# Samsung/tf-fast-rnnt

Hardware: AMD Instinct MI355X
Metric: rnnt_loss_pruned_fwd_bwd_throughput (higher is better)
Workload: dtype f32; 1 GPU; c3: rnnt_loss_pruned fwd+bwd step, B=32/GPU T=1000 S=200 C=500 s_range=5, regular, full boundary, first pass rnnt_loss_simple; global_batch=32, am_pruned=broadcast view

## Files before the change

### tf-fast-rnnt_amd/csrc/capi.hip

```cpp
#include "ftr_common.h"
#ifdef FTR_DIAG
#include "../../include/ftr_diag.h"
#endif
#include <stdlib.h>
#include <string.h>

namespace ftr {
namespace {
thread_local char g_err[512] = {0};
#ifdef FTR_DIAG
int g_mi_impl = -1;
#endif

int device_ok() {
  int n = 0;
  hipError_t e = hipGetDeviceCount(&n);
  if (e != hipSuccess || n <= 0) {
    (void)hipGetLastError();
    set_error("no usable HIP device (%s); this library has no CPU path", e == hipSuccess ? "device count is 0" : hipGetErrorString(e));
    return FTR_ERR_NO_DEVICE;
  }
  return FTR_OK;
}

// ... 334 lines not shown
int ftr_pruned_joiner_act_bwd_ws_dt(const void* g_out, const void* out, int kind, int act, const int32_t* ranges,
                                    void* d_am, void* d_lm, int B, int T, int S1, int C, int r,
                                    void* workspace, size_t workspace_bytes, void* stream) {
  clear_error();
  FTR_TRY(check_dtype("pruned_joiner_act_bwd_ws_dt", kind, 0));
  FTR_TRY(check_act("pruned_joiner_act_bwd_ws_dt", act));
  const char* what = "do_pruning_bwd_ws";
  FTR_TRY(check_sizes(what, B >= 0 && T >= 0 && S1 >= 1 && C >= 0 && r >= 0));
  if ((size_t)B * C == 0) return FTR_OK;
  FTR_TRY(pointers_then_device(what, g_out && out && ranges && d_am && d_lm));
  return pruned_joiner_act_bwd_ws(g_out, out, kind, act, ranges, d_am, d_lm, B, T, S1, C, r, workspace, workspace_bytes, stream_of(stream));
}

static int pruned_logprobs_fwd_entry(const void* logits, int dtype, const int32_t* symbols, const int32_t* ranges,
                                     const int32_t* boundary, int termination_symbol, double delay_penalty,
                                     float* lse, float* px, float* py, int B, int T, int S, int C, int r,
                                     int modified, int hat, void* stream) {
  const char* what = hat ? "hat_pruned_logprobs_fwd" : "pruned_logprobs_fwd";
  clear_error();
  FTR_TRY(check_builder(what, B >= 0 && T >= 1 && S >= 1 && C >= 1 && r >= 1, termination_symbol, C, false, hat));
  FTR_TRY(check_s_range(what, r, S));
  if (B == 0) return FTR_OK;
  FTR_TRY(pointers_then_device(what, logits && symbols && ranges && lse && px && py));
  return pruned_logprobs_fwd(logits, dtype, symbols, ranges, boundary, termination_symbol, delay_penalty, lse, px, py, B, T, S, C, r, modified, hat, stream_of(stream));
}

int ftr_pruned_logprobs_fwd_f32(const float* logits, const int32_t* symbols, const int32_t* ranges,
                                const int32_t* boundary, int termination_symbol, double delay_penalty,
                                float* lse, float* px, float* py, int B, int T, int S, int C, int r,
                                int modified, void* stream) {
  return pruned_logprobs_fwd_entry(logits, FTR_DTYPE_F32, symbols, ranges, boundary, termination_symbol, delay_penalty, lse, px, py, B, T, S, C, r, modified, 0, stream);
}

int ftr_hat_pruned_logprobs_fwd_f32(const float* logits, const int32_t* symbols, const int32_t* ranges,
                                    const int32_t* boundary, int termination_symbol, double delay_penalty,
                                    float* lse, float* px, float* py, int B, int T, int S, int C, int r,
                                    int modified, void* stream) {
  return pruned_logprobs_fwd_entry(logits, FTR_DTYPE_F32, symbols, ranges, boundary, termination_symbol, delay_penalty, lse, px, py, B, T, S, C, r, modified, 1, stream);
}

int ftr_pruned_logprobs_fwd_dt(const void* logits, int kind, const int32_t* symbols, const int32_t* ranges,
                               const int32_t* boundary, int termination_symbol, double delay_penalty, float* lse,
                               float* px, float* py, int B, int T, int S, int C, int r, int modified, int flags,
                               void* stream) {
  clear_error();
  FTR_TRY(check_dtype("pruned_logprobs_fwd_dt", kind, flags));
  return pruned_logprobs_fwd_entry(logits, kind, symbols, ranges, boundary, termination_symbol, delay_penalty, lse, px, py, B, T, S, C, r, modified, flags & FTR_PRUNED_HAT, stream);
}

int ftr_pruned_logprobs_bwd_f32(const float* logits, const int32_t* symbols, const int32_t* ranges,
                                const int32_t* boundary, int termination_symbol, const float* lse,
                                const float* gpx, const float* gpy, const float* scale, float* glogits,
                                int B, int T, int S, int C, int r, int modified, void* stream) {
  const char* what = "pruned_logprobs_bwd";
  clear_error();
  FTR_TRY(check_builder(what, B >= 0 && T >= 1 && S >= 1 && C >= 1 && r >= 1, termination_symbol, C));
  if (B == 0) return FTR_OK;
  FTR_TRY(pointers_then_device(what, logits && symbols && ranges && lse && gpx && gpy && glogits));
  return pruned_logprobs_bwd(logits, FTR_DTYPE_F32, symbols, ranges, boundary, termination_symbol, lse, gpx, gpy, Scale{scale, 1, 1.0f}, glogits, B, T, S, C, r, modified, 0, stream_of(stream));
}

static int rowmax_exp_entry(const char* what, const float* x, float* probs, float* rowmax, float* rowsum, const float* dotvec,
                            float* dot, bool extras_there, long long rows, int C, void* stream) {
  clear_error();
  FTR_REQUIRE(rows >= 0 && C >= 0, "%s: negative size", what);
  if (rows == 0 || C == 0) return FTR_OK;
  FTR_TRY(pointers_then_device(what, x && probs && rowmax && extras_there));
  return simple_rowmax_exp(x, probs, rowmax, rowsum, dotvec, dot, (size_t)rows, C, stream_of(stream));
}

int ftr_rowmax_exp_f32(const float* x, float* probs, float* rowmax, long long rows, int C, void* stream) {
  return rowmax_exp_entry("rowmax_exp", x, probs, rowmax, nullptr, nullptr, nullptr, true, rows, C, stream);
}

int ftr_rowmax_exp_sum_f32(const float* x, float* probs, float* rowmax, float* rowsum, long long rows, int C,
                           void* stream) {
  return rowmax_exp_entry("rowmax_exp_sum", x, probs, rowmax, rowsum, nullptr, nullptr, rowsum != nullptr, rows, C, stream);
}

int ftr_rowmax_exp_dot_f32(const float* x, float* probs, float* rowmax, const float* dotvec, float* dot, long long rows,
                           int C, void* stream) {
  return rowmax_exp_entry("rowmax_exp_dot", x, probs, rowmax, nullptr, dotvec, dot, dotvec && dot, rows, C, stream);
}

int ftr_rowmax_exp_pair_f32(const float* x1, float* probs1, float* rowmax1, long long rows1, const float* x2, float* probs2,
                            float* rowmax2, long long rows2, int C, void* stream) {
  clear_error();
  FTR_REQUIRE(rows1 >= 0 && rows2 >= 0 && C >= 0, "rowmax_exp_pair: negative size");
  if (rows1 + rows2 == 0 || C == 0) return FTR_OK;
  FTR_TRY(pointers_then_device("rowmax_exp_pair", (rows1 == 0 || (x1 && probs1 && rowmax1)) && (rows2 == 0 || (x2 && probs2 && rowmax2))));
  return simple_rowmax_exp_pair(x1, probs1, rowmax1, (size_t)rows1, x2, probs2, rowmax2, (size_t)rows2, C, stream_of(stream));
}

int ftr_rowdot_f32(const float* x, const float* v, float* dot, long long rows, int C, void* stream) {
  clear_error();
  FTR_REQUIRE(rows >= 0 && C >= 0, "rowdot: negative size");
  if (rows == 0) return FTR_OK;
  FTR_TRY(pointers_then_device("rowdot", dot && ((x && v) || C == 0)));
  return simple_rowdot(x, v, dot, (size_t)rows, C, stream_of(stream));
}

size_t ftr_colsum_weighted_workspace_floats(long long rows, int C) {
  return (rows < 0 || C < 0) ? 0 : simple_colsum_workspace_floats((size_t)rows, C);
}

int ftr_colsum_weighted_f32(const float* x, const float* w, float* out, float* workspace, size_t workspace_floats,
                            long long rows, int C, void* stream) {
  clear_error();
  FTR_REQUIRE(rows >= 0 && C >= 0, "colsum_weighted: negative size");
  if (C == 0) return FTR_OK;
  FTR_TRY(pointers_then_device("colsum_weighted", out && ((x && w && workspace) || rows == 0)));
  return simple_colsum_weighted(x, w, out, workspace, workspace_floats, (size_t)rows, C, stream_of(stream));
}

static int simple_fwd_entry(const char* what, bool smoothed, const float* am, const float* lm, const int32_t* symbols,
                            const float* prod, const float* am_max, const float* lm_max, const float* lmonly_norm,
                            const float* amonly_norm, const float* unigram_log, const int32_t* boundary,
                            int termination_symbol, double delay_penalty, float combined_scale, float lm_only_scale,
                            float am_only_scale, float* px, float* py, int B, int T, int S, int C, int modified, void* stream) {
  clear_error();
  FTR_TRY(check_builder(what, B >= 0 && T >= 1 && S >= 0 && C >= 1, termination_symbol, C));
  if (B == 0) return FTR_OK;
  FTR_TRY(pointers_then_device(what, am && lm && prod && am_max && lm_max && (!smoothed || (lmonly_norm && amonly_norm && unigram_log)) && py && (symbols || S == 0) && (px || S == 0)));
  return simple_logprobs_fwd(am, lm, symbols, prod, am_max, lm_max, boundary, termination_symbol, delay_penalty, lmonly_norm, amonly_norm, unigram_log, combined_scale, lm_only_scale, am_only_scale, px, py, B, T, S, C, modified, stream_of(stream));
}

int ftr_simple_logprobs_fwd_f32(const float* am, const float* lm, const int32_t* symbols, const float* prod,
                                const float* am_max, const float* lm_max, const int32_t* boundary,
                                int termination_symbol, double delay_penalty, float* px, float* py, int B, int T,
                                int S, int C, int modified, void* stream) {
  return simple_fwd_entry("simple_logprobs_fwd", false, am, lm, symbols, prod, am_max, lm_max, nullptr, nullptr, nullptr, boundary, termination_symbol, delay_penalty, 1.0f, 0.0f, 0.0f, px, py, B, T, S, C, modified, stream);
}

int ftr_smoothed_logprobs_fwd_f32(const float* am, const float* lm, const int32_t* symbols, const float* prod,
                                  const float* am_max, const float* lm_max, const float* lmonly_norm,
                                  const float* amonly_norm, const float* unigram_log, const int32_t* boundary,
                                  int termination_symbol, float combined_scale, float lm_only_scale,
                                  float am_only_scale, float* px, float* py, int B, int T, int S, int C,
                                  int modified, void* stream) {
  return simple_fwd_entry("smoothed_logprobs_fwd", true, am, lm, symbols, prod, am_max, lm_max, lmonly_norm, amonly_norm, unigram_log, boundary, termination_symbol, 0.0, combined_scale, lm_only_scale, am_only_scale, px, py, B, T, S, C, modified, stream);
}

int ftr_smoothed_logprobs_fwd_pen_f32(const float* am, const float* lm, const int32_t* symbols, const float* prod,
                                      const float* am_max, const float* lm_max, const float* lmonly_norm,
                                      const float* amonly_norm, const float* unigram_log, const int32_t* boundary,
                                      int termination_symbol, double delay_penalty, float combined_scale,
                                      float lm_only_scale, float am_only_scale, float* px, float* py, int B, int T,
                                      int S, int C, int modified, void* stream) {
  return simple_fwd_entry("smoothed_logprobs_fwd_pen", true, am, lm, symbols, prod, am_max, lm_max, lmonly_norm, amonly_norm, unigram_log, boundary, termination_symbol, delay_penalty, combined_scale, lm_only_scale, am_only_scale, px, py, B, T, S, C, modified, stream);
}

static int bwd_w_entry(const char* what, const float* gpx, const float* gpy, const float* scale, int scale_stride,
                       float scale_mul, const float* prod, const int32_t* boundary, float combined_scale, float* W,
                       float* rsx, float* rsy, int B, int T, int S, int modified, void* stream) {
  clear_error();
  FTR_TRY(check_sizes(what, B >= 0 && T >= 1 && S >= 0));
  FTR_TRY(check_scale_stride(what, scale_stride));
  if (B == 0) return FTR_OK;
  FTR_TRY(pointers_then_device(what, gpy && prod && W && rsx && rsy && (gpx || S == 0)));
  return simple_logprobs_bwd_w(gpx, gpy, Scale{scale, scale_stride, scale_mul}, prod, boundary, W, rsx, rsy, combined_scale, B, T, S, modified, stream_of(stream));
}

int ftr_simple_logprobs_bwd_w_f32(const float* gpx, const float* gpy, const float* prod, const int32_t* boundary,
                                  float* W, float* rsx, float* rsy, int B, int T, int S, int modified, void* stream) {
  return bwd_w_entry("simple_logprobs_bwd_w", gpx, gpy, nullptr, 0, 1.0f, prod, boundary, 1.0f, W, rsx, rsy, B, T, S, modified, stream);
}

int ftr_smoothed_logprobs_bwd_w_f32(const float* gpx, const float* gpy, const float* prod, const int32_t* boundary,
                                    float combined_scale, float* W, float* rsx, float* rsy, int B, int T, int S,
                                    int modified, void* stream) {
  return bwd_w_entry("smoothed_logprobs_bwd_w", gpx, gpy, nullptr, 0, 1.0f, prod, boundary, combined_scale, W, rsx, rsy, B, T, S, modified, stream);
}

int ftr_simple_logprobs_bwd_w_scaled_f32(const float* gpx, const float* gpy, const float* scale, int scale_stride,
                                         float scale_mul, const float* prod, const int32_t* boundary, float* W,
                                         float* rsx, float* rsy, int B, int T, int S, int modified, void* stream) {
  return bwd_w_entry("simple_logprobs_bwd_w_scaled", gpx, gpy, scale, scale_stride, scale_mul, prod, boundary, 1.0f, W, rsx, rsy, B, T, S, modified, stream);
}

int ftr_smoothed_logprobs_bwd_w_scaled_f32(const float* gpx, const float* gpy, const float* scale, int scale_stride,
                                           float scale_mul, const float* prod, const int32_t* boundary,
                                           float combined_scale, float* W, float* rsx, float* rsy, int B, int T, int S,
                                           int modified, void* stream) {
  return bwd_w_entry("smoothed_logprobs_bwd_w_scaled", gpx, gpy, scale, scale_stride, scale_mul, prod, boundary, combined_scale, W, rsx, rsy, B, T, S, modified, stream);
}

static int bwd_am_entry(const char* what, bool smoothed, const float* gpx, const float* gpy, const float* scale,
                        int scale_stride, float scale_mul, const float* damp, const float* am_probs,
                        const int32_t* symbols, const int32_t* boundary, int termination_symbol, float direct_scale,
                        const float* unigram, const float* am_dot, float am_only_scale, float* R, float* d_am, int B,
                        int T, int S, int C, int modified, void* stream) {
  clear_error();
  FTR_TRY(check_builder(what, B >= 0 && T >= 1 && S >= 0 && C >= 1, termination_symbol, C, true));
  FTR_TRY(check_scale_stride(what, scale_stride));
  if (B == 0) return FTR_OK;
  FTR_TRY(pointers_then_device(what, gpy && damp && am_probs && d_am && (!smoothed || (unigram && am_dot && R)) && (gpx || S == 0) && (symbols || S == 0)));
  return simple_logprobs_bwd_am(gpx, gpy, Scale{scale, scale_stride, scale_mul}, damp, am_probs, symbols, boundary, termination_symbol, direct_scale, unigram, am_dot, am_only_scale, R, d_am, B, T, S, C, modified, stream_of(stream));
}

int ftr_simple_logprobs_bwd_am_f32(const float* gpx, const float* gpy, const float* damp, const float* am_probs,
                                   const int32_t* symbols, const int32_t* boundary, int termination_symbol,
                                   float* d_am, int B, int T, int S, int C, int modified, void* stream) {
  return bwd_am_entry("simple_logprobs_bwd_am", false, gpx, gpy, nullptr, 0, 1.0f, damp, am_probs, symbols, boundary, termination_symbol, 1.0f, nullptr, nullptr, 0.0f, nullptr, d_am, B, T, S, C, modified, stream);
}

int ftr_smoothed_logprobs_bwd_am_f32(const float* gpx, const float* gpy, const float* damp, const float* am_probs,
                                     const int32_t* symbols, const int32_t* boundary, int termination_symbol,
                                     float direct_scale, const float* unigram, const float* am_dot,
                                     float am_only_scale, float* R, float* d_am, int B, int T, int S, int C,
                                     int modified, void* stream) {
  return bwd_am_entry("smoothed_logprobs_bwd_am", true, gpx, gpy, nullptr, 0, 1.0f, damp, am_probs, symbols, boundary, termination_symbol, direct_scale, unigram, am_dot, am_only_scale, R, d_am, B, T, S, C, modified, stream);
}

int ftr_simple_logprobs_bwd_am_scaled_f32(const float* gpx, const float* gpy, const float* scale, int scale_stride,
                                          float scale_mul, const float* damp, const float* am_probs,
                                          const int32_t* symbols, const int32_t* boundary, int termination_symbol,
                                          float* d_am, int B, int T, int S, int C, int modified, void* stream) {
  return bwd_am_entry("simple_logprobs_bwd_am_scaled", false, gpx, gpy, scale, scale_stride, scale_mul, damp, am_probs, symbols, boundary, termination_symbol, 1.0f, nullptr, nullptr, 0.0f, nullptr, d_am, B, T, S, C, modified, stream);
}

int ftr_smoothed_logprobs_bwd_am_scaled_f32(const float* gpx, const float* gpy, const float* scale, int scale_stride,
                                            float scale_mul, const float* damp, const float* am_probs,
                                            const int32_t* symbols, const int32_t* boundary, int termination_symbol,
                                            float direct_scale, const float* unigram, const float* am_dot,
                                            float am_only_scale, float* R, float* d_am, int B, int T, int S, int C,
                                            int modified, void* stream) {
  return bwd_am_entry("smoothed_logprobs_bwd_am_scaled", true, gpx, gpy, scale, scale_stride, scale_mul, damp, am_probs, symbols, boundary, termination_symbol, direct_scale, unigram, am_dot, am_only_scale, R, d_am, B, T, S, C, modified, stream);
}

static int bwd_lm_entry(const char* what, bool smoothed, const float* dlmp, const float* lm_probs, const int32_t* symbols,
                        const float* rsx, const float* rsy, int termination_symbol, float direct_scale,
                        const float* row_term, const float* inv_rowsum, const float* unigram_grad, float* d_lm, int B,
                        int S, int C, void* stream) {
  clear_error();
  FTR_TRY(check_builder(what, B >= 0 && S >= 0 && C >= 1, termination_symbol, C, true));
  if (B == 0) return FTR_OK;
  FTR_TRY(pointers_then_device(what, dlmp && lm_probs && rsx && rsy && d_lm && (!smoothed || (row_term && inv_rowsum && unigram_grad)) && (symbols || S == 0)));
  return simple_logprobs_bwd_lm(dlmp, lm_probs, symbols, rsx, rsy, termination_symbol, direct_scale, row_term, inv_rowsum, unigram_grad, d_lm, B, S, C, stream_of(stream));
}

int ftr_simple_logprobs_bwd_lm_f32(const float* dlmp, const float* lm_probs, const int32_t* symbols,
                                   const float* rsx, const float* rsy, int termination_symbol, float* d_lm, int B,
                                   int S, int C, void* stream) {
  return bwd_lm_entry("simple_logprobs_bwd_lm", false, dlmp, lm_probs, symbols, rsx, rsy, termination_symbol, 1.0f, nullptr, nullptr, nullptr, d_lm, B, S, C, stream);
}

int ftr_smoothed_logprobs_bwd_lm_f32(const float* dlmp, const float* lm_probs, const int32_t* symbols,
                                     const float* rsx, const float* rsy, int termination_symbol, float direct_scale,
                                     const float* row_term, const float* inv_rowsum, const float* unigram_grad,
                                     float* d_lm, int B, int S, int C, void* stream) {
  return bwd_lm_entry("smoothed_logprobs_bwd_lm", true, dlmp, lm_probs, symbols, rsx, rsy, termination_symbol, direct_scale, row_term, inv_rowsum, unigram_grad, d_lm, B, S, C, stream);
}

int ftr_negated_reduce_f32(const float* ans, int B, int reduction, float* out, void* stream) {
  clear_error();
  FTR_REQUIRE(B >= 1 && reduction >= 0 && reduction <= 2, "negated_reduce: bad arguments B=%d reduction=%d", B, reduction);
  FTR_TRY(pointers_then_device("negated_reduce", ans && out));
  return negated_reduce(ans, B, reduction, out, stream_of(stream));
}

static int pruned_logprobs_bwd_scaled_entry(const void* logits, int dtype, const int32_t* symbols, const int32_t* ranges,
                                            const int32_t* boundary, int termination_symbol, const float* lse,
                                            const float* gpx, const float* gpy, const float* scale, int scale_stride,
                                            float scale_mul, void* glogits, int B, int T, int S, int C, int r,
                                            int modified, int hat, void* stream) {
  const char* what = hat ? "hat_pruned_logprobs_bwd_scaled" : "pruned_logprobs_bwd_scaled";
  clear_error();
  FTR_TRY(check_builder(what, B >= 0 && T >= 1 && S >= 0 && C >= 1 && r >= 1, termination_symbol, C, true, hat));
  FTR_TRY(check_scale_stride(what, scale_stride));
  if (B == 0) return FTR_OK;
  FTR_TRY(pointers_then_device(what, logits && ranges && lse && gpy && glogits && (symbols || S == 0) && (gpx || S == 0)));
  return pruned_logprobs_bwd(logits, dtype, symbols, ranges, boundary, termination_symbol, lse, gpx, gpy, Scale{scale, scale_stride, scale_mul}, glogits, B, T, S, C, r, modified, hat, stream_of(stream));
}

int ftr_pruned_logprobs_bwd_scaled_f32(const float* logits, const int32_t* symbols, const int32_t* ranges,
                                       const int32_t* boundary, int termination_symbol, const float* lse,
                                       const float* gpx, const float* gpy, const float* scale, int scale_stride,
                                       float scale_mul, float* glogits, int B, int T, int S, int C, int r,
                                       int modified, void* stream) {
  return pruned_logprobs_bwd_scaled_entry(logits, FTR_DTYPE_F32, symbols, ranges, boundary, termination_symbol, lse, gpx, gpy, scale, scale_stride, scale_mul, glogits, B, T, S, C, r, modified, 0, stream);
}

int ftr_hat_pruned_logprobs_bwd_scaled_f32(const float* logits, const int32_t* symbols, const int32_t* ranges,
                                           const int32_t* boundary, int termination_symbol, const float* lse,
                                           const float* gpx, const float* gpy, const float* scale, int scale_stride,
                                           float scale_mul, float* glogits, int B, int T, int S, int C, int r,
                                           int modified, void* stream) {
  return pruned_logprobs_bwd_scaled_entry(logits, FTR_DTYPE_F32, symbols, ranges, boundary, termination_symbol, lse, gpx, gpy, scale, scale_stride, scale_mul, glogits, B, T, S, C, r, modified, 1, stream);
}

int ftr_pruned_logprobs_bwd_scaled_dt(const void* logits, int kind, const int32_t* symbols, const int32_t* ranges,
                                      const int32_t* boundary, int termination_symbol, const float* lse,
                                      const float* gpx, const float* gpy, const float* scale, int scale_stride,
                                      float scale_mul, void* glogits, int B, int T, int S, int C, int r, int modified,
                                      int flags, void* stream) {
  clear_error();
  FTR_TRY(check_dtype("pruned_logprobs_bwd_scaled_dt", kind, flags));
  return pruned_logprobs_bwd_scaled_entry(logits, kind, symbols, ranges, boundary, termination_symbol, lse, gpx, gpy, scale, scale_stride, scale_mul, glogits, B, T, S, C, r, modified, flags & FTR_PRUNED_HAT, stream);
}

int ftr_simple_logprobs_fused_supported(int C) { return simple_fused_supported(C); }
int ftr_simple_logprobs_fused_bwd_supported(int T, int C) { return simple_fused_bwd_supported(T, C); }

int ftr_normalizer_gemm_f32(int kind, const float* x, const float* y, float* out, int B, int T, int S1, int C, void* stream) {
  FTR_REQUIRE(B >= 0 && T >= 0 && S1 >= 0 && C >= 0, "normalizer_gemm: bad sizes");
  if ((size_t)B * T * S1 * C == 0) return FTR_OK;
  FTR_REQUIRE(x && y && out, "normalizer_gemm: null pointer");
  return normalizer_gemm(kind, x, y, out, B, T, S1, C, reinterpret_cast<hipStream_t>(stream));
}

int ftr_normalizer_gemm_choice(int kind, int B, int T, int S1, int C, int* solution, float* us, float* us_default, int* candidates) {
  return normalizer_gemm_choice(kind, B, T, S1, C, solution, us, us_default, candidates);
}

int ftr_normalizer_gemm_set_choice(int kind, int B, int T, int S1, int C, int solution) {
  return normalizer_gemm_set_choice(kind, B, T, S1, C, solution);
}

static int fused_fwd_entry(const char* what, bool smoothed, const float* am, const float* lm, const int32_t* symbols,
                           const float* am_probs, const float* lm_probs, const float* am_max, const float* lm_max,
                           const float* lmonly_norm, const float* amonly_norm, const float* unigram_log,
                           const int32_t* boundary, int termination_symbol, double delay_penalty, float combined_scale,
                           float lm_only_scale, float am_only_scale, float* px, float* py, float* prod, int B, int T,
                           int S, int C, int modified, void* stream) {
  clear_error();
  FTR_TRY(check_builder(what, B >= 0 && T >= 1 && S >= 0 && C >= 1, termination_symbol, C));
  if (B == 0) return FTR_OK;
  FTR_TRY(pointers_then_device(what, am && lm && am_probs && lm_probs && am_max && lm_max && (!smoothed || (lmonly_norm && amonly_norm && unigram_log)) && py && (symbols || S == 0) && (px || S == 0)));
  return simple_fused_fwd(am, lm, symbols, am_probs, lm_probs, am_max, lm_max, boundary, termination_symbol, delay_penalty, lmonly_norm, amonly_norm, unigram_log, combined_scale, lm_only_scale, am_only_scale, px, py, prod, B, T, S, C, modified, stream_of(stream));
}

int ftr_simple_logprobs_fused_fwd_f32(const float* am, const float* lm, const int32_t* symbols, const float* am_probs,
                                      const float* lm_probs, const float* am_max, const float* lm_max,
                                      const int32_t* boundary, int termination_symbol, double delay_penalty, float* px,
                                      float* py, float* prod, int B, int T, int S, int C, int modified, void* stream) {
  return fused_fwd_entry("simple_logprobs_fused_fwd", false, am, lm, symbols, am_probs, lm_probs, am_max, lm_max, nullptr, nullptr, nullptr, boundary, termination_symbol, delay_penalty, 1.0f, 0.0f, 0.0f, px, py, prod, B, T, S, C, modified, stream);
}

int ftr_smoothed_logprobs_fused_fwd_f32(const float* am, const float* lm, const int32_t* symbols, const float* am_probs,
                                        const float* lm_probs, const float* am_max, const float* lm_max,
                                        const float* lmonly_norm, const float* amonly_norm, const float* unigram_log,
                                        const int32_t* boundary, int termination_symbol, double delay_penalty,
                                        float combined_scale, float lm_only_scale, float am_only_scale, float* px,
                                        float* py, float* prod, int B, int T, int S, int C, int modified, void* stream) {
  return fused_fwd_entry("smoothed_logprobs_fused_fwd", true, am, lm, symbols, am_probs, lm_probs, am_max, lm_max, lmonly_norm, amonly_norm, unigram_log, boundary, termination_symbol, delay_penalty, combined_scale, lm_only_scale, am_only_scale, px, py, prod, B, T, S, C, modified, stream);
}

static int fused_bwd_am_entry(const char* what, bool smoothed, const float* gpx, const float* gpy, const float* scale,
                              int scale_stride, float scale_mul, const float* prod, const float* lm_probs,
                              const float* am_probs, const int32_t* symbols, const int32_t* boundary,
                              int termination_symbol, float combined_scale, float direct_scale, const float* unigram,
                              const float* am_dot, float am_only_scale, float* R, float* d_am, int B, int T, int S, int C,
                              int modified, void* stream) {
  clear_error();
  FTR_TRY(check_builder(what, B >= 0 && T >= 1 && S >= 0 && C >= 1, termination_symbol, C, true));
  FTR_TRY(check_scale_stride(what, scale_stride));
  if (B == 0) return FTR_OK;
  FTR_TRY(pointers_then_device(what, gpy && prod && lm_probs && am_probs && d_am && (!smoothed || (unigram && am_dot && R)) && (gpx || S == 0) && (symbols || S == 0)));
  return simple_fused_bwd_am(gpx, gpy, Scale{scale, scale_stride, scale_mul}, prod, lm_probs, am_probs, symbols, boundary, termination_symbol, combined_scale, direct_scale, unigram, am_dot, am_only_scale, R, d_am, B, T, S, C, modified, stream_of(stream));
}

int ftr_simple_logprobs_fused_bwd_am_f32(const float* gpx, const float* gpy, const float* scale, int scale_stride,
                                         float scale_mul, const float* prod, const float* lm_probs, const float* am_probs,
                                         const int32_t* symbols, const int32_t* boundary, int termination_symbol,
                                         float* d_am, int B, int T, int S, int C, int modified, void* stream) {
  return fused_bwd_am_entry("simple_logprobs_fused_bwd_am", false, gpx, gpy, scale, scale_stride, scale_mul, prod, lm_probs, am_probs, symbols, boundary, termination_symbol, 1.0f, 1.0f, nullptr, nullptr, 0.0f, nullptr, d_am, B, T, S, C, modified, stream);
}

int ftr_smoothed_logprobs_fused_bwd_am_f32(const float* gpx, const float* gpy, const float* scale, int scale_stride,
                                           float scale_mul, const float* prod, const float* lm_probs,
                                           const float* am_probs, const int32_t* symbols, const int32_t* boundary,
                                           int termination_symbol, float combined_scale, float direct_scale,
                                           const float* unigram, const float* am_dot, float am_only_scale, float* R,
                                           float* d_am, int B, int T, int S, int C, int modified, void* stream) {
  return fused_bwd_am_entry("smoothed_logprobs_fused_bwd_am", true, gpx, gpy, scale, scale_stride, scale_mul, prod, lm_probs, am_probs, symbols, boundary, termination_symbol, combined_scale, direct_scale, unigram, am_dot, am_only_scale, R, d_am, B, T, S, C, modified, stream);
}

static int fused_bwd_am_w_entry(const char* what, bool smoothed, const float* gpx, const float* gpy, const float* scale,
                                int scale_stride, float scale_mul, const float* W, const float* lm_probs,
                                const float* am_probs, const int32_t* symbols, const int32_t* boundary,
                                int termination_symbol, float direct_scale, const float* unigram, const float* am_dot,
                                float am_only_scale, float* R, float* d_am, int B, int T, int S, int C, int modified,
                                void* stream) {
  clear_error();
  FTR_TRY(check_builder(what, B >= 0 && T >= 1 && S >= 0 && C >= 1, termination_symbol, C, true));
  FTR_TRY(check_scale_stride(what, scale_stride));
  if (B == 0) return FTR_OK;
  FTR_TRY(pointers_then_device(what, gpy && W && lm_probs && am_probs && d_am && (!smoothed || (unigram && am_dot && R)) && (gpx || S == 0) && (symbols || S == 0)));
  return simple_fused_bwd_am_w(gpx, gpy, Scale{scale, scale_stride, scale_mul}, W, lm_probs, am_probs, symbols, boundary, termination_symbol, direct_scale, unigram, am_dot, am_only_scale, R, d_am, B, T, S, C, modified, stream_of(stream));
}

int ftr_simple_logprobs_fused_bwd_am_w_f32(const float* gpx, const float* gpy, const float* scale, int scale_stride,
                                           float scale_mul, const float* W, const float* lm_probs, const float* am_probs,
                                           const int32_t* symbols, const int32_t* boundary, int termination_symbol,
                                           float* d_am, int B, int T, int S, int C, int modified, void* stream) {
  return fused_bwd_am_w_entry("simple_logprobs_fused_bwd_am_w", false, gpx, gpy, scale, scale_stride, scale_mul, W, lm_probs, am_probs, symbols, boundary, termination_symbol, 1.0f, nullptr, nullptr, 0.0f, nullptr, d_am, B, T, S, C, modified, stream);
}

int ftr_smoothed_logprobs_fused_bwd_am_w_f32(const float* gpx, const float* gpy, const float* scale, int scale_stride,
                                             float scale_mul, const float* W, const float* lm_probs,
                                             const float* am_probs, const int32_t* symbols, const int32_t* boundary,
                                             int termination_symbol, float direct_scale, const float* unigram,
                                             const float* am_dot, float am_only_scale, float* R, float* d_am, int B, int T,
                                             int S, int C, int modified, void* stream) {
  return fused_bwd_am_w_entry("smoothed_logprobs_fused_bwd_am_w", true, gpx, gpy, scale, scale_stride, scale_mul, W, lm_probs, am_probs, symbols, boundary, termination_symbol, direct_scale, unigram, am_dot, am_only_scale, R, d_am, B, T, S, C, modified, stream);
}

int ftr_simple_logprobs_fused_bwd_am_w_columns(int B, int T, int C) { return simple_fused_bwd_columns(B, T, C); }

int ftr_mutual_information_band_supported(int T, int S, int r) { return mi_band_supported(T, S, r); }

static int pruned_band_fwd_entry(const void* logits, int dtype, const int32_t* symbols, const int32_t* ranges, const int32_t* boundary,
                                 int termination_symbol, double delay_penalty, float* lse, float* px_band, float* py_band,
                                 int B, int T, int S, int C, int r, int modified, int hat, void* stream) {
  const char* what = hat ? "hat_pruned_band_fwd" : "pruned_band_fwd";
  clear_error();
  FTR_TRY(check_builder(what, B >= 0 && T >= 1 && S >= 0 && C >= 1 && r >= 1, termination_symbol, C, false, hat));
  if (B == 0) return FTR_OK;
  FTR_TRY(pointers_then_device(what, logits && ranges && lse && px_band && py_band && (symbols || S == 0)));
  FTR_TRY(lse_rows_dtype(logits, dtype, lse, (size_t)B * T * r, C, termination_symbol, hat, stream_of(stream)));
  return band_gather(logits, dtype, symbols, ranges, boundary, lse, termination_symbol, delay_penalty, px_band, py_band, B, T, S, C, r, modified, hat, stream_of(stream));
}

int ftr_pruned_band_fwd_f32(const float* logits, const int32_t* symbols, const int32_t* ranges, const int32_t* boundary,
                            int termination_symbol, double delay_penalty, float* lse, float* px_band, float* py_band,
                            int B, int T, int S, int C, int r, int modified, void* stream) {
  return pruned_band_fwd_entry(logits, FTR_DTYPE_F32, symbols, ranges, boundary, termination_symbol, delay_penalty, lse, px_band, py_band, B, T, S, C, r, modified, 0, stream);
}

int ftr_hat_pruned_band_fwd_f32(const float* logits, const int32_t* symbols, const int32_t* ranges, const int32_t* boundary,
                                int termination_symbol, double delay_penalty, float* lse, float* px_band, float* py_band,
                                int B, int T, int S, int C, int r, int modified, void* stream) {
  return pruned_band_fwd_entry(logits, FTR_DTYPE_F32, symbols, ranges, boundary, termination_symbol, delay_penalty, lse, px_band, py_band, B, T, S, C, r, modified, 1, stream);
}

int ftr_pruned_band_fwd_dt(const void* logits, int kind, const int32_t* symbols, const int32_t* ranges,
                           const int32_t* boundary, int termination_symbol, double delay_penalty, float* lse,
                           float* px_band, float* py_band, int B, int T, int S, int C, int r, int modified, int flags,
                           void* stream) {
  clear_error();
  FTR_TRY(check_dtype("pruned_band_fwd_dt", kind, flags));
  return pruned_band_fwd_entry(logits, kind, symbols, ranges, boundary, termination_symbol, delay_penalty, lse, px_band, py_band, B, T, S, C, r, modified, flags & FTR_PRUNED_HAT, stream);
}

int ftr_band_ranges_check_i32(const int32_t* ranges, const int32_t* boundary, int32_t* flags, int B, int T, int r, void* stream) {
  clear_error();
  FTR_TRY(check_sizes("band_ranges_check", B >= 0 && T >= 0 && r >= 1));
  FTR_TRY(pointers_then_device("band_ranges_check", flags && (ranges || B == 0 || T == 0)));
  return band_ranges_check(ranges, boundary, flags, B, T, r, stream_of(stream));
}

int ftr_mutual_information_band_f32(const float* px_band, const float* py_band, const int32_t* ranges,
                                    const int32_t* boundary, float* ans, float* gx_band, float* gy_band, int B, int T,
                                    int S, int r, int modified, void* stream) {
  return ftr_mutual_information_band_ws_f32(px_band, py_band, ranges, boundary, nullptr, 0, ans, gx_band, gy_band, B, T, S, r, modified, stream);
}

size_t ftr_mutual_information_band_workspace_floats(int B, int T, int S, int r) {
  return (B < 0 || T < 1 || S < 0 || r < 1) ? 0 : mi_band_workspace_floats(B, T, S, r);
}

int ftr_mutual_information_band_ws_f32(const float* px_band, const float* py_band, const int32_t* ranges,
                                       const int32_t* boundary, float* workspace, size_t workspace_floats, float* ans,
                                       float* gx_band, float* gy_band, int B, int T, int S, int r, int modified,
                                       void* stream) {
  clear_error();
  FTR_TRY(check_sizes("mutual_information_band", B >= 0 && T >= 1 && S >= 0 && r >= 1));
  if (B == 0) return FTR_OK;
  FTR_TRY(pointers_then_device("mutual_information_band", px_band && py_band && ranges && ans && gx_band && gy_band));
  return mi_band(px_band, py_band, ranges, boundary, workspace, workspace_floats, ans, gx_band, gy_band, B, T, S, r, modified, stream_of(stream));
}

static int pruned_band_bwd_scaled_entry(const void* logits, int dtype, const int32_t* symbols, const int32_t* ranges,
                                        const int32_t* boundary, int termination_symbol, const float* lse,
                                        const float* gx_band, const float* gy_band, const float* scale, int scale_stride,
                                        float scale_mul, void* glogits, int B, int T, int S, int C, int r, int modified,
                                        int hat, void* stream) {
  const char* what = hat ? "hat_pruned_band_bwd_scaled" : "pruned_band_bwd_scaled";
  clear_error();
  FTR_TRY(check_builder(what, B >= 0 && T >= 1 && S >= 0 && C >= 1 && r >= 1, termination_symbol, C, true, hat));
  FTR_TRY(check_scale_stride(what, scale_stride));
  if (B == 0) return FTR_OK;
  FTR_TRY(pointers_then_device(what, logits && ranges && lse && gx_band && gy_band && glogits && (symbols || S == 0)));
  return band_grad_banded(logits, dtype, symbols, ranges, boundary, termination_symbol, lse, gx_band, gy_band, Scale{scale, scale_stride, scale_mul}, glogits, B, T, S, C, r, modified, hat, stream_of(stream));
}

int ftr_pruned_band_bwd_scaled_f32(const float* logits, const int32_t* symbols, const int32_t* ranges,
                                   const int32_t* boundary, int termination_symbol, const float* lse,
                                   const float* gx_band, const float* gy_band, const float* scale, int scale_stride,
                                   float scale_mul, float* glogits, int B, int T, int S, int C, int r, int modified,
                                   void* stream) {
  return pruned_band_bwd_scaled_entry(logits, FTR_DTYPE_F32, symbols, ranges, boundary, termination_symbol, lse, gx_band, gy_band, scale, scale_stride, scale_mul, glogits, B, T, S, C, r, modified, 0, stream);
}

int ftr_hat_pruned_band_bwd_scaled_f32(const float* logits, const int32_t* symbols, const int32_t* ranges,
                                       const int32_t* boundary, int termination_symbol, const float* lse,
                                       const float* gx_band, const float* gy_band, const float* scale, int scale_stride,
                                       float scale_mul, float* glogits, int B, int T, int S, int C, int r, int modified,
                                       void* stream) {
  return pruned_band_bwd_scaled_entry(logits, FTR_DTYPE_F32, symbols, ranges, boundary, termination_symbol, lse, gx_band, gy_band, scale, scale_stride, scale_mul, glogits, B, T, S, C, r, modified, 1, stream);
}

int ftr_pruned_band_bwd_scaled_dt(const void* logits, int kind, const int32_t* symbols, const int32_t* ranges,
                                  const int32_t* boundary, int termination_symbol, const float* lse,
                                  const float* gx_band, const float* gy_band, const float* scale, int scale_stride,
                                  float scale_mul, void* glogits, int B, int T, int S, int C, int r, int modified,
                                  int flags, void* stream) {
  clear_error();
  FTR_TRY(check_dtype("pruned_band_bwd_scaled_dt", kind, flags));
  return pruned_band_bwd_scaled_entry(logits, kind, symbols, ranges, boundary, termination_symbol, lse, gx_band, gy_band, scale, scale_stride, scale_mul, glogits, B, T, S, C, r, modified, flags & FTR_PRUNED_HAT, stream);
}

namespace {
int mb_check_durations(const char* what, const int32_t* durations, int D, bool first_is_one) {
  FTR_REQUIRE(D >= 1 && D <= 8, "%s: D = %d, the number of blanks must be in 1..8", what, D);
  FTR_REQUIRE(durations, "%s: null durations", what);
  for (int j = 0; j < D; ++j) {
    FTR_REQUIRE(durations[j] >= 1 && durations[j] <= 32, "%s: durations[%d] = %d is outside 1..32", what, j, durations[j]);
    FTR_REQUIRE(j == 0 || durations[j] > durations[j - 1], "%s: durations must be strictly increasing (durations[%d] = %d after %d)",
                what, j, durations[j], durations[j - 1]);
  }
  FTR_REQUIRE(!first_is_one || durations[0] == 1, "%s: durations[0] = %d, the standard blank advances one frame", what, durations[0]);
  return FTR_OK;
}
int mb_check_ids(const char* what, const int32_t* ids, int D, int blank, int C) {
  FTR_REQUIRE(C >= 1 && blank >= 0 && blank < C, "%s: termination_symbol %d not in [0,%d)", what, blank, C);
  FTR_REQUIRE(ids || D == 1, "%s: null big_blank_ids", what);
  for (int j = 0; j + 1 < D; ++j) {
    FTR_REQUIRE(ids[j] >= 0 && ids[j] < C, "%s: big_blank_ids[%d] = %d not in [0,%d)", what, j, ids[j], C);
    FTR_REQUIRE(ids[j] != blank, "%s: big_blank_ids[%d] = %d is the termination_symbol", what, j, ids[j]);
    for (int i = 0; i < j; ++i)
      FTR_REQUIRE(ids[i] != ids[j], "%s: big_blank_ids[%d] = %d is a duplicate of big_blank_ids[%d]", what, j, ids[j], i);
  }
  return FTR_OK;
}
}

namespace {
int tdt_check_list(const char* what, const char* name, const int32_t* v, int n, int nmax, int lo, int hi = 16) {
  FTR_REQUIRE(n >= 1 && n <= nmax, "%s: %s holds %d values, must be 1..%d", what, name, n, nmax);
  FTR_REQUIRE(v, "%s: null %s", what, name);
  for (int j = 0; j < n; ++j) {
    FTR_REQUIRE(v[j] >= lo && v[j] <= hi, "%s: %s[%d] = %d is outside %d..%d", what, name, j, v[j], lo, hi);
    FTR_REQUIRE(j == 0 || v[j] > v[j - 1], "%s: %s must be strictly increasing (%s[%d] = %d after %d)", what, name, name, j,
                v[j], v[j - 1]);
  }
  return FTR_OK;
}
int tdt_check_moves(const char* what, const int32_t* token_durations, int Dx, const int32_t* blank_durations, int Dy,
                    int blank_hi = 16, int max_moves = 9) {
  FTR_TRY(tdt_check_list(what, "token_durations", token_durations, Dx, 8, 0));
  FTR_TRY(tdt_check_list(what, "blank_durations", blank_durations, Dy, 8, 1, blank_hi));
  FTR_REQUIRE(Dx + Dy <= max_moves, "%s: Dx + Dy = %d moves (token_durations and blank_durations together), at most %d", what,
              Dx + Dy, max_moves);
  return FTR_OK;
}
int tdt_check_head(const char* what, const int32_t* durations, int N, double sigma, int blank, int C) {
  FTR_TRY(tdt_check_list(what, "durations", durations, N, 5, 0));
  FTR_REQUIRE(durations[N - 1] >= 1, "%s: durations holds no positive value: no move advances a frame", what);
  FTR_REQUIRE(sigma >= 0.0, "%s: sigma = %g must not be negative", what, sigma);
  FTR_REQUIRE(C >= 1 && blank >= 0 && blank < C, "%s: termination_symbol %d not in [0,%d)", what, blank, C);
// ... 398 lines not shown
```

### tf-fast-rnnt_amd/csrc/ftr_common.h

```cpp
#pragma once
#include <hip/hip_runtime.h>
#include <stdint.h>
#include <stdio.h>
#include <stdarg.h>
#include "../../include/ftr_kd.h"
#include "../../include/ftr_prune_sum.h"
#include "../../include/ftr_joiner_act.h"
#include "../../include/ftr_fused.h"
#include "../../include/ftr_band_tdt.h"
#include "../../include/ftr_band_multiblank.h"
#include "../../include/ftr_band_viterbi.h"

namespace ftr {

void set_error(const char* fmt, ...);
void clear_error();

inline int check_launch(const char* what) {
  hipError_t e = hipGetLastError();
  if (e != hipSuccess) {
    set_error("%s: launch failed: %s", what, hipGetErrorString(e));
    return FTR_ERR_LAUNCH;
  }
  return FTR_OK;
}

inline int require_rows_32bit(const char* what, size_t rows) {
  if (rows > 0x7fffffffull) {
    set_error("%s: %zu rows (B*T*s_range) exceed the 2^31 - 1 that the launch grids index", what, rows);
    return FTR_ERR_INVALID_ARG;
  }
  return FTR_OK;
}

__global__ void zero_words_kernel(uint32_t* __restrict__ p, size_t n);
__global__ void copy_words_kernel(uint32_t* __restrict__ dst, const uint32_t* __restrict__ src, size_t n);
inline int zero_words(void* p, size_t n_words, hipStream_t st, const char* what) {
  if (n_words == 0) return FTR_OK;
  const size_t blocks = (n_words + 4 * 256 - 1) / (4 * 256);
  hipLaunchKernelGGL(zero_words_kernel, dim3((unsigned)(blocks > 4096 ? 4096 : blocks)), dim3(256), 0, st, static_cast<uint32_t*>(p), n_words);
  return check_launch(what);
}
inline int copy_words(void* dst, const void* src, size_t n_words, hipStream_t st, const char* what) {
  if (n_words == 0) return FTR_OK;
  const size_t blocks = (n_words + 255) / 256;
  hipLaunchKernelGGL(copy_words_kernel, dim3((unsigned)(blocks > 4096 ? 4096 : blocks)), dim3(256), 0, st, static_cast<uint32_t*>(dst),
                     static_cast<const uint32_t*>(src), n_words);
  return check_launch(what);
}

constexpr float kNeg = -1.0e30f;
constexpr float kNegThresh = -1.0e29f;
constexpr float kLog2e = 1.4426950408889634f;
constexpr float kLn2 = 0.6931471805599453f;

typedef float f4u __attribute__((ext_vector_type(4), aligned(4)));
typedef float f4 __attribute__((ext_vector_type(4)));

struct bf16_t { uint16_t bits; };
struct fp16_t { uint16_t bits; };
typedef uint16_t h4 __attribute__((ext_vector_type(4)));

__device__ __forceinline__ float elem_to_float(float v) { return v; }
__device__ __forceinline__ float elem_to_float(bf16_t v) { return (float)__builtin_bit_cast(__bf16, v.bits); }
__device__ __forceinline__ float elem_to_float(fp16_t v) { return (float)__builtin_bit_cast(_Float16, v.bits); }
template <typename E> __device__ __forceinline__ E elem_from_float(float v);
template <> __device__ __forceinline__ float elem_from_float<float>(float v) { return v; }
template <> __device__ __forceinline__ bf16_t elem_from_float<bf16_t>(float v) { return bf16_t{__builtin_bit_cast(uint16_t, (__bf16)v)}; }
template <> __device__ __forceinline__ fp16_t elem_from_float<fp16_t>(float v) { return fp16_t{__builtin_bit_cast(uint16_t, (_Float16)v)}; }

__device__ __forceinline__ f4 load4(const float* row, int i) { return reinterpret_cast<const f4u*>(row)[i]; }
__device__ __forceinline__ void store4(float* row, int i, f4 v) { reinterpret_cast<f4u*>(row)[i] = v; }
template <typename E>
__device__ __forceinline__ f4 load4(const E* row, int i) {
  const h4 h = reinterpret_cast<const h4*>(row)[i];
  f4 v;
#pragma unroll
  for (int e = 0; e < 4; ++e) v[e] = elem_to_float(E{h[e]});
  return v;
}
template <typename E>
__device__ __forceinline__ void store4(E* row, int i, f4 v) {
  h4 h;
#pragma unroll
  for (int e = 0; e < 4; ++e) h[e] = elem_from_float<E>(v[e]).bits;
  reinterpret_cast<h4*>(row)[i] = h;
}
__device__ __forceinline__ void store4_nt(float* row, int i, f4 v) { __builtin_nontemporal_store(v, reinterpret_cast<f4u*>(row) + i); }
template <typename E>
__device__ __forceinline__ void store4_nt(E* row, int i, f4 v) {
  h4 h;
#pragma unroll
  for (int e = 0; e < 4; ++e) h[e] = elem_from_float<E>(v[e]).bits;
  __builtin_nontemporal_store(h, reinterpret_cast<h4*>(row) + i);
}

struct Scale {
  const float* p; int stride; float mul;
  __device__ __forceinline__ float at(int b) const { return (p ? p[(size_t)b * stride] : 1.0f) * mul; }
};
inline Scale scale_none() { return Scale{nullptr, 0, 1.0f}; }

template <int CTRL, int ROW_MASK, int BANK_MASK>
__device__ __forceinline__ float dpp_take(float identity, float src) {
  return __builtin_bit_cast(float, __builtin_amdgcn_update_dpp(__builtin_bit_cast(int, identity), __builtin_bit_cast(int, src),
                                                               CTRL, ROW_MASK, BANK_MASK, false));
}
__device__ __forceinline__ float wave_sum_dpp(float v) {
  v += dpp_take<0x111, 0xf, 0xf>(0.0f, v);
  v += dpp_take<0x112, 0xf, 0xf>(0.0f, v);
  v += dpp_take<0x114, 0xf, 0xe>(0.0f, v);
  v += dpp_take<0x118, 0xf, 0xc>(0.0f, v);
  v += dpp_take<0x142, 0xa, 0xf>(0.0f, v);
  v += dpp_take<0x143, 0xc, 0xf>(0.0f, v);
  return __builtin_bit_cast(float, __builtin_amdgcn_readlane(__builtin_bit_cast(int, v), 63));
}
__device__ __forceinline__ float wave_max_dpp(float v) {
  constexpr float ninf = -__builtin_inff();
  v = fmaxf(v, dpp_take<0x111, 0xf, 0xf>(ninf, v));
  v = fmaxf(v, dpp_take<0x112, 0xf, 0xf>(ninf, v));
  v = fmaxf(v, dpp_take<0x114, 0xf, 0xe>(ninf, v));
  v = fmaxf(v, dpp_take<0x118, 0xf, 0xc>(ninf, v));
  v = fmaxf(v, dpp_take<0x142, 0xa, 0xf>(ninf, v));
  v = fmaxf(v, dpp_take<0x143, 0xc, 0xf>(ninf, v));
  return __builtin_bit_cast(float, __builtin_amdgcn_readlane(__builtin_bit_cast(int, v), 63));
}

struct Shift { float cx2, cy2; };
__device__ __forceinline__ bool shift_sample_ok(float v) { return v > -1.0e4f && v < 1.0e4f; }
template <bool MOD>
__device__ __forceinline__ Shift shift_from_sums(float sumx, float nx, float sumy, float ny, int Sn, int Tn) {
  const float steps = MOD ? (float)(Tn - 1) : (float)(Sn - 1 + Tn - 1);
  float f = steps > 0.0f ? (float)(Sn - 1) / steps : 0.5f;
  f = fminf(fmaxf(f, 1.0e-3f), 1.0f - 1.0e-3f);
  const float mx = nx > 0.0f ? sumx / nx : 0.0f, my = ny > 0.0f ? sumy / ny : 0.0f;
  Shift s;
  s.cx2 = mx * kLog2e - __builtin_amdgcn_logf(f);
  s.cy2 = my * kLog2e - __builtin_amdgcn_logf(1.0f - f);
  return s;
}
template <bool MOD>
__device__ __forceinline__ double shift_total(const Shift s, int Sn, int Tn) {
  const int nx = Sn - 1, ny = MOD ? (Tn - 1) - (Sn - 1) : (Tn - 1);
  return (double)nx * (double)s.cx2 + (double)ny * (double)s.cy2;
}

struct Bound { int sb, tb, se, te; };
__device__ __forceinline__ Bound load_boundary(const int32_t* __restrict__ boundary, int b, int S, int T) {
  Bound r;
  if (boundary) {
    r.sb = max(boundary[4 * b + 0], 0); r.tb = max(boundary[4 * b + 1], 0);
    r.se = min(boundary[4 * b + 2], S); r.te = min(boundary[4 * b + 3], T);
  } else { r.sb = 0; r.tb = 0; r.se = S; r.te = T; }
  return r;
}

__device__ __forceinline__ float softplus(float v) { return fmaxf(v, 0.0f) + log1pf(expf(-fabsf(v))); }
__device__ __forceinline__ void hat_logprobs(float xb, float xs, float Z, bool sym_is_blank, float* vx, float* vy) {
  *vy = -softplus(-xb);
  *vx = sym_is_blank ? -INFINITY : (xs - Z) - softplus(xb);
}
__device__ __forceinline__ void hat_sigmoids(float xb, float* sp, float* sn) {
  const float e = expf(-fabsf(xb)), big = 1.0f / (1.0f + e), small = e / (1.0f + e);
  *sp = xb >= 0.0f ? big : small;
  *sn = xb >= 0.0f ? small : big;
}

}

namespace ftr {
int mi_plain_fwd(const float* px, const float* py, const int32_t* boundary, float* p, float* ans, int B, int S, int T, int modified, hipStream_t st);
int mi_plain_bwd(const float* px, const float* py, const int32_t* boundary, const float* p, float* p_grad, float* px_grad, float* py_grad, float* ans_grad, int overwrite, int B, int S, int T, int modified, hipStream_t st);
int mi_bidir_fwd(const float* px, const float* py, const int32_t* boundary, float* ws, size_t ws_floats, int flags, float* ans, int B, int S, int T, int modified, hipStream_t st);
int mi_bidir_bwd(const int32_t* boundary, const float* ws, size_t ws_floats, int flags, float* px_grad, float* py_grad, float* ans_grad, int overwrite, int B, int S, int T, int modified, hipStream_t st, const float* ans = nullptr, float* loss_out = nullptr, int loss_code = 0);
int mi_bidir_ws_init(float* ws, size_t ws_floats, int B, int S, int T, hipStream_t st);
int mi_bidir_status(const float* ws, size_t ws_floats, int B, int S, int T, int* status_host, long long* dirty_host, hipStream_t st);
size_t mi_bidir_workspace_floats(int B, int S, int T);
size_t mi_bidir_handoff_floats(int B, int S, int T);
size_t mi_viterbi_workspace_bytes(int B, int S, int T);
int mi_viterbi(const float* px, const float* py, const int32_t* boundary, void* ws, size_t ws_bytes, float* score, int32_t* frames, int B, int S, int T, int modified, hipStream_t st);
size_t mi_multiblank_workspace_floats(int B, int S, int T);
int mi_multiblank_fwd(const float* px, const float* py, const int32_t* boundary, const int32_t* durations, int D, float* ws, size_t ws_floats, float* ans, int B, int S, int T, hipStream_t st);
int mi_multiblank_bwd(const float* px, const float* py, const int32_t* boundary, const int32_t* durations, int D, float* ws, size_t ws_floats, const float* ans_grad, float* px_grad, float* py_grad, int B, int S, int T, hipStream_t st);
int multiblank_logprobs_fwd(const float* logits, const int32_t* symbols, const int32_t* ranges, const int32_t* boundary, int blank, const int32_t* big_ids, const int32_t* durations, int D, double sigma, double delay_penalty, float* lse, float* px, float* py, int B, int T, int S, int C, int r, hipStream_t st);
int multiblank_logprobs_bwd(const float* logits, const int32_t* symbols, const int32_t* ranges, const int32_t* boundary, int blank, const int32_t* big_ids, const int32_t* durations, int D, const float* lse, const float* gpx, const float* gpy, Scale scale, float* glogits, int B, int T, int S, int C, int r, hipStream_t st);
size_t mi_tdt_workspace_floats(int B, int S, int T);
int mi_tdt_fwd(const float* px, const float* py, const int32_t* boundary, const int32_t* token_durations, int Dx, const int32_t* blank_durations, int Dy, float* ws, size_t ws_floats, float* ans, int B, int S, int T, hipStream_t st);
int mi_tdt_bwd(const float* px, const float* py, const int32_t* boundary, const int32_t* token_durations, int Dx, const int32_t* blank_durations, int Dy, float* ws, size_t ws_floats, const float* ans_grad, float* px_grad, float* py_grad, int B, int S, int T, hipStream_t st);
int tdt_logprobs_fwd(const float* logits, const int32_t* symbols, const int32_t* ranges, const int32_t* boundary, int blank, const int32_t* durations, int N, double sigma, double delay_penalty, float* lse_tok, float* lse_dur, float* px, float* py, int B, int T, int S, int C, int r, hipStream_t st);
int tdt_logprobs_bwd(const float* logits, const int32_t* symbols, const int32_t* ranges, const int32_t* boundary, int blank, const int32_t* durations, int N, const float* lse_tok, const float* lse_dur, const float* gpx, const float* gpy, Scale scale, float* glogits, int B, int T, int S, int C, int r, hipStream_t st);
struct BandMoveDomain { int max_tok, max_blk, max_dur; };
constexpr BandMoveDomain kBandTdtDomain{5, 5, 16};
constexpr BandMoveDomain kBandMultiblankDomain{1, 8, 32};
int mi_band_tdt_supported(int T, int S, int r, int N, int Ny, BandMoveDomain dom);
size_t mi_band_tdt_workspace_floats(int B, int T, int S, int r, int N, int Ny, BandMoveDomain dom);
int mi_band_tdt(const float* pxb, const float* pyb, const int32_t* ranges, const int32_t* boundary, const int32_t* token_durations, int N, const int32_t* blank_durations, int Ny, float* ws, size_t ws_floats, float* ans, float* gxb, float* gyb, int B, int T, int S, int r, BandMoveDomain dom, const char* what, hipStream_t st);
int tdt_band_fwd(const float* logits, const int32_t* symbols, const int32_t* ranges, const int32_t* boundary, int blank, const int32_t* durations, int N, double sigma, double delay_penalty, float* lse_tok, float* lse_dur, float* pxb, float* pyb, int B, int T, int S, int C, int r, hipStream_t st);
int tdt_band_bwd(const float* logits, const int32_t* symbols, const int32_t* ranges, const int32_t* boundary, int blank, const int32_t* durations, int N, const float* lse_tok, const float* lse_dur, const float* gxb, const float* gyb, Scale scale, float* glogits, int B, int T, int S, int C, int r, hipStream_t st);
int mi_band_multiblank(const float* pxb, const float* pyb, const int32_t* ranges, const int32_t* boundary, const int32_t* durations, int D, float* ws, size_t ws_floats, float* ans, float* gxb, float* gyb, int B, int T, int S, int r, hipStream_t st);
int multiblank_band_fwd(const float* logits, const int32_t* symbols, const int32_t* ranges, const int32_t* boundary, int blank, const int32_t* big_ids, const int32_t* durations, int D, double sigma, double delay_penalty, float* lse, float* pxb, float* pyb, int B, int T, int S, int C, int r, hipStream_t st);
int multiblank_band_bwd(const float* logits, const int32_t* symbols, const int32_t* ranges, const int32_t* boundary, int blank, const int32_t* big_ids, const int32_t* durations, int D, const float* lse, const float* gxb, const float* gyb, Scale scale, float* glogits, int B, int T, int S, int C, int r, hipStream_t st);
size_t mi_viterbi_tdt_workspace_bytes(int B, int S, int T);
int mi_viterbi_tdt(const float* px, const float* py, const int32_t* boundary, const int32_t* token_durations, int Dx, const int32_t* blank_durations, int Dy, void* ws, size_t ws_bytes, float* score, int32_t* frames, int32_t* durations, int32_t* blank_steps, int B, int S, int T, hipStream_t st);
int mi_band_viterbi_supported(int T, int S, int r, int N, int Ny);
size_t mi_band_viterbi_workspace_bytes(int B, int T, int S, int r, int N, int Ny);
int mi_band_viterbi(const float* pxb, const float* pyb, const int32_t* ranges, const int32_t* boundary, const int32_t* token_durations, int N, const int32_t* blank_durations, int Ny, void* ws, size_t ws_bytes, float* score, int32_t* frames, int32_t* durations, int32_t* blank_steps, int B, int T, int S, int r, hipStream_t st);
int cummin_i32(const int32_t* in, int32_t* out, int rows, int cols, hipStream_t st);
int prune_ranges(const float* px_grad, const float* py_grad, const int32_t* boundary, int32_t* ranges, int32_t* s_begin, int B, int S, int T, int T1, int r, hipStream_t st);
int do_pruning(const float* am, const float* lm, const int32_t* ranges, float* am_p, float* lm_p, int B, int T, int S1, int C, int r, hipStream_t st);
size_t do_pruning_bwd_workspace_bytes(int B, int T, int S1, int C, int r);
int do_pruning_bwd_ws(const float* g_am_p, const float* g_lm_p, const int32_t* ranges, float* d_am, float* d_lm, int B, int T, int S1, int C, int r, void* ws, size_t ws_bytes, hipStream_t st);
int do_pruning_bwd(const float* g_am_p, const float* g_lm_p, const int32_t* ranges, float* d_am, float* d_lm, int B, int T, int S1, int C, int r, hipStream_t st);
int do_pruning_sum(const void* am, const void* lm, int dtype, const int32_t* ranges, void* out, int B, int T, int S1, int C, int r, hipStream_t st);
int do_pruning_sum_bwd_ws(const void* g, int dtype, const int32_t* ranges, void* d_am, void* d_lm, int B, int T, int S1, int C, int r, void* ws, size_t ws_bytes, hipStream_t st);
int pruned_joiner_act(const void* am, const void* lm, int dtype, int act, const int32_t* ranges, void* out, int B, int T, int S1, int C, int r, hipStream_t st);
int pruned_joiner_act_bwd_ws(const void* g, const void* out, int dtype, int act, const int32_t* ranges, void* d_am, void* d_lm, int B, int T, int S1, int C, int r, void* ws, size_t ws_bytes, hipStream_t st);
int pruned_logprobs_fwd(const void* logits, int dtype, const int32_t* symbols, const int32_t* ranges, const int32_t* boundary, int blank, double delay_penalty, float* lse, float* px, float* py, int B, int T, int S, int C, int r, int modified, int hat, hipStream_t st);
int pruned_logprobs_bwd(const void* logits, int dtype, const int32_t* symbols, const int32_t* ranges, const int32_t* boundary, int blank, const float* lse, const float* gpx, const float* gpy, Scale scale, void* glogits, int B, int T, int S, int C, int r, int modified, int hat, hipStream_t st);
int simple_rowmax_exp(const float* x, float* probs, float* rowmax, float* rowsum, const float* dotvec, float* dot, size_t rows, int C, hipStream_t st);
int simple_rowmax_exp_pair(const float* x1, float* probs1, float* rowmax1, size_t rows1, const float* x2, float* probs2, float* rowmax2, size_t rows2, int C, hipStream_t st);
int simple_rowdot(const float* x, const float* v, float* dot, size_t rows, int C, hipStream_t st);
size_t simple_colsum_workspace_floats(size_t rows, int C);
int simple_colsum_weighted(const float* x, const float* w, float* out, float* ws, size_t ws_floats, size_t rows, int C, hipStream_t st);
int simple_logprobs_fwd(const float* am, const float* lm, const int32_t* symbols, const float* prod, const float* am_max, const float* lm_max, const int32_t* boundary, int blank, double delay_penalty, const float* lmonly_norm, const float* amonly_norm, const float* ulog, float cs, float ls, float as, float* px, float* py, int B, int T, int S, int C, int modified, hipStream_t st);
int simple_logprobs_bwd_w(const float* gpx, const float* gpy, Scale scale, const float* prod, const int32_t* boundary, float* W, float* rsx, float* rsy, float cs, int B, int T, int S, int modified, hipStream_t st);
int simple_logprobs_bwd_am(const float* gpx, const float* gpy, Scale scale, const float* damp, const float* am_probs, const int32_t* symbols, const int32_t* boundary, int blank, float kdir, const float* uvec, const float* amdot, float as, float* Rout, float* d_am, int B, int T, int S, int C, int modified, hipStream_t st);
int simple_logprobs_bwd_lm(const float* dlmp, const float* lm_probs, const int32_t* symbols, const float* rsx, const float* rsy, int blank, float kdir, const float* arow, const float* invsum, const float* gu, float* d_lm, int B, int S, int C, hipStream_t st);
int simple_fused_supported(int C);
int simple_fused_bwd_supported(int T, int C);
int normalizer_gemm(int kind, const float* x, const float* y, float* out, int B, int T, int S1, int C, hipStream_t st);
int normalizer_gemm_choice(int kind, int B, int T, int S1, int C, int* solution, float* us, float* us_default, int* candidates);
int normalizer_gemm_set_choice(int kind, int B, int T, int S1, int C, int solution);
int simple_fused_fwd(const float* am, const float* lm, const int32_t* symbols, const float* am_probs, const float* lm_probs, const float* am_max, const float* lm_max, const int32_t* boundary, int blank, double delay_penalty, const float* lmonly_norm, const float* amonly_norm, const float* ulog, float cs, float ls, float as, float* px, float* py, float* prod_out, int B, int T, int S, int C, int modified, hipStream_t st);
int simple_fused_bwd_am(const float* gpx, const float* gpy, Scale scale, const float* prod, const float* lm_probs, const float* am_probs, const int32_t* symbols, const int32_t* boundary, int blank, float cs, float kdir, const float* uvec, const float* amdot, float as, float* Rout, float* d_am, int B, int T, int S, int C, int modified, hipStream_t st);
int simple_fused_bwd_columns(int B, int T, int C);
int simple_fused_bwd_am_w(const float* gpx, const float* gpy, Scale scale, const float* W, const float* lm_probs, const float* am_probs, const int32_t* symbols, const int32_t* boundary, int blank, float kdir, const float* uvec, const float* amdot, float as, float* Rout, float* d_am, int B, int T, int S, int C, int modified, hipStream_t st);
int negated_reduce(const float* ans, int B, int reduction, float* out, hipStream_t st, float sign = -1.0f);
int pruned_kd_fwd(const void* logits, int dtype, const void* teacher, int teacher_dtype, const int32_t* symbols, const int32_t* ranges, const int32_t* boundary, int blank, float temperature, int collapsed, float* node, float* saved, float* utt, int B, int T, int S, int C, int r, hipStream_t st);
int pruned_kd_bwd(const void* logits, int dtype, const void* teacher, int teacher_dtype, const int32_t* symbols, const int32_t* ranges, const int32_t* boundary, int blank, float temperature, int collapsed, const float* saved, Scale scale, void* glogits, int B, int T, int S, int C, int r, hipStream_t st);
int lse_rows(const float* logits, float* lse, size_t rows, int C, int blank, int hat, hipStream_t st);
int lse_rows_dtype(const void* logits, int dtype, float* lse, size_t rows, int C, int blank, int hat, hipStream_t st);
int mi_band_supported(int T, int S, int r);
int band_ranges_check(const int32_t* ranges, const int32_t* boundary, int* flags, int B, int T, int r, hipStream_t st);
int band_gather(const void* logits, int dtype, const int32_t* symbols, const int32_t* ranges, const int32_t* boundary, const float* lse, int blank, double delay_penalty, float* pxb, float* pyb, int B, int T, int S, int C, int r, int modified, int hat, hipStream_t st);
size_t mi_band_workspace_floats(int B, int T, int S, int r);
int mi_band_seg_supported(int T, int S, int r);
size_t mi_band_seg_workspace_floats(int B, int T, int S, int r);
int mi_band_seg(const float* pxb, const float* pyb, const int32_t* ranges, const int32_t* boundary, float* ws, size_t ws_floats, float* ans, float* gxb, float* gyb, int B, int T, int S, int r, int modified, hipStream_t st);
int mi_band(const float* pxb, const float* pyb, const int32_t* ranges, const int32_t* boundary, float* ws, size_t ws_floats, float* ans, float* gxb, float* gyb, int B, int T, int S, int r, int modified, hipStream_t st);
int band_grad_banded(const void* logits, int dtype, const int32_t* symbols, const int32_t* ranges, const int32_t* boundary, int blank, const float* lse, const float* gxb, const float* gyb, Scale scale, void* glogits, int B, int T, int S, int C, int r, int modified, int hat, hipStream_t st);
int selftest(hipStream_t st, int* result_dev);
int debug_stamps(unsigned long long* out16);
int debug_trace(unsigned long long* out, int n);
}
```

### tf-fast-rnnt_amd/csrc/simple_fused.hip

```cpp
#include "ftr_common.h"
#include "launch.h"
#include <cstdlib>

namespace ftr {
namespace {

constexpr float kTinyF = 1.401298464324817e-45f;
template <int MB> struct FusedTile {
  static constexpr int FT = 64 * MB, FK = 32, FLD = FK + 4, NBUF = MB == 1 ? 2 : 1;
};
typedef float v4f __attribute__((ext_vector_type(4)));

constexpr int kGLD = 68;
template <int NS, int MB>
__host__ __device__ constexpr size_t fused_lds_bytes() {
  constexpr size_t tile = FusedTile<MB>::NBUF * (size_t)(FusedTile<MB>::FT + 16 * NS) * FusedTile<MB>::FLD;
  constexpr size_t gather = (size_t)16 * NS * kGLD + 16 * NS + (size_t)16 * NS * 8 + (size_t)FusedTile<MB>::FT * 4;
  return sizeof(float) * (tile > gather ? tile : gather);
}

template <bool MOD, bool SMOOTH, int NS, int MB>
__global__ __launch_bounds__(256, 2) void simple_fused_fwd_kernel(
    const float* __restrict__ am, const float* __restrict__ lm, const int32_t* __restrict__ symbols,
    const float* __restrict__ am_probs, const float* __restrict__ lm_probs, const float* __restrict__ am_max,
// ... 99 lines not shown
    constexpr int kAheadU = 4, RING = 8;
    f4 af[MB][kFK / 16], ring[RING];
#pragma unroll
    for (int m = 0; m < MB; ++m)
#pragma unroll
      for (int g = 0; g < kFK / 16; ++g) af[m][g] = *reinterpret_cast<const f4*>(A + 64 * m * kFLD + 16 * g);
    auto bfetch = [&](int u) { return *reinterpret_cast<const f4*>(Bm + (u % NS) * 16 * kFLD + 16 * (u / NS)); };
#pragma unroll
    for (int u = 0; u < kAheadU; ++u) if (u < NUNIT) ring[u % RING] = bfetch(u);
#pragma unroll
    for (int u = 0; u < NUNIT; u += 2) {
      if (u + kAheadU < NUNIT) ring[(u + kAheadU) % RING] = bfetch(u + kAheadU);
      if (u + kAheadU + 1 < NUNIT) ring[(u + kAheadU + 1) % RING] = bfetch(u + kAheadU + 1);
      const int g0 = u / NS, i0 = u % NS;
      const f4 b0 = ring[u % RING];
      if (u + 1 < NUNIT) {
        const int g1 = (u + 1) / NS, i1 = (u + 1) % NS;
        const f4 b1 = ring[(u + 1) % RING];
#pragma unroll
        for (int e = 0; e < 4; ++e) {
#pragma unroll
          for (int m = 0; m < MB; ++m) {
            acc[m][i0] = __builtin_amdgcn_mfma_f32_16x16x4f32(af[m][g0][e], b0[e], acc[m][i0], 0, 0, 0);
            acc[m][i1] = __builtin_amdgcn_mfma_f32_16x16x4f32(af[m][g1][e], b1[e], acc[m][i1], 0, 0, 0);
          }
        }
      } else {
#pragma unroll
        for (int e = 0; e < 4; ++e)
#pragma unroll
          for (int m = 0; m < MB; ++m) acc[m][i0] = __builtin_amdgcn_mfma_f32_16x16x4f32(af[m][g0][e], b0[e], acc[m][i0], 0, 0, 0);
      }
      __builtin_amdgcn_sched_barrier(0);
    }
    if (NBUF == 1) __syncthreads();
    if (kc + 1 < nk) lstore(NBUF == 2 ? ((kc + 1) & 1) : 0, v);
    __syncthreads();
  }

  const int n = lane & 15;
  const int te = boundary ? boundary[4 * b + 3] : T;
  const float ulog_blank = SMOOTH ? ulog[blank] : 0.0f;
  float* asym = smem;
  int* sym_l = reinterpret_cast<int*>(smem + 16 * NS * kGLD);
  float* rrec = smem + 16 * NS * kGLD + 16 * NS;
  float* frec = rrec + 16 * NS * 8;
  if (tid < 16 * NS) {
    sym_l[tid] = r_sym;
    *reinterpret_cast<f4*>(rrec + 8 * tid) = f4{r_lmblank, r_lmx, r_lmsym, 0.f};
    if (SMOOTH) *reinterpret_cast<f4*>(rrec + 8 * tid + 4) = f4{r_lon, r_ulog, 0.f, 0.f};
  }
  if (tid < kFT) *reinterpret_cast<f4*>(frec + 4 * tid) = f4{f_amx, f_ablank, f_aon, 0.f};
  __syncthreads();
  float lm_blank[NS], lmx[NS], lon[NS], lm_sym[NS], ulog_sym[NS];
#pragma unroll
  for (int i = 0; i < NS; ++i) {
    const f4 ra = *reinterpret_cast<const f4*>(rrec + 8 * (16 * i + n));
    lm_blank[i] = ra[0]; lmx[i] = ra[1]; lm_sym[i] = ra[2];
    lon[i] = 0.f; ulog_sym[i] = 0.f;
    if (SMOOTH) { const f4 rb = *reinterpret_cast<const f4*>(rrec + 8 * (16 * i + n) + 4); lon[i] = rb[0]; ulog_sym[i] = rb[1]; }
  }
  constexpr int NSL = (16 * NS + 63) / 64;
  int mysym[NSL];
#pragma unroll
  for (int u = 0; u < NSL; ++u) mysym[u] = sym_l[min(lane + 64 * u, 16 * NS - 1)];
#pragma unroll
  for (int m = 0; m < MB; ++m) {
    if (m > 0) __syncthreads();
    {
      constexpr int GB = (MB == 2 && NS > 10) ? 8 : 16;
#pragma unroll
      for (int k0 = 0; k0 < 16; k0 += GB) {
        float gv[GB][NSL];
#pragma unroll
        for (int k = 0; k < GB; ++k) {
          const float* row = amb + (size_t)min(t0 + 64 * m + wave + 4 * (k0 + k), T - 1) * C;
#pragma unroll
          for (int u = 0; u < NSL; ++u) gv[k][u] = row[mysym[u]];
        }
#pragma unroll
        for (int k = 0; k < GB; ++k)
#pragma unroll
          for (int u = 0; u < NSL; ++u) {
            const int sl = lane + 64 * u;
            if (sl < 16 * NS) asym[sl * kGLD + wave + 4 * (k0 + k)] = gv[k][u];
          }
      }
    }
    __syncthreads();
    const int tq = t0 + 64 * m + 16 * wave + 4 * (lane >> 4);
    if (tq >= T1) continue;
    float amx[4], a_blank[4], aon[4], pen[4];
#pragma unroll
    for (int j = 0; j < 4; ++j) {
      const int t = tq + j;
      const f4 fr = *reinterpret_cast<const f4*>(frec + 4 * (64 * m + 16 * wave + 4 * (lane >> 4) + j));
      amx[j] = fr[0]; a_blank[j] = fr[1]; aon[j] = fr[2];
      pen[j] = (delay_penalty > 0.0) ? (float)((((double)te - 1.0) / 2.0 - (double)t) * delay_penalty) : 0.0f;
    }
    f4 a_sym[NS];
#pragma unroll
    for (int i = 0; i < NS; ++i) a_sym[i] = *reinterpret_cast<const f4*>(asym + (16 * i + n) * kGLD + 16 * wave + 4 * (lane >> 4));
#pragma unroll
    for (int i = 0; i < NS; ++i) {
      const int s = s0 + 16 * i + n;
      if (s > S) continue;
      f4 vy, vx, vp;
#pragma unroll
      for (int j = 0; j < 4; ++j) {
        const int t = tq + j;
        const float pr = acc[m][i][j];
        vp[j] = pr;
        const float nrm = logf(pr + kTinyF) + lmx[i] + amx[j];
        float y = a_blank[j] + lm_blank[i] - nrm;
        if (SMOOTH) y = y * cs + (lm_blank[i] - lon[i]) * ls + (a_blank[j] + ulog_blank - aon[j]) * as;
        vy[j] = y;
        float x = -INFINITY;
        if (s < S && t < T && (MOD || t != te)) {
          x = a_sym[i][j] + lm_sym[i] - nrm;
          if (SMOOTH) x = x * cs + (lm_sym[i] - lon[i]) * ls + (a_sym[i][j] + ulog_sym[i] - aon[j]) * as;
        }
        if (delay_penalty > 0.0) x += pen[j];
        vx[j] = x;
      }
      float* yrow = py + ((size_t)b * (S + 1) + s) * T + tq;
      if (tq + 3 < T) *reinterpret_cast<f4u*>(yrow) = vy;
      else { for (int j = 0; j < 4; ++j) if (tq + j < T) yrow[j] = vy[j]; }
      if (prod_out) {
        float* prow = prod_out + ((size_t)b * (S + 1) + s) * T + tq;
        if (tq + 3 < T) *reinterpret_cast<f4u*>(prow) = vp;
        else { for (int j = 0; j < 4; ++j) if (tq + j < T) prow[j] = vp[j]; }
      }
      if (s < S) {
        float* xrow = px + ((size_t)b * S + s) * T1 + tq;
        if (tq + 3 < T1) *reinterpret_cast<f4u*>(xrow) = vx;
        else { for (int j = 0; j < 4; ++j) if (tq + j < T1) xrow[j] = vx[j]; }
      }
    }
  }
}


constexpr int kBT = 64;
constexpr int kBS = 16;
constexpr int kBLT = kBT + 4;
constexpr int kBCB = 16;

template <int NCB>
__host__ __device__ constexpr size_t fused_bwd_lds_bytes() {
  return sizeof(float) * (2 * kBS * (16 * NCB) + 2 * kBS * kBLT + 2 * kBS * kBT);
}

template <bool MOD, bool USEW, int NCB>
__global__ __launch_bounds__(256, NCB <= 8 ? 4 : 2) void simple_fused_bwd_am_kernel(
    const float* __restrict__ gpx, const float* __restrict__ gpy, const Scale scale, const float* __restrict__ prod,
    const float* __restrict__ lm_probs, const float* __restrict__ am_probs, const int32_t* __restrict__ symbols,
    const int32_t* __restrict__ boundary, int blank, float cs, float kdir, const float* __restrict__ uvec,
    const float* __restrict__ amdot, float as, float* __restrict__ Rout, float* __restrict__ d_am, int T, int S, int C) {
  extern __shared__ __attribute__((aligned(16))) float smem[];
  constexpr int CT = 16 * NCB, LDC = CT, NG = NCB / 4;
  static_assert(NCB % 4 == 0 && NCB >= 8 && NCB <= 16, "column blocks come in interleaved groups of four");
  float* lmT = smem;
  float* wT = lmT + 2 * kBS * LDC;
  float* csb = wT + 2 * kBS * kBLT;
  int bx = blockIdx.x, by = blockIdx.y, bz = blockIdx.z;
  {
    const unsigned total = gridDim.x * gridDim.y * gridDim.z;
    if ((total & 7u) == 0) {
      const unsigned lin = blockIdx.x + gridDim.x * (blockIdx.y + gridDim.y * blockIdx.z);
      const unsigned j = (lin & 7u) * (total >> 3) + (lin >> 3);
      by = j % gridDim.y; bx = (j / gridDim.y) % gridDim.x; bz = j / (gridDim.x * gridDim.y);
    }
  }
  const int b = bz, t0 = bx * kBT, c0 = by * CT;
  const int tid = threadIdx.x, lane = tid & 63;
  const int wave = __builtin_amdgcn_readfirstlane(tid >> 6);
  const int T1 = MOD ? T : T + 1;
  const int te = boundary ? boundary[4 * b + 3] : T;
  const float sc = scale.at(b);
  const float* gxb = gpx + (size_t)b * S * T1;
  const float* gyb = gpy + (size_t)b * (S + 1) * T;
  const float* prb = prod + (size_t)b * (S + 1) * T;
  const float* lmb = lm_probs + (size_t)b * (S + 1) * C;
  const int nk = (S + 1 + kBS - 1) / kBS;

  constexpr int NL = (kBS * CT / 4) / 256;
  int lrow[NL], lcol[NL];
  float lmask[NL];
#pragma unroll
  for (int u = 0; u < NL; ++u) {
    const int e = tid + 256 * u, c = c0 + 4 * (e % (CT / 4));
    lrow[u] = e / (CT / 4);
    lcol[u] = min(c, C - 4);
    lmask[u] = c < C ? 1.0f : 0.0f;
  }
  const int wrow = tid >> 4, wq = tid & 15, wt = t0 + 4 * wq;
  const int wtc = min(wt, T - 4);
  const float tmask = wt < T ? 1.0f : 0.0f;
  f4 xmask;
#pragma unroll
  for (int e = 0; e < 4; ++e) xmask[e] = (wt < T && (MOD || wt + e != te)) ? sc : 0.0f;
  const bool want_y = !USEW || uvec != nullptr || (blank >= c0 && blank < c0 + CT);
  const bool want_x = !USEW || uvec != nullptr;
  struct Stage { f4 lv[NL]; f4 x, y, pr; };
  auto load = [&](int kc, Stage& g, bool want_all) {
    const int s = kc * kBS + wrow;
    const int sy_ = min(s, S), sx_ = min(s, S > 0 ? S - 1 : 0);
    if (want_all) {
#pragma unroll
      for (int u = 0; u < NL; ++u) g.lv[u] = *reinterpret_cast<const f4*>(lmb + (size_t)min(kc * kBS + lrow[u], S) * C + lcol[u]);
      g.pr = *reinterpret_cast<const f4u*>(prb + (size_t)sy_ * T + wtc);
      if (want_y) g.y = *reinterpret_cast<const f4u*>(gyb + (size_t)sy_ * T + wtc);
    }
    if (want_x) g.x = (S > 0) ? (f4)*reinterpret_cast<const f4u*>(gxb + (size_t)sx_ * T1 + wtc) : f4{0.f, 0.f, 0.f, 0.f};
  };
  f4 sx = {0.f, 0.f, 0.f, 0.f}, sy = {0.f, 0.f, 0.f, 0.f};

  v4f acc[NCB];
#pragma unroll
  for (int i = 0; i < NCB; ++i) acc[i] = v4f{0.f, 0.f, 0.f, 0.f};
  const int fk = lane >> 4, fn = lane & 15;

  {
    auto park = [&](int kc, const Stage& g) {
      const int buf = kc & 1;
#pragma unroll
      for (int u = 0; u < NL; ++u) {
        const float m = (kc * kBS + lrow[u] <= S) ? lmask[u] : 0.0f;
        *reinterpret_cast<f4*>(lmT + (buf * kBS + lrow[u]) * LDC + 4 * ((tid + 256 * u) % (CT / 4))) = g.lv[u] * m;
      }
      const int s = kc * kBS + wrow;
      const float rowy = s <= S ? sc * tmask : 0.0f, rowx = s < S ? 1.0f : 0.0f;
      f4 w;
      if (USEW) {
        w = (s <= S && wt < T) ? g.pr : f4{0.f, 0.f, 0.f, 0.f};
        if (want_x) sx += g.x * xmask * rowx;
        if (want_y) sy += g.y * rowy;
      } else {
        const f4 x = g.x * xmask * rowx, y = g.y * rowy;
#pragma unroll
        for (int e = 0; e < 4; ++e) w[e] = -cs * (x[e] + y[e]) / (g.pr[e] + kTinyF);
        sx += x; sy += y;
      }
      *reinterpret_cast<f4*>(wT + (buf * kBS + wrow) * kBLT + 4 * wq) = w;
    };
    auto compute = [&](int kc) {
      const int buf = kc & 1;
      const float* abase = lmT + (buf * kBS + fk) * LDC + 4 * fn;
      const float* bbase = wT + (buf * kBS + fk) * kBLT + 16 * wave + fn;
      f4 af[2][NG];
      float bw[kBS / 4];
#pragma unroll
      for (int kk = 0; kk < kBS / 4; ++kk) bw[kk] = bbase[4 * kk * kBLT];
#pragma unroll
      for (int g = 0; g < NG; ++g) af[0][g] = *reinterpret_cast<const f4*>(abase + 64 * g);
#pragma unroll
      for (int kk = 0; kk < kBS / 4; ++kk) {
        if (kk + 1 < kBS / 4) {
#pragma unroll
          for (int g = 0; g < NG; ++g) af[(kk + 1) & 1][g] = *reinterpret_cast<const f4*>(abase + 4 * (kk + 1) * LDC + 64 * g);
        }
        __builtin_amdgcn_sched_barrier(0);
#pragma unroll
        for (int g = 0; g < NG; ++g)
#pragma unroll
          for (int e = 0; e < 4; ++e)
            acc[4 * g + e] = __builtin_amdgcn_mfma_f32_16x16x4f32(af[kk & 1][g][e], bw[kk], acc[4 * g + e], 0, 0, 0);
        __builtin_amdgcn_sched_barrier(0);
      }
    };
    Stage g;
    load(0, g, true);
    park(0, g);
    __syncthreads();
    for (int kc = 0; kc < nk; ++kc) {
      if (kc + 1 < nk) load(kc + 1, g, true);
      compute(kc);
      if (kc + 1 < nk) park(kc + 1, g);
      __syncthreads();
    }
  }
  *reinterpret_cast<f4*>(csb + (0 * kBS + wrow) * kBT + 4 * wq) = sx;
  *reinterpret_cast<f4*>(csb + (1 * kBS + wrow) * kBT + 4 * wq) = sy;
  __syncthreads();
  const int tl = 16 * wave + fn, t = t0 + tl;
  float cx = 0.0f, cy = 0.0f;
#pragma unroll
  for (int r8 = 0; r8 < kBS; ++r8) { cx += csb[(0 * kBS + r8) * kBT + tl]; cy += csb[(1 * kBS + r8) * kBT + tl]; }
  const bool tok = t < T;
  float R = 0.0f;
  if (uvec && tok) {
    R = -as * (cx + cy) / amdot[(size_t)b * T + t];
    if (by == 0 && fk == 0) Rout[(size_t)b * T + t] = R;
  }
  const float* aprow = am_probs + ((size_t)b * T + (tok ? t : 0)) * C;
#pragma unroll
  for (int g = 0; g < NG; ++g)
#pragma unroll
    for (int j = 0; j < 4; ++j) {
      const int c = c0 + 64 * g + 16 * fk + 4 * j;
      f4 ap = {0.f, 0.f, 0.f, 0.f};
      if (tok && c < C) ap = *reinterpret_cast<const f4*>(aprow + c);
      if (uvec) {
        f4 uv = {0.f, 0.f, 0.f, 0.f};
        if (c < C) uv = *reinterpret_cast<const f4*>(uvec + c);
#pragma unroll
        for (int e = 0; e < 4; ++e) acc[4 * g + e][j] = ap[e] * (acc[4 * g + e][j] + uv[e] * R);
      } else {
#pragma unroll
        for (int e = 0; e < 4; ++e) acc[4 * g + e][j] = ap[e] * acc[4 * g + e][j];
      }
    }
  {
    constexpr int kB2 = CT / 2;
    static_assert(kB2 * kBT <= 2 * kBS * LDC && kB2 <= 2 * kBS * kBLT, "pass 2 reuses the tiles of pass 1");
    float* xT = lmT;
    int* sym2 = reinterpret_cast<int*>(wT);
    constexpr int kCap = (2 * kBS * kBLT - kB2) * 2;
    unsigned short* rlist = reinterpret_cast<unsigned short*>(wT + kB2);
    int* wcnt = reinterpret_cast<int*>(csb);
    int count = 0;
    const bool listed = S <= 65535;
    __syncthreads();
    if (listed) {
      for (int base = 0; base < S; base += 256) {
        const int srow = base + tid;
        const int sy = srow < S ? min(max(symbols[(size_t)b * S + srow], 0), C - 1) : -1;
        const bool mine = sy >= c0 && sy < c0 + CT;
        const unsigned long long m = __ballot(mine);
        if (lane == 0) wcnt[wave] = __popcll(m);
        __syncthreads();
        int off = count;
        for (int w = 0; w < wave; ++w) off += wcnt[w];
        const int tot = wcnt[0] + wcnt[1] + wcnt[2] + wcnt[3];
        const int at = off + __popcll(m & ((1ull << lane) - 1ull));
        if (mine && at < kCap) rlist[at] = (unsigned short)srow;
        count += tot;
        __syncthreads();
      }
    }
    const bool all_rows = !listed || count > kCap;
    if (all_rows) count = S;
    auto row_of = [&](int i) { return all_rows ? i : (int)rlist[i]; };
    constexpr int NX = kB2 * (kBT / 4) / 256;
    for (int r0 = 0; r0 < count; r0 += kB2) {
      f4 xv[NX];
#pragma unroll
      for (int u = 0; u < NX; ++u) {
        const int row = row_of(min(r0 + wrow + 16 * u, count - 1));
        xv[u] = *reinterpret_cast<const f4u*>(gxb + (size_t)row * T1 + wtc);
      }
      const int li = r0 + tid;
      const int symr = (tid < kB2 && li < count) ? min(max(symbols[(size_t)b * S + row_of(li)], 0), C - 1) : -1;
      __syncthreads();
#pragma unroll
      for (int u = 0; u < NX; ++u) {
        const float rowx = (r0 + wrow + 16 * u < count) ? kdir : 0.0f;
        *reinterpret_cast<f4*>(xT + (wrow + 16 * u) * kBT + 4 * wq) = xv[u] * xmask * rowx;
      }
      if (tid < kB2) sym2[tid] = symr;
      __syncthreads();
      const int nks = (min(kB2, count - r0) + 3) / 4;
      for (int kk = 0; kk < nks; ++kk) {
        const float bx = xT[(4 * kk + fk) * kBT + 16 * wave + fn];
        const int lc = sym2[4 * kk + fk] - c0;
        const int myblk = (lc >= 0 && lc < CT && ((lc & 63) >> 2) == fn) ? 4 * (lc >> 6) + (lc & 3) : -1;
        unsigned mask = 0;
#pragma unroll
        for (int q = 0; q < 4; ++q) {
          const int sb = __builtin_amdgcn_readfirstlane(sym2[4 * kk + q]) - c0;
          if (sb >= 0 && sb < CT) mask |= 1u << (4 * (sb >> 6) + (sb & 3));
        }
#pragma unroll
        for (int i = 0; i < NCB; ++i)
          if (mask & (1u << i)) acc[i] = __builtin_amdgcn_mfma_f32_16x16x4f32((myblk == i) ? 1.0f : 0.0f, bx, acc[i], 0, 0, 0);
      }
    }
  }
  if (!tok) return;
  float* drow = d_am + ((size_t)b * T + t) * C;
  const float colb = kdir * cy;
#pragma unroll
  for (int g = 0; g < NG; ++g)
#pragma unroll
    for (int j = 0; j < 4; ++j) {
      const int c = c0 + 64 * g + 16 * fk + 4 * j;
      if (c >= C) continue;
      f4 v = {acc[4 * g + 0][j], acc[4 * g + 1][j], acc[4 * g + 2][j], acc[4 * g + 3][j]};
      if (blank >= c && blank < c + 4) v[blank - c] += colb;
      *reinterpret_cast<f4*>(drow + c) = v;
    }
}

}

int simple_fused_supported(int C) { return (C % 4 == 0) ? 1 : 0; }

int simple_fused_fwd(const float* am, const float* lm, const int32_t* symbols, const float* am_probs,
                     const float* lm_probs, const float* am_max, const float* lm_max, const int32_t* boundary, int blank,
                     double delay_penalty, const float* lmonly_norm, const float* amonly_norm, const float* ulog, float cs,
                     float ls, float as, float* px, float* py, float* prod_out, int B, int T, int S, int C, int modified,
                     hipStream_t st) {
  if (!simple_fused_supported(C)) { set_error("simple_logprobs_fused_fwd: C = %d is not a multiple of 4", C); return FTR_ERR_UNSUPPORTED; }
  const int T1 = modified ? T : T + 1;
  const int blocks = (S + 1 + 15) / 16;
  const int ny = (blocks + 12) / 13;
  const int need = (blocks + ny - 1) / ny;
  int ns = need <= 4 ? 4 : need <= 7 ? 7 : need <= 10 ? 10 : 13;
  {
    const size_t ftiles = (size_t)((T1 + 63) / 64) * B;
    while (ns > 4 && ftiles * ((blocks + ns - 1) / ns) < 512) ns -= 3;
  }
  if (const char* e = getenv("FTR_FUSED_NS")) { const int v = atoi(e); if (v == 4 || v == 7 || v == 10 || v == 13) ns = v; }
  int mb = ((size_t)16 * ns * C * sizeof(float) > 512 * 1024 && T1 > 64) ? 2 : 1;
  if (const char* e = getenv("FTR_FUSED_FT")) { const int v = atoi(e); if (v == 64) mb = 1; else if (v == 128) mb = 2; }
  const dim3 grid((T1 + 64 * mb - 1) / (64 * mb), (blocks + ns - 1) / ns, B);
  if (grid.z > 65535) { set_error("simple_logprobs_fused_fwd: B = %d > 65535", B); return FTR_ERR_UNSUPPORTED; }
  const bool smooth = lmonly_norm != nullptr;
  return dispatch(modified != 0, [&](auto mod) {
    return dispatch(smooth, [&](auto sm) {
      return dispatch_among<4, 7, 10, 13>(ns, [&](auto nsv) {
        return dispatch_among<2, 1>(mb, [&](auto mbv) {
          constexpr auto kernel = simple_fused_fwd_kernel<decltype(mod)::value, decltype(sm)::value, decltype(nsv)::value, decltype(mbv)::value>;
          constexpr size_t lds = fused_lds_bytes<decltype(nsv)::value, decltype(mbv)::value>();
          const int rc = reserve_lds<kernel>(lds, "simple_logprobs_fused_fwd");
          if (rc != FTR_OK) return rc;
          hipLaunchKernelGGL(kernel, grid, dim3(256), lds, st, am, lm, symbols, am_probs, lm_probs, am_max, lm_max, boundary, blank,
                             delay_penalty, lmonly_norm, amonly_norm, ulog, cs, ls, as, px, py, prod_out, T, S, C);
          return check_launch("simple_logprobs_fused_fwd");
        });
      });
    });
  });
}

int simple_fused_bwd_supported(int T, int C) {
  return (simple_fused_supported(C) && C >= 4 && T >= 4 && (T % 4) == 0) ? 1 : 0;
}

int simple_fused_bwd_columns(int B, int T, int C) {
  if (const char* e = getenv("FTR_FUSED_BWD_CT")) { const int v = atoi(e); if (v == 128 || v == 256) return v; }
  const long long slots_cu = current_device_cus(), ft = (long long)((T + kBT - 1) / kBT) * B;
  auto cost = [&](int ncb, int wgs) {
    const long long tiles = ft * ((C + 16 * ncb - 1) / (16 * ncb)), slots = slots_cu * wgs;
    return ((tiles + slots - 1) / slots) * wgs * ncb;
  };
  return cost(8, 4) <= cost(16, 3) ? 128 : 256;
}

template <bool USEW>
static int fused_bwd_am_launch(const char* what, int ncb, const float* gpx, const float* gpy, Scale scale, const float* prod_or_w,
                               const float* lm_probs, const float* am_probs, const int32_t* symbols, const int32_t* boundary,
                               int blank, float cs, float kdir, const float* uvec, const float* amdot, float as, float* Rout,
                               float* d_am, int B, int T, int S, int C, int modified, hipStream_t st) {
  if (!simple_fused_bwd_supported(T, C)) {
    set_error("%s: T = %d, C = %d is outside the fused kernel's domain (T %% 4 == 0, C %% 4 == 0)", what, T, C);
    return FTR_ERR_UNSUPPORTED;
  }
  const dim3 grid((T + kBT - 1) / kBT, (C + 16 * ncb - 1) / (16 * ncb), B);
  if (grid.z > 65535) { set_error("%s: B = %d > 65535", what, B); return FTR_ERR_UNSUPPORTED; }
  dispatch(modified != 0, [&](auto mod) {
    dispatch_among<8, kBCB>(ncb, [&](auto nb) {
      constexpr int NCB = USEW ? decltype(nb)::value : kBCB;
      hipLaunchKernelGGL((simple_fused_bwd_am_kernel<decltype(mod)::value, USEW, NCB>), grid, dim3(256), fused_bwd_lds_bytes<NCB>(), st, gpx, gpy, scale, prod_or_w, lm_probs, am_probs, symbols, boundary, blank, cs, kdir, uvec, amdot, as, Rout, d_am, T, S, C);
    });
  });
  return check_launch(what);
}

int simple_fused_bwd_am(const float* gpx, const float* gpy, Scale scale, const float* prod, const float* lm_probs,
                        const float* am_probs, const int32_t* symbols, const int32_t* boundary, int blank, float cs,
                        float kdir, const float* uvec, const float* amdot, float as, float* Rout, float* d_am, int B,
                        int T, int S, int C, int modified, hipStream_t st) {
  return fused_bwd_am_launch<false>("simple_logprobs_fused_bwd_am", kBCB, gpx, gpy, scale, prod, lm_probs, am_probs, symbols, boundary, blank, cs, kdir, uvec, amdot, as, Rout, d_am, B, T, S, C, modified, st);
}

int simple_fused_bwd_am_w(const float* gpx, const float* gpy, Scale scale, const float* W, const float* lm_probs,
                          const float* am_probs, const int32_t* symbols, const int32_t* boundary, int blank, float kdir,
                          const float* uvec, const float* amdot, float as, float* Rout, float* d_am, int B, int T, int S,
                          int C, int modified, hipStream_t st) {
  const int ncb = simple_fused_bwd_columns(B, T, C) / 16;
  return fused_bwd_am_launch<true>("simple_logprobs_fused_bwd_am_w", ncb, gpx, gpy, scale, W, lm_probs, am_probs, symbols, boundary, blank, 1.0f, kdir, uvec, amdot, as, Rout, d_am, B, T, S, C, modified, st);
}

}
```

### tf-fast-rnnt_amd/csrc/simple_logprobs.hip

```cpp
#include "ftr_common.h"
#include "launch.h"

namespace ftr {
namespace {

constexpr float kTiny = 1.401298464324817e-45f;
constexpr int kTTnarrowAbove = 300;
constexpr int kTTwide = 32;
constexpr int kTTnarrow = 16;

__device__ __forceinline__ float wave_max(float v) { return wave_max_dpp(v); }
__device__ __forceinline__ float wave_sum(float v) { return wave_sum_dpp(v); }

template <bool VEC>
__device__ __forceinline__ void rowmax_exp_row(const float* __restrict__ x, float* __restrict__ probs,
                                               float* __restrict__ rowmax, float* __restrict__ rowsum,
                                               const float* __restrict__ dotvec, float* __restrict__ dot, size_t row, int C, int lane) {
  const float* xr = x + row * C;
  float* pr = probs + row * C;
  float m = -INFINITY;
  float sum = 0.0f, dsum = 0.0f;
  if (VEC) {
    const f4u* x4 = reinterpret_cast<const f4u*>(xr);
    f4u* p4 = reinterpret_cast<f4u*>(pr);
    const f4u* d4 = reinterpret_cast<const f4u*>(dotvec);
    const int n4 = C >> 2;
    for (int i = lane; i < n4; i += 64) { const f4 v = x4[i]; m = fmaxf(fmaxf(m, fmaxf(v[0], v[1])), fmaxf(v[2], v[3])); }
    m = wave_max(m);
    for (int i = lane; i < n4; i += 64) {
      const f4 v = x4[i];
      f4 o;
#pragma unroll
      for (int e = 0; e < 4; ++e) { o[e] = expf(v[e] - m); sum += o[e]; }
      if (dotvec) { const f4 dv = d4[i]; dsum += (o[0] * dv[0] + o[1] * dv[1]) + (o[2] * dv[2] + o[3] * dv[3]); }
      p4[i] = o;
    }
  } else {
    for (int i = lane; i < C; i += 64) m = fmaxf(m, xr[i]);
    m = wave_max(m);
    for (int i = lane; i < C; i += 64) { const float o = expf(xr[i] - m); pr[i] = o; sum += o; if (dotvec) dsum += o * dotvec[i]; }
  }
  if (rowsum) { sum = wave_sum(sum); if (lane == 0) rowsum[row] = sum; }
  if (dotvec) { dsum = wave_sum(dsum); if (lane == 0) dot[row] = dsum; }
  if (lane == 0) rowmax[row] = m;
}

template <bool VEC>
__global__ void rowmax_exp_kernel(const float* __restrict__ x, float* __restrict__ probs,
                                  float* __restrict__ rowmax, float* __restrict__ rowsum,
                                  const float* __restrict__ dotvec, float* __restrict__ dot, size_t rows, int C) {
  const int lane = threadIdx.x & 63;
  const size_t row = (size_t)blockIdx.x * (blockDim.x >> 6) + (threadIdx.x >> 6);
  if (row >= rows) return;
  rowmax_exp_row<VEC>(x, probs, rowmax, rowsum, dotvec, dot, row, C, lane);
}

template <bool VEC>
__global__ void rowmax_exp_pair_kernel(const float* __restrict__ x1, float* __restrict__ probs1, float* __restrict__ rowmax1, size_t rows1,
                                       const float* __restrict__ x2, float* __restrict__ probs2, float* __restrict__ rowmax2, size_t rows2, int C) {
  const int lane = threadIdx.x & 63;
  const size_t row = (size_t)blockIdx.x * (blockDim.x >> 6) + (threadIdx.x >> 6);
  if (row < rows1) rowmax_exp_row<VEC>(x1, probs1, rowmax1, nullptr, nullptr, nullptr, row, C, lane);
  else if (row - rows1 < rows2) rowmax_exp_row<VEC>(x2, probs2, rowmax2, nullptr, nullptr, nullptr, row - rows1, C, lane);
}

template <bool VEC>
__global__ void rowdot_kernel(const float* __restrict__ x, const float* __restrict__ v, float* __restrict__ dot, size_t rows, int C) {
  const int lane = threadIdx.x & 63;
  const size_t row = (size_t)blockIdx.x * (blockDim.x >> 6) + (threadIdx.x >> 6);
  if (row >= rows) return;
  const float* xr = x + row * C;
  float acc = 0.0f;
  if (VEC) {
    const f4u* x4 = reinterpret_cast<const f4u*>(xr);
    const f4u* v4 = reinterpret_cast<const f4u*>(v);
    for (int i = lane; i < (C >> 2); i += 64) { const f4 a = x4[i], b = v4[i]; acc += (a[0] * b[0] + a[1] * b[1]) + (a[2] * b[2] + a[3] * b[3]); }
  } else {
    for (int i = lane; i < C; i += 64) acc += xr[i] * v[i];
  }
  acc = wave_sum(acc);
  if (lane == 0) dot[row] = acc;
}

constexpr int kColsumSlab = 64;
template <bool VEC>
__global__ __launch_bounds__(256) void colsum_partial_kernel(const float* __restrict__ x, const float* __restrict__ w,
                                                             float* __restrict__ partial, size_t rows, int C) {
  const size_t r0 = (size_t)blockIdx.x * kColsumSlab;
  const size_t r1 = r0 + kColsumSlab < rows ? r0 + kColsumSlab : rows;
  if (VEC) {
    const int c = (blockIdx.y * 256 + threadIdx.x) * 4;
    if (c >= C) return;
    f4 acc = {0.f, 0.f, 0.f, 0.f};
    size_t r = r0;
    for (; r + 16 <= r1; r += 16) {
      f4 v[16]; float ww[16];
#pragma unroll
      for (int u = 0; u < 16; ++u) { v[u] = *reinterpret_cast<const f4u*>(x + (r + u) * C + c); ww[u] = w[r + u]; }
#pragma unroll
      for (int u = 0; u < 16; ++u) acc += v[u] * ww[u];
    }
    for (; r < r1; ++r) acc += *reinterpret_cast<const f4u*>(x + r * C + c) * w[r];
    *reinterpret_cast<f4u*>(partial + (size_t)blockIdx.x * C + c) = acc;
  } else {
    const int c = blockIdx.y * 256 + threadIdx.x;
    if (c >= C) return;
    float acc = 0.0f;
    for (size_t r = r0; r < r1; ++r) acc += x[r * C + c] * w[r];
    partial[(size_t)blockIdx.x * C + c] = acc;
  }
}
__global__ __launch_bounds__(256) void colsum_final_kernel(const float* __restrict__ partial, float* __restrict__ out, int nslab, int C) {
  __shared__ float part[4][64];
  const int cl = threadIdx.x & 63, gq = threadIdx.x >> 6;
  const int c = blockIdx.x * 64 + cl;
  const int per = (nslab + 3) / 4;
  const int i0 = gq * per, i1 = min(i0 + per, nslab);
  float a0 = 0.0f, a1 = 0.0f, a2 = 0.0f, a3 = 0.0f;
  if (c < C) {
    int i = i0;
    for (; i + 4 <= i1; i += 4) {
      a0 += partial[(size_t)i * C + c]; a1 += partial[(size_t)(i + 1) * C + c];
      a2 += partial[(size_t)(i + 2) * C + c]; a3 += partial[(size_t)(i + 3) * C + c];
    }
    for (; i < i1; ++i) a0 += partial[(size_t)i * C + c];
  }
  part[gq][cl] = (a0 + a1) + (a2 + a3);
  __syncthreads();
  if (gq == 0 && c < C) out[c] = (part[0][cl] + part[1][cl]) + (part[2][cl] + part[3][cl]);
}

template <bool MOD, int TT>
__global__ void simple_fwd_kernel(const float* __restrict__ am, const float* __restrict__ lm,
                                  const int32_t* __restrict__ symbols, const float* __restrict__ prod,
                                  const float* __restrict__ am_max, const float* __restrict__ lm_max,
                                  const int32_t* __restrict__ boundary, int blank, double delay_penalty,
                                  const float* __restrict__ lmonly_norm, const float* __restrict__ amonly_norm,
                                  const float* __restrict__ ulog, float cs, float ls, float as,
                                  float* __restrict__ px, float* __restrict__ py, int T, int S, int C) {
  extern __shared__ float tile[];
  const int b = blockIdx.y;
  const int t0 = blockIdx.x * TT;
  const int T1 = MOD ? T : T + 1;
  const int ld = C + 1;
  const float* amb = am + (size_t)b * T * C;
  {
    const int half = threadIdx.x >> 7, cl = threadIdx.x & 127;
    if ((C & 3) == 0) {
      const int n4 = C >> 2;
      for (int tt = half; tt < TT; tt += 2) {
        const bool ok = t0 + tt < T;
        const f4u* src = reinterpret_cast<const f4u*>(amb + (size_t)(t0 + tt) * C);
        for (int c4 = cl; c4 < n4; c4 += 128) {
          f4 v = {0.f, 0.f, 0.f, 0.f};
          if (ok) v = src[c4];
          float* dst = tile + tt * ld + 4 * c4;
          dst[0] = v[0]; dst[1] = v[1]; dst[2] = v[2]; dst[3] = v[3];
        }
      }
    } else {
      for (int tt = half; tt < TT; tt += 2)
        for (int c = cl; c < C; c += 128)
          tile[tt * ld + c] = (t0 + tt < T) ? amb[(size_t)(t0 + tt) * C + c] : 0.0f;
    }
  }
  const float* lmb = lm + (size_t)b * (S + 1) * C;
  const bool smooth = lmonly_norm != nullptr;
  float* rs_lmsym = tile + TT * ld;
  float* rs_lmblank = rs_lmsym + (S + 1);
  float* rs_lmmax = rs_lmblank + (S + 1);
  float* rs_lon = rs_lmmax + (S + 1);
  float* rs_ulog = rs_lon + (S + 1);
  int* rs_sym = reinterpret_cast<int*>(rs_ulog + (S + 1));
  for (int s = threadIdx.x; s <= S; s += blockDim.x) {
    const int sym = (s < S) ? min(max(symbols[(size_t)b * S + s], 0), C - 1) : blank;
    rs_sym[s] = sym;
    rs_lmsym[s] = lmb[(size_t)s * C + sym];
    rs_lmblank[s] = lmb[(size_t)s * C + blank];
    rs_lmmax[s] = lm_max[(size_t)b * (S + 1) + s];
    rs_lon[s] = smooth ? lmonly_norm[(size_t)b * (S + 1) + s] : 0.0f;
    rs_ulog[s] = smooth ? ulog[sym] : 0.0f;
  }
  __syncthreads();
  const int tx = threadIdx.x & (TT - 1);
  constexpr int NY = 256 / TT;
  const int ty = threadIdx.x / TT;
  const int t = t0 + tx;
  const int te = boundary ? boundary[4 * b + 3] : T;
  const float amx = (t < T) ? am_max[(size_t)b * T + t] : 0.0f;
  const float am_blank = tile[tx * ld + blank];
  float pen = 0.0f;
  if (delay_penalty > 0.0) pen = (float)((((double)te - 1.0) / 2.0 - (double)t) * delay_penalty);
  const float aon = (smooth && t < T) ? amonly_norm[(size_t)b * T + t] : 0.0f;
  const float ulog_blank = smooth ? ulog[blank] : 0.0f;
  const float* prodb = prod + (size_t)b * (S + 1) * T + t;
#pragma unroll 4
  for (int s = ty; s <= S; s += NY) {
    float nrm = 0.0f;
    const float lon = rs_lon[s];
    if (t < T) {
      nrm = logf(prodb[(size_t)s * T] + kTiny) + rs_lmmax[s] + amx;
      const float lmv = rs_lmblank[s];
      float v = am_blank + lmv - nrm;
      if (smooth) v = v * cs + (lmv - lon) * ls + (am_blank + ulog_blank - aon) * as;
      py[((size_t)b * (S + 1) + s) * T + t] = v;
    }
    if (s < S && t < T1) {
      float v = -INFINITY;
      if (t < T && (MOD || t != te)) {
        const float amv = tile[tx * ld + rs_sym[s]], lmv = rs_lmsym[s];
        v = amv + lmv - nrm;
        if (smooth) v = v * cs + (lmv - lon) * ls + (amv + rs_ulog[s] - aon) * as;
      }
      if (delay_penalty > 0.0) v += pen;
      px[((size_t)b * S + s) * T1 + t] = v;
    }
  }
}

template <bool MOD>
__global__ __launch_bounds__(256) void simple_bwd_w_kernel(const float* __restrict__ gpx, const float* __restrict__ gpy,
                                                           const Scale scale, const float* __restrict__ prod,
                                                           const int32_t* __restrict__ boundary, float* __restrict__ W,
                                                           float* __restrict__ rsx, float* __restrict__ rsy, float cs,
                                                           int T, int S, int B) {
  const int lane = threadIdx.x & 63;
  const size_t rowid = (size_t)blockIdx.x * 4 + (threadIdx.x >> 6);
  if (rowid >= (size_t)B * (S + 1)) return;
  const int b = (int)(rowid / (S + 1));
  const int s = (int)(rowid - (size_t)b * (S + 1));
  const int T1 = MOD ? T : T + 1;
  const int te = boundary ? boundary[4 * b + 3] : T;
  const size_t rowy = rowid * T;
  const size_t rowx = ((size_t)b * S + s) * T1;
  const float sc = scale.at(b);
  const bool hasx = s < S;
  float sx = 0.0f, sy = 0.0f;
  const int n4 = T >> 2;
  for (int q = lane; q < n4; q += 64) {
    const int t = 4 * q;
    f4 gx = {0.f, 0.f, 0.f, 0.f};
    if (hasx) gx = *reinterpret_cast<const f4u*>(gpx + rowx + t);
    const f4 gy = *reinterpret_cast<const f4u*>(gpy + rowy + t);
    const f4 pr = *reinterpret_cast<const f4u*>(prod + rowy + t);
    f4 w;
#pragma unroll
    for (int e = 0; e < 4; ++e) {
      float x = gx[e] * sc;
      if (!MOD && t + e == te) x = 0.0f;
      const float y = gy[e] * sc;
      sx += x; sy += y;
      w[e] = -cs * (x + y) / (pr[e] + kTiny);
    }
    *reinterpret_cast<f4u*>(W + rowy + t) = w;
  }
  for (int t = 4 * n4 + lane; t < T; t += 64) {
    float x = 0.0f;
    if (hasx && (MOD || t != te)) x = gpx[rowx + t] * sc;
    const float y = gpy[rowy + t] * sc;
    sx += x; sy += y;
    W[rowy + t] = -cs * (x + y) / (prod[rowy + t] + kTiny);
  }
  sx = wave_sum(sx); sy = wave_sum(sy);
  if (lane == 0) { rsx[rowid] = sx; rsy[rowid] = sy; }
}

constexpr int kBwdAmPF = 1;
constexpr int kBwdAmWGs = 4;
template <bool MOD, int TT>
__global__ __launch_bounds__(256, kBwdAmWGs) void simple_bwd_am_kernel(const float* __restrict__ gpx, const float* __restrict__ gpy, const Scale scale,
                                     const float* __restrict__ damp, const float* __restrict__ am_probs,
                                     const int32_t* __restrict__ symbols, const int32_t* __restrict__ boundary,
                                     int blank, float kdir, const float* __restrict__ uvec,
                                     const float* __restrict__ amdot, float as, float* __restrict__ Rout,
                                     float* __restrict__ d_am, int T, int S, int C) {
  extern __shared__ float acc[];
  int tile = blockIdx.x, b = blockIdx.y;
  if (TT == 16) {
    const unsigned total = gridDim.x * gridDim.y;
    const unsigned lin = blockIdx.x + gridDim.x * blockIdx.y;
    if ((lin | 15u) < total) {
      const unsigned nl = (lin & ~15u) + 2 * (lin & 7u) + ((lin >> 3) & 1u);
      tile = (int)(nl % gridDim.x); b = (int)(nl / gridDim.x);
    }
  }
  const int t0 = tile * TT;
  const int T1 = MOD ? T : T + 1;
  const int ld = C + 1;
  constexpr int NF = TT / 2, PF = NF < kBwdAmPF ? NF : kBwdAmPF;
  const int wo_half = threadIdx.x >> 7, wo_cl = threadIdx.x & 127;
  f4 pdp[PF > 0 ? PF : 1], pap[PF > 0 ? PF : 1];
  if ((C & 3) == 0) {
    const int c4 = min(wo_cl, (C >> 2) - 1);
#pragma unroll
    for (int k = 0; k < PF; ++k) {
      const size_t o = ((size_t)b * T + min(t0 + wo_half + 2 * k, T - 1)) * C;
      pdp[k] = reinterpret_cast<const f4u*>(damp + o)[c4];
      pap[k] = reinterpret_cast<const f4u*>(am_probs + o)[c4];
    }
  }
  float* csy = acc + TT * ld;
  constexpr int NY = 256 / TT;
  float* csx = csy + NY * TT;
  for (int i = threadIdx.x; i < TT * ld; i += blockDim.x) acc[i] = 0.0f;
  __syncthreads();
  const int tx = threadIdx.x & (TT - 1);
  const int ty = threadIdx.x / TT;
  const int t = t0 + tx;
  const int te = boundary ? boundary[4 * b + 3] : T;
  const bool tok = t < T;
  const bool xok = tok && (MOD || t != te);
  const int32_t* symb = symbols + (size_t)b * S;
  auto symc = [&](int si) { return min(max(symb[si], 0), C - 1); };
  unsigned short* slist = reinterpret_cast<unsigned short*>(csx + NY * TT) + (size_t)ty * S;
  int cnt = 0;
  {
    const int hshift = TT * (ty % (64 / TT));
    constexpr unsigned kRowMask = (TT == 32) ? 0xffffffffu : ((1u << (TT & 31)) - 1u);
    for (int s0 = 0; s0 < S; s0 += TT) {
      const int s = s0 + tx;
      const bool mine = s < S && (symc(s) & (NY - 1)) == ty;
      const unsigned m32 = (unsigned)(__ballot(mine) >> hshift) & kRowMask;
      if (mine) slist[cnt + __popc(m32 & ((1u << tx) - 1u))] = (unsigned short)s;
      cnt += __popc(m32);
    }
  }
  __syncthreads();
  float cs = 0.0f, cx = 0.0f;
  const float sc = scale.at(b);
  if (xok) {
    const float* gcol = gpx + (size_t)b * S * T1 + t;
    int i = 0;
    for (; i + 7 < cnt; i += 8) {
      int sr[8], cr[8];
      float g[8];
#pragma unroll
      for (int e = 0; e < 8; ++e) sr[e] = slist[i + e];
#pragma unroll
      for (int e = 0; e < 8; ++e) { g[e] = gcol[(size_t)sr[e] * T1]; cr[e] = symc(sr[e]); }
#pragma unroll
      for (int e = 0; e < 8; ++e) { const float ge = g[e] * sc; acc[tx * ld + cr[e]] += ge; cx += ge; }
    }
    for (; i + 3 < cnt; i += 4) {
      const int s_0 = slist[i], s_1 = slist[i + 1], s_2 = slist[i + 2], s_3 = slist[i + 3];
      const float g0 = gcol[(size_t)s_0 * T1] * sc, g1 = gcol[(size_t)s_1 * T1] * sc;
      const float g2 = gcol[(size_t)s_2 * T1] * sc, g3 = gcol[(size_t)s_3 * T1] * sc;
      acc[tx * ld + symc(s_0)] += g0; cx += g0;
      acc[tx * ld + symc(s_1)] += g1; cx += g1;
      acc[tx * ld + symc(s_2)] += g2; cx += g2;
      acc[tx * ld + symc(s_3)] += g3; cx += g3;
    }
    for (; i < cnt; ++i) {
      const int s_0 = slist[i];
      const float g0 = gcol[(size_t)s_0 * T1] * sc;
      acc[tx * ld + symc(s_0)] += g0; cx += g0;
    }
  }
  if (tok) {
    const float* ycol = gpy + (size_t)b * (S + 1) * T + t;
#pragma unroll 8
    for (int s = ty; s <= S; s += NY) cs += ycol[(size_t)s * T] * sc;
  }
  csy[ty * TT + tx] = cs;
  csx[ty * TT + tx] = cx;
  __syncthreads();
  if (threadIdx.x < TT) {
    float col = 0.0f, colx = 0.0f;
#pragma unroll
    for (int g = 0; g < NY; ++g) { col += csy[g * TT + threadIdx.x]; colx += csx[g * TT + threadIdx.x]; }
    csy[threadIdx.x] = col; csx[threadIdx.x] = colx;
  }
  __syncthreads();
  {
    const int half = wo_half, cl = wo_cl;
    const bool vec = (C & 3) == 0;
    const int n4 = C >> 2;
    auto frame_terms = [&](int tt, float& col, float& R) {
      const float colx = csx[tt];
      col = csy[tt];
      R = 0.0f;
      if (uvec) R = -as * (colx + col) / amdot[(size_t)b * T + t0 + tt];
      col *= kdir;
    };
    auto quad = [&](size_t o, int c4, const float* arow, f4 dp, f4 ap, float col, float R) {
      f4 v;
#pragma unroll
      for (int e = 0; e < 4; ++e) {
        v[e] = dp[e] * ap[e] + kdir * arow[4 * c4 + e];
        if (4 * c4 + e == blank) v[e] += col;
        if (uvec) v[e] += ap[e] * uvec[4 * c4 + e] * R;
      }
      reinterpret_cast<f4u*>(d_am + o)[c4] = v;
    };
    if (vec) {
#pragma unroll
      for (int k = 0; k < PF; ++k) {
        const int tt = half + 2 * k;
        if (t0 + tt >= T || cl >= n4) continue;
        float col, R;
        frame_terms(tt, col, R);
        quad(((size_t)b * T + t0 + tt) * C, cl, acc + tt * ld, pdp[k], pap[k], col, R);
      }
    }
    for (int tt = half; tt < TT; tt += 2) {
      if (t0 + tt >= T) continue;
      float col, R;
      frame_terms(tt, col, R);
      if (uvec && cl == 0) Rout[(size_t)b * T + t0 + tt] = R;
      const size_t o = ((size_t)b * T + t0 + tt) * C;
      const float* arow = acc + tt * ld;
      if (vec) {
        for (int c4 = (tt < 2 * PF ? cl + 128 : cl); c4 < n4; c4 += 128)
          quad(o, c4, arow, reinterpret_cast<const f4u*>(damp + o)[c4], reinterpret_cast<const f4u*>(am_probs + o)[c4], col, R);
      } else {
        for (int c = cl; c < C; c += 128) {
          float v = damp[o + c] * am_probs[o + c] + kdir * arow[c];
          if (c == blank) v += col;
          if (uvec) v += am_probs[o + c] * uvec[c] * R;
          d_am[o + c] = v;
        }
      }
    }
  }
}

__global__ void simple_bwd_lm_kernel(const float* __restrict__ dlmp, const float* __restrict__ lm_probs,
                                     const int32_t* __restrict__ symbols, const float* __restrict__ rsx,
                                     const float* __restrict__ rsy, int blank, float kdir,
                                     const float* __restrict__ arow, const float* __restrict__ invsum,
                                     const float* __restrict__ gu, float* __restrict__ d_lm, int S, int C,
                                     size_t total) {
  for (size_t i = (size_t)blockIdx.x * blockDim.x + threadIdx.x; i < total; i += (size_t)gridDim.x * blockDim.x) {
    const size_t row = i / C;
    const int c = (int)(i - row * C);
    const int s = (int)(row % (size_t)(S + 1));
    const size_t b = row / (size_t)(S + 1);
    float v = dlmp[i] * lm_probs[i];
    if (s < S && c == symbols[b * S + s]) v += kdir * rsx[row];
    if (c == blank) v += kdir * rsy[row];
    if (arow) v += lm_probs[i] * (arow[row] + gu[c] * invsum[row]);
    d_lm[i] = v;
  }
}

__global__ __launch_bounds__(256) void simple_bwd_lm_rows_kernel(const float* __restrict__ dlmp, const float* __restrict__ lm_probs,
                                                                 const int32_t* __restrict__ symbols, const float* __restrict__ rsx,
                                                                 const float* __restrict__ rsy, int blank, float kdir,
                                                                 const float* __restrict__ arow, const float* __restrict__ invsum,
                                                                 const float* __restrict__ gu, float* __restrict__ d_lm, int S, int C,
                                                                 size_t rows) {
  const int lane = threadIdx.x & 63;
  const size_t row = (size_t)blockIdx.x * 4 + (threadIdx.x >> 6);
  if (row >= rows) return;
  const int s = (int)(row % (size_t)(S + 1));
  const size_t b = row / (size_t)(S + 1);
  const int sym = s < S ? symbols[b * S + s] : -1;
  const float ax = kdir * rsx[row], ay = kdir * rsy[row];
  const float ar = arow ? arow[row] : 0.0f, is = arow ? invsum[row] : 0.0f;
  const int n4 = C >> 2;
  const f4u* dp4 = reinterpret_cast<const f4u*>(dlmp + row * C);
  const f4u* lp4 = reinterpret_cast<const f4u*>(lm_probs + row * C);
  f4u* o4 = reinterpret_cast<f4u*>(d_lm + row * C);
  for (int q = lane; q < n4; q += 64) {
    const f4 dp = dp4[q], lp = lp4[q];
    f4 g = {0.f, 0.f, 0.f, 0.f};
    if (arow) g = reinterpret_cast<const f4u*>(gu)[q];
    f4 v;
#pragma unroll
    for (int e = 0; e < 4; ++e) {
      const int c = 4 * q + e;
      float x = dp[e] * lp[e];
      if (c == sym) x += ax;
      if (c == blank) x += ay;
      if (arow) x += lp[e] * (ar + g[e] * is);
      v[e] = x;
    }
    o4[q] = v;
  }
}

}

int simple_rowmax_exp(const float* x, float* probs, float* rowmax, float* rowsum, const float* dotvec, float* dot,
                      size_t rows, int C, hipStream_t st) {
  if (rows == 0 || C == 0) return FTR_OK;
  const int wpb = 4;
  const unsigned blocks = (unsigned)((rows + wpb - 1) / wpb);
  dispatch((C & 3) == 0, [&](auto vec) {
    hipLaunchKernelGGL(rowmax_exp_kernel<decltype(vec)::value>, dim3(blocks), dim3(64 * wpb), 0, st, x, probs, rowmax, rowsum, dotvec, dot, rows, C);
  });
  return check_launch("rowmax_exp");
}

int simple_rowmax_exp_pair(const float* x1, float* probs1, float* rowmax1, size_t rows1, const float* x2, float* probs2, float* rowmax2,
                           size_t rows2, int C, hipStream_t st) {
  if (rows1 + rows2 == 0 || C == 0) return FTR_OK;
  const int wpb = 4;
  const unsigned blocks = (unsigned)((rows1 + rows2 + wpb - 1) / wpb);
  dispatch((C & 3) == 0, [&](auto vec) {
    hipLaunchKernelGGL(rowmax_exp_pair_kernel<decltype(vec)::value>, dim3(blocks), dim3(64 * wpb), 0, st, x1, probs1, rowmax1, rows1, x2, probs2, rowmax2, rows2, C);
  });
  return check_launch("rowmax_exp_pair");
}

int simple_rowdot(const float* x, const float* v, float* dot, size_t rows, int C, hipStream_t st) {
  if (rows == 0) return FTR_OK;
  const int wpb = 4;
  const unsigned blocks = (unsigned)((rows + wpb - 1) / wpb);
  dispatch((C & 3) == 0, [&](auto vec) {
    hipLaunchKernelGGL(rowdot_kernel<decltype(vec)::value>, dim3(blocks), dim3(64 * wpb), 0, st, x, v, dot, rows, C);
  });
  return check_launch("rowdot");
}

size_t simple_colsum_workspace_floats(size_t rows, int C) { return ((rows + kColsumSlab - 1) / kColsumSlab) * (size_t)C; }

int simple_colsum_weighted(const float* x, const float* w, float* out, float* ws, size_t ws_floats, size_t rows, int C,
                           hipStream_t st) {
  if (C == 0) return FTR_OK;
  const size_t nslab = (rows + kColsumSlab - 1) / kColsumSlab;
  if (ws_floats < nslab * (size_t)C) { set_error("colsum_weighted: workspace of %zu floats, %zu needed", ws_floats, nslab * (size_t)C); return FTR_ERR_INVALID_ARG; }
  if (nslab > 0x7fffffff) { set_error("colsum_weighted: too many rows"); return FTR_ERR_UNSUPPORTED; }
  if (nslab > 0) {
    dispatch((C & 3) == 0, [&](auto vec) {
      const int cols = decltype(vec)::value ? C / 4 : C;
      hipLaunchKernelGGL(colsum_partial_kernel<decltype(vec)::value>, dim3((unsigned)nslab, (cols + 255) / 256), dim3(256), 0, st, x, w, ws, rows, C);
    });
    int rc = check_launch("colsum_weighted (partial)");
    if (rc != FTR_OK) return rc;
  }
  hipLaunchKernelGGL(colsum_final_kernel, dim3((C + 63) / 64), dim3(256), 0, st, ws, out, (int)nslab, C);
  return check_launch("colsum_weighted (final)");
}

static int tile_lds_ok(size_t lds, const char* what) {
  if (lds > 160 * 1024) { set_error("%s: C too large for the LDS tile (%zu bytes)", what, lds); return FTR_ERR_UNSUPPORTED; }
  return FTR_OK;
}

int simple_logprobs_fwd(const float* am, const float* lm, const int32_t* symbols, const float* prod,
                        const float* am_max, const float* lm_max, const int32_t* boundary, int blank,
                        double delay_penalty, const float* lmonly_norm, const float* amonly_norm, const float* ulog,
                        float cs, float ls, float as, float* px, float* py, int B, int T, int S, int C, int modified,
                        hipStream_t st) {
  const int T1 = modified ? T : T + 1;
  const int TT = C > kTTnarrowAbove ? kTTnarrow : kTTwide;
  const size_t lds = sizeof(float) * ((size_t)TT * (C + 1) + 6 * (size_t)(S + 1));
  int rc = tile_lds_ok(lds, "simple_logprobs_fwd");
  if (rc != FTR_OK) return rc;
  const dim3 grid((T1 + TT - 1) / TT, B);
  return dispatch(modified != 0, [&](auto mod) {
    return dispatch_among<kTTnarrow, kTTwide>(TT, [&](auto tt) {
      constexpr auto kernel = simple_fwd_kernel<decltype(mod)::value, decltype(tt)::value>;
      const int rcl = reserve_lds<kernel>(lds, "simple_logprobs_fwd", LdsText::reserve_bytes_why);
      if (rcl != FTR_OK) return rcl;
      hipLaunchKernelGGL(kernel, grid, dim3(256), lds, st, am, lm, symbols, prod, am_max, lm_max,
                         boundary, blank, delay_penalty, lmonly_norm, amonly_norm, ulog, cs, ls, as, px, py, T, S, C);
      return check_launch("simple_logprobs_fwd");
    });
  });
}

int simple_logprobs_bwd_w(const float* gpx, const float* gpy, Scale scale, const float* prod, const int32_t* boundary,
                          float* W, float* rsx, float* rsy, float cs, int B, int T, int S, int modified, hipStream_t st) {
  const size_t rows = (size_t)B * (S + 1);
  const dim3 grid((unsigned)((rows + 3) / 4));
  dispatch(modified != 0, [&](auto mod) {
    hipLaunchKernelGGL(simple_bwd_w_kernel<decltype(mod)::value>, grid, dim3(256), 0, st, gpx, gpy, scale, prod, boundary, W, rsx, rsy, cs, T, S, B);
  });
  return check_launch("simple_logprobs_bwd_w");
}

int simple_logprobs_bwd_am(const float* gpx, const float* gpy, Scale scale, const float* damp, const float* am_probs,
                           const int32_t* symbols, const int32_t* boundary, int blank, float kdir, const float* uvec,
                           const float* amdot, float as, float* Rout, float* d_am, int B, int T, int S, int C,
                           int modified, hipStream_t st) {
  if (S > 65535) { set_error("simple_logprobs_bwd_am: S = %d > 65535 is not supported", S); return FTR_ERR_UNSUPPORTED; }
  const int TT = C > kTTnarrowAbove ? kTTnarrow : kTTwide;
  const size_t lds = sizeof(float) * ((size_t)TT * (C + 1) + 2 * 256) + sizeof(unsigned short) * (256 / TT) * (size_t)S;
  int rc = tile_lds_ok(lds, "simple_logprobs_bwd_am");
  if (rc != FTR_OK) return rc;
  const dim3 grid((T + TT - 1) / TT, B);
  return dispatch(modified != 0, [&](auto mod) {
    return dispatch_among<kTTnarrow, kTTwide>(TT, [&](auto tt) {
      constexpr auto kernel = simple_bwd_am_kernel<decltype(mod)::value, decltype(tt)::value>;
      const int rcl = reserve_lds<kernel>(lds, "simple_logprobs_bwd_am", LdsText::reserve_bytes_why);
      if (rcl != FTR_OK) return rcl;
      hipLaunchKernelGGL(kernel, grid, dim3(256), lds, st, gpx, gpy, scale, damp, am_probs,
                         symbols, boundary, blank, kdir, uvec, amdot, as, Rout, d_am, T, S, C);
      return check_launch("simple_logprobs_bwd_am");
    });
  });
}

int simple_logprobs_bwd_lm(const float* dlmp, const float* lm_probs, const int32_t* symbols, const float* rsx,
                           const float* rsy, int blank, float kdir, const float* arow, const float* invsum,
                           const float* gu, float* d_lm, int B, int S, int C, hipStream_t st) {
  const size_t total = (size_t)B * (S + 1) * C;
  if (total == 0) return FTR_OK;
  if ((C & 3) == 0) {
    const size_t rows = (size_t)B * (S + 1);
    hipLaunchKernelGGL(simple_bwd_lm_rows_kernel, dim3((unsigned)((rows + 3) / 4)), dim3(256), 0, st, dlmp, lm_probs, symbols, rsx, rsy,
                       blank, kdir, arow, invsum, gu, d_lm, S, C, rows);
    return check_launch("simple_logprobs_bwd_lm");
  }
  const size_t blocks = (total + 255) / 256;
  hipLaunchKernelGGL(simple_bwd_lm_kernel, dim3((unsigned)(blocks > 65535 * 16 ? 65535 * 16 : blocks)), dim3(256), 0, st,
                     dlmp, lm_probs, symbols, rsx, rsy, blank, kdir, arow, invsum, gu, d_lm, S, C, total);
  return check_launch("simple_logprobs_bwd_lm");
}

}
```

### tf-fast-rnnt_amd/tf_fast_rnnt/_lib.py

```python
from __future__ import annotations

import ctypes
import os

_HERE = os.path.dirname(os.path.abspath(__file__))
LIB_PATH = os.environ.get("FTR_LIB_PATH") or os.path.join(_HERE, "libftr_hip.so")
_lib = None

_c_fp = ctypes.c_void_p
_c_ip = ctypes.c_void_p
_c_st = ctypes.c_void_p
_c_hi = ctypes.POINTER(ctypes.c_int32)
_i = ctypes.c_int
_f = ctypes.c_float

_SIGNATURES = {
    "ftr_abi_version": (ctypes.c_int, []),
    "ftr_package_version": (ctypes.c_char_p, []),
    "ftr_last_error": (ctypes.c_char_p, []),
    "ftr_mutual_information_workspace_floats": (ctypes.c_size_t, [_i, _i, _i]),
    "ftr_mutual_information_handoff_floats": (ctypes.c_size_t, [_i, _i, _i]),
    "ftr_mutual_information_fwd_f32": (_i, [_c_fp, _c_fp, _c_ip, _c_fp, _c_fp, _i, _i, _i, _i, _c_st]),
    "ftr_mutual_information_bwd_f32": (_i, [_c_fp, _c_fp, _c_ip, _c_fp, _c_fp, _c_fp, _c_fp, _c_fp, _i, _i, _i, _i, _i, _c_st]),
    "ftr_mutual_information_fwd_ws_f32": (_i, [_c_fp, _c_fp, _c_ip, _c_fp, ctypes.c_size_t, _i, _c_fp, _i, _i, _i, _i, _c_st]),
    "ftr_mutual_information_bwd_ws_f32": (_i, [_c_fp, _c_fp, _c_ip, _c_fp, ctypes.c_size_t, _i, _c_fp, _c_fp, _c_fp, _c_fp, _i, _i, _i, _i, _i, _c_st]),
    "ftr_mutual_information_bwd_loss_ws_f32": (_i, [_c_fp, _c_fp, _c_ip, _c_fp, ctypes.c_size_t, _i, _c_fp, _c_fp, _c_fp, _i, _c_fp, _i, _i, _i, _i, _c_st]),
    "ftr_mutual_information_workspace_init": (_i, [_c_fp, ctypes.c_size_t, _i, _i, _i, _c_st]),
    "ftr_mutual_information_status": (_i, [_c_fp, ctypes.c_size_t, _i, _i, _i, ctypes.POINTER(ctypes.c_int), ctypes.POINTER(ctypes.c_longlong), _c_st]),
    "ftr_mutual_information_viterbi_workspace_bytes": (ctypes.c_size_t, [_i, _i, _i]),
    "ftr_mutual_information_viterbi_f32": (_i, [_c_fp, _c_fp, _c_ip, ctypes.c_void_p, ctypes.c_size_t, _c_fp, _c_ip, _i, _i, _i, _i, _c_st]),
    "ftr_cummin_i32": (_i, [_c_ip, _c_ip, _i, _i, _c_st]),
    "ftr_prune_ranges_i32": (_i, [_c_fp, _c_fp, _c_ip, _c_ip, _c_ip, _i, _i, _i, _i, _i, ctypes.POINTER(ctypes.c_int), _c_st]),
    "ftr_do_pruning_f32": (_i, [_c_fp, _c_fp, _c_ip, _c_fp, _c_fp, _i, _i, _i, _i, _i, _c_st]),
    "ftr_do_pruning_bwd_f32": (_i, [_c_fp, _c_fp, _c_ip, _c_fp, _c_fp, _i, _i, _i, _i, _i, _c_st]),
    "ftr_do_pruning_bwd_workspace_bytes": (ctypes.c_size_t, [_i, _i, _i, _i, _i]),
    "ftr_do_pruning_bwd_ws_f32": (_i, [_c_fp, _c_fp, _c_ip, _c_fp, _c_fp, _i, _i, _i, _i, _i, ctypes.c_void_p, ctypes.c_size_t, _c_st]),
    "ftr_pruned_logprobs_fwd_f32": (_i, [_c_fp, _c_ip, _c_ip, _c_ip, _i, ctypes.c_double, _c_fp, _c_fp, _c_fp, _i, _i, _i, _i, _i, _i, _c_st]),
    "ftr_pruned_logprobs_bwd_f32": (_i, [_c_fp, _c_ip, _c_ip, _c_ip, _i, _c_fp, _c_fp, _c_fp, _c_fp, _c_fp, _i, _i, _i, _i, _i, _i, _c_st]),
    "ftr_negated_reduce_f32": (_i, [_c_fp, _i, _i, _c_fp, _c_st]),
    "ftr_pruned_logprobs_bwd_scaled_f32": (_i, [_c_fp, _c_ip, _c_ip, _c_ip, _i, _c_fp, _c_fp, _c_fp, _c_fp, _i, _f, _c_fp, _i, _i, _i, _i, _i, _i, _c_st]),
    "ftr_simple_logprobs_bwd_w_scaled_f32": (_i, [_c_fp, _c_fp, _c_fp, _i, _f, _c_fp, _c_ip, _c_fp, _c_fp, _c_fp, _i, _i, _i, _i, _c_st]),
    "ftr_simple_logprobs_bwd_am_scaled_f32": (_i, [_c_fp, _c_fp, _c_fp, _i, _f, _c_fp, _c_fp, _c_ip, _c_ip, _i, _c_fp, _i, _i, _i, _i, _i, _c_st]),
    "ftr_rowmax_exp_f32": (_i, [_c_fp, _c_fp, _c_fp, ctypes.c_longlong, _i, _c_st]),
    "ftr_rowmax_exp_pair_f32": (_i, [_c_fp, _c_fp, _c_fp, ctypes.c_longlong, _c_fp, _c_fp, _c_fp, ctypes.c_longlong, _i, _c_st]),
    "ftr_rowmax_exp_sum_f32": (_i, [_c_fp, _c_fp, _c_fp, _c_fp, ctypes.c_longlong, _i, _c_st]),
    "ftr_smoothed_logprobs_fwd_f32": (_i, [_c_fp, _c_fp, _c_ip, _c_fp, _c_fp, _c_fp, _c_fp, _c_fp, _c_fp, _c_ip, _i, _f, _f, _f, _c_fp, _c_fp, _i, _i, _i, _i, _i, _c_st]),
    "ftr_smoothed_logprobs_bwd_w_f32": (_i, [_c_fp, _c_fp, _c_fp, _c_ip, _f, _c_fp, _c_fp, _c_fp, _i, _i, _i, _i, _c_st]),
    "ftr_smoothed_logprobs_bwd_am_f32": (_i, [_c_fp, _c_fp, _c_fp, _c_fp, _c_ip, _c_ip, _i, _f, _c_fp, _c_fp, _f, _c_fp, _c_fp, _i, _i, _i, _i, _i, _c_st]),
    "ftr_smoothed_logprobs_bwd_lm_f32": (_i, [_c_fp, _c_fp, _c_ip, _c_fp, _c_fp, _i, _f, _c_fp, _c_fp, _c_fp, _c_fp, _i, _i, _i, _c_st]),
    "ftr_smoothed_logprobs_fwd_pen_f32": (_i, [_c_fp, _c_fp, _c_ip, _c_fp, _c_fp, _c_fp, _c_fp, _c_fp, _c_fp, _c_ip, _i, ctypes.c_double, _f, _f, _f, _c_fp, _c_fp, _i, _i, _i, _i, _i, _c_st]),
    "ftr_smoothed_logprobs_bwd_w_scaled_f32": (_i, [_c_fp, _c_fp, _c_fp, _i, _f, _c_fp, _c_ip, _f, _c_fp, _c_fp, _c_fp, _i, _i, _i, _i, _c_st]),
    "ftr_smoothed_logprobs_bwd_am_scaled_f32": (_i, [_c_fp, _c_fp, _c_fp, _i, _f, _c_fp, _c_fp, _c_ip, _c_ip, _i, _f, _c_fp, _c_fp, _f, _c_fp, _c_fp, _i, _i, _i, _i, _i, _c_st]),
    "ftr_rowmax_exp_dot_f32": (_i, [_c_fp, _c_fp, _c_fp, _c_fp, _c_fp, ctypes.c_longlong, _i, _c_st]),
    "ftr_rowdot_f32": (_i, [_c_fp, _c_fp, _c_fp, ctypes.c_longlong, _i, _c_st]),
    "ftr_colsum_weighted_workspace_floats": (ctypes.c_size_t, [ctypes.c_longlong, _i]),
    "ftr_colsum_weighted_f32": (_i, [_c_fp, _c_fp, _c_fp, _c_fp, ctypes.c_size_t, ctypes.c_longlong, _i, _c_st]),
    "ftr_simple_logprobs_fused_supported": (_i, [_i]),
    "ftr_simple_logprobs_fused_bwd_supported": (_i, [_i, _i]),
    "ftr_normalizer_gemm_f32": (_i, [_i, _c_fp, _c_fp, _c_fp, _i, _i, _i, _i, _c_st]),
    "ftr_normalizer_gemm_set_choice": (_i, [_i, _i, _i, _i, _i, _i]),
    "ftr_normalizer_gemm_choice": (_i, [_i, _i, _i, _i, _i, ctypes.POINTER(ctypes.c_int), ctypes.POINTER(ctypes.c_float), ctypes.POINTER(ctypes.c_float), ctypes.POINTER(ctypes.c_int)]),
    "ftr_simple_logprobs_fused_fwd_f32": (_i, [_c_fp, _c_fp, _c_ip, _c_fp, _c_fp, _c_fp, _c_fp, _c_ip, _i, ctypes.c_double, _c_fp, _c_fp, _c_fp, _i, _i, _i, _i, _i, _c_st]),
    "ftr_smoothed_logprobs_fused_fwd_f32": (_i, [_c_fp, _c_fp, _c_ip, _c_fp, _c_fp, _c_fp, _c_fp, _c_fp, _c_fp, _c_fp, _c_ip, _i, ctypes.c_double, _f, _f, _f, _c_fp, _c_fp, _c_fp, _i, _i, _i, _i, _i, _c_st]),
    "ftr_simple_logprobs_fused_bwd_am_f32": (_i, [_c_fp, _c_fp, _c_fp, _i, _f, _c_fp, _c_fp, _c_fp, _c_ip, _c_ip, _i, _c_fp, _i, _i, _i, _i, _i, _c_st]),
    "ftr_smoothed_logprobs_fused_bwd_am_f32": (_i, [_c_fp, _c_fp, _c_fp, _i, _f, _c_fp, _c_fp, _c_fp, _c_ip, _c_ip, _i, _f, _f, _c_fp, _c_fp, _f, _c_fp, _c_fp, _i, _i, _i, _i, _i, _c_st]),
    "ftr_mutual_information_band_supported": (_i, [_i, _i, _i]),
    "ftr_band_ranges_check_i32": (_i, [_c_ip, _c_ip, _c_ip, _i, _i, _i, _c_st]),
    "ftr_pruned_band_fwd_f32": (_i, [_c_fp, _c_ip, _c_ip, _c_ip, _i, ctypes.c_double, _c_fp, _c_fp, _c_fp, _i, _i, _i, _i, _i, _i, _c_st]),
    "ftr_mutual_information_band_f32": (_i, [_c_fp, _c_fp, _c_ip, _c_ip, _c_fp, _c_fp, _c_fp, _i, _i, _i, _i, _i, _c_st]),
    "ftr_mutual_information_band_workspace_floats": (ctypes.c_size_t, [_i, _i, _i, _i]),
    "ftr_mutual_information_band_ws_f32": (_i, [_c_fp, _c_fp, _c_ip, _c_ip, _c_fp, ctypes.c_size_t, _c_fp, _c_fp, _c_fp, _i, _i, _i, _i, _i, _c_st]),
    "ftr_pruned_band_bwd_scaled_f32": (_i, [_c_fp, _c_ip, _c_ip, _c_ip, _i, _c_fp, _c_fp, _c_fp, _c_fp, _i, _f, _c_fp, _i, _i, _i, _i, _i, _i, _c_st]),
    "ftr_hat_pruned_logprobs_fwd_f32": (_i, [_c_fp, _c_ip, _c_ip, _c_ip, _i, ctypes.c_double, _c_fp, _c_fp, _c_fp, _i, _i, _i, _i, _i, _i, _c_st]),
    "ftr_hat_pruned_logprobs_bwd_scaled_f32": (_i, [_c_fp, _c_ip, _c_ip, _c_ip, _i, _c_fp, _c_fp, _c_fp, _c_fp, _i, _f, _c_fp, _i, _i, _i, _i, _i, _i, _c_st]),
    "ftr_hat_pruned_band_fwd_f32": (_i, [_c_fp, _c_ip, _c_ip, _c_ip, _i, ctypes.c_double, _c_fp, _c_fp, _c_fp, _i, _i, _i, _i, _i, _i, _c_st]),
    "ftr_hat_pruned_band_bwd_scaled_f32": (_i, [_c_fp, _c_ip, _c_ip, _c_ip, _i, _c_fp, _c_fp, _c_fp, _c_fp, _i, _f, _c_fp, _i, _i, _i, _i, _i, _i, _c_st]),
    "ftr_mutual_information_multiblank_workspace_floats": (ctypes.c_size_t, [_i, _i, _i]),
    "ftr_mutual_information_multiblank_fwd_f32": (_i, [_c_fp, _c_fp, _c_ip, _c_hi, _i, _c_fp, ctypes.c_size_t, _c_fp, _i, _i, _i, _c_st]),
    "ftr_mutual_information_multiblank_bwd_f32": (_i, [_c_fp, _c_fp, _c_ip, _c_hi, _i, _c_fp, ctypes.c_size_t, _c_fp, _c_fp, _c_fp, _i, _i, _i, _c_st]),
    "ftr_multiblank_pruned_logprobs_fwd_f32": (_i, [_c_fp, _c_ip, _c_ip, _c_ip, _i, _c_hi, _c_hi, _i, ctypes.c_double, ctypes.c_double, _c_fp, _c_fp, _c_fp, _i, _i, _i, _i, _i, _c_st]),
    "ftr_multiblank_pruned_logprobs_bwd_scaled_f32": (_i, [_c_fp, _c_ip, _c_ip, _c_ip, _i, _c_hi, _c_hi, _i, _c_fp, _c_fp, _c_fp, _c_fp, _i, _f, _c_fp, _i, _i, _i, _i, _i, _c_st]),
    "ftr_mutual_information_tdt_workspace_floats": (ctypes.c_size_t, [_i, _i, _i]),
    "ftr_mutual_information_tdt_fwd_f32": (_i, [_c_fp, _c_fp, _c_ip, _c_hi, _i, _c_hi, _i, _c_fp, ctypes.c_size_t, _c_fp, _i, _i, _i, _c_st]),
    "ftr_mutual_information_tdt_bwd_f32": (_i, [_c_fp, _c_fp, _c_ip, _c_hi, _i, _c_hi, _i, _c_fp, ctypes.c_size_t, _c_fp, _c_fp, _c_fp, _i, _i, _i, _c_st]),
    "ftr_mutual_information_viterbi_tdt_workspace_bytes": (ctypes.c_size_t, [_i, _i, _i]),
    "ftr_mutual_information_viterbi_tdt_f32": (_i, [_c_fp, _c_fp, _c_ip, _c_hi, _i, _c_hi, _i, ctypes.c_void_p, ctypes.c_size_t, _c_fp, _c_ip, _c_ip, _c_ip, _i, _i, _i, _c_st]),
    "ftr_tdt_pruned_logprobs_fwd_f32": (_i, [_c_fp, _c_ip, _c_ip, _c_ip, _i, _c_hi, _i, ctypes.c_double, ctypes.c_double, _c_fp, _c_fp, _c_fp, _c_fp, _i, _i, _i, _i, _i, _c_st]),
    "ftr_tdt_pruned_logprobs_bwd_scaled_f32": (_i, [_c_fp, _c_ip, _c_ip, _c_ip, _i, _c_hi, _i, ctypes.c_double, ctypes.c_double, _c_fp, _c_fp, _c_fp, _c_fp, _c_fp, _i, _f, _c_fp, _i, _i, _i, _i, _i, _c_st]),
    "ftr_simple_logprobs_fwd_f32": (_i, [_c_fp, _c_fp, _c_ip, _c_fp, _c_fp, _c_fp, _c_ip, _i, ctypes.c_double, _c_fp, _c_fp, _i, _i, _i, _i, _i, _c_st]),
    "ftr_simple_logprobs_bwd_w_f32": (_i, [_c_fp, _c_fp, _c_fp, _c_ip, _c_fp, _c_fp, _c_fp, _i, _i, _i, _i, _c_st]),
    "ftr_simple_logprobs_bwd_am_f32": (_i, [_c_fp, _c_fp, _c_fp, _c_fp, _c_ip, _c_ip, _i, _c_fp, _i, _i, _i, _i, _i, _c_st]),
    "ftr_simple_logprobs_bwd_lm_f32": (_i, [_c_fp, _c_fp, _c_ip, _c_fp, _c_fp, _i, _c_fp, _i, _i, _i, _c_st]),
    "ftr_selftest": (_i, [ctypes.c_void_p, _c_st]),
}
_LOWP_SIGNATURES = {
    "ftr_pruned_logprobs_fwd_dt": (_i, [_c_fp, _i, _c_ip, _c_ip, _c_ip, _i, ctypes.c_double, _c_fp, _c_fp, _c_fp, _i, _i, _i, _i, _i, _i, _i, _c_st]),
    "ftr_pruned_logprobs_bwd_scaled_dt": (_i, [_c_fp, _i, _c_ip, _c_ip, _c_ip, _i, _c_fp, _c_fp, _c_fp, _c_fp, _i, _f, _c_fp, _i, _i, _i, _i, _i, _i, _i, _c_st]),
    "ftr_pruned_band_fwd_dt": (_i, [_c_fp, _i, _c_ip, _c_ip, _c_ip, _i, ctypes.c_double, _c_fp, _c_fp, _c_fp, _i, _i, _i, _i, _i, _i, _i, _c_st]),
    "ftr_pruned_band_bwd_scaled_dt": (_i, [_c_fp, _i, _c_ip, _c_ip, _c_ip, _i, _c_fp, _c_fp, _c_fp, _c_fp, _i, _f, _c_fp, _i, _i, _i, _i, _i, _i, _i, _c_st]),
}
_PRUNE_SUM_SIGNATURES = {
    "ftr_do_pruning_sum_dt": (_i, [_c_fp, _c_fp, _i, _c_ip, _c_fp, _i, _i, _i, _i, _i, _c_st]),
    "ftr_do_pruning_sum_bwd_ws_dt": (_i, [_c_fp, _i, _c_ip, _c_fp, _c_fp, _i, _i, _i, _i, _i, ctypes.c_void_p, ctypes.c_size_t, _c_st]),
}
_JOINER_ACT_SIGNATURES = {
    "ftr_pruned_joiner_act_dt": (_i, [_c_fp, _c_fp, _i, _i, _c_ip, _c_fp, _i, _i, _i, _i, _i, _c_st]),
    "ftr_pruned_joiner_act_bwd_ws_dt": (_i, [_c_fp, _c_fp, _i, _i, _c_ip, _c_fp, _c_fp, _i, _i, _i, _i, _i, ctypes.c_void_p, ctypes.c_size_t, _c_st]),
}
_KD_SIGNATURES = {
    "ftr_pruned_kd_fwd_dt": (_i, [_c_fp, _i, _c_fp, _i, _c_ip, _c_ip, _c_ip, _i, _f, _i, _c_fp, _c_fp, _c_fp, _i, _i, _i, _i, _i, _c_st]),
    "ftr_pruned_kd_bwd_scaled_dt": (_i, [_c_fp, _i, _c_fp, _i, _c_ip, _c_ip, _c_ip, _i, _f, _i, _c_fp, _c_fp, _i, _f, _c_fp, _i, _i, _i, _i, _i, _c_st]),
    "ftr_pruned_kd_reduce_f32": (_i, [_c_fp, _i, _i, _c_fp, _c_st]),
}
_FUSED_SIGNATURES = {
    "ftr_simple_logprobs_fused_bwd_am_w_f32": (_i, [_c_fp, _c_fp, _c_fp, _i, _f, _c_fp, _c_fp, _c_fp, _c_ip, _c_ip, _i, _c_fp, _i, _i, _i, _i, _i, _c_st]),
    "ftr_smoothed_logprobs_fused_bwd_am_w_f32": (_i, [_c_fp, _c_fp, _c_fp, _i, _f, _c_fp, _c_fp, _c_fp, _c_ip, _c_ip, _i, _f, _c_fp, _c_fp, _f, _c_fp, _c_fp, _i, _i, _i, _i, _i, _c_st]),
    "ftr_simple_logprobs_fused_bwd_am_w_columns": (_i, [_i, _i, _i]),
}
_BAND_TDT_SIGNATURES = {
    "ftr_mutual_information_band_tdt_workspace_floats": (ctypes.c_size_t, [_i, _i, _i, _i, _i, _i]),
    "ftr_mutual_information_band_tdt_supported": (_i, [_i, _i, _i, _i, _i]),
    "ftr_mutual_information_band_tdt_f32": (_i, [_c_fp, _c_fp, _c_ip, _c_ip, _c_hi, _i, _c_hi, _i, _c_fp, ctypes.c_size_t, _c_fp, _c_fp, _c_fp, _i, _i, _i, _i, _c_st]),
    "ftr_tdt_pruned_band_fwd_f32": (_i, [_c_fp, _c_ip, _c_ip, _c_ip, _i, _c_hi, _i, ctypes.c_double, ctypes.c_double, _c_fp, _c_fp, _c_fp, _c_fp, _i, _i, _i, _i, _i, _c_st]),
    "ftr_tdt_pruned_band_bwd_scaled_f32": (_i, [_c_fp, _c_ip, _c_ip, _c_ip, _i, _c_hi, _i, ctypes.c_double, ctypes.c_double, _c_fp, _c_fp, _c_fp, _c_fp, _c_fp, _i, _f, _c_fp, _i, _i, _i, _i, _i, _c_st]),
}
_BAND_MULTIBLANK_SIGNATURES = {
    "ftr_mutual_information_band_multiblank_workspace_floats": (ctypes.c_size_t, [_i, _i, _i, _i, _i]),
    "ftr_mutual_information_band_multiblank_supported": (_i, [_i, _i, _i, _i]),
    "ftr_mutual_information_band_multiblank_f32": (_i, [_c_fp, _c_fp, _c_ip, _c_ip, _c_hi, _i, _c_fp, ctypes.c_size_t, _c_fp, _c_fp, _c_fp, _i, _i, _i, _i, _c_st]),
    "ftr_multiblank_pruned_band_fwd_f32": (_i, [_c_fp, _c_ip, _c_ip, _c_ip, _i, _c_hi, _c_hi, _i, ctypes.c_double, ctypes.c_double, _c_fp, _c_fp, _c_fp, _i, _i, _i, _i, _i, _c_st]),
    "ftr_multiblank_pruned_band_bwd_scaled_f32": (_i, [_c_fp, _c_ip, _c_ip, _c_ip, _i, _c_hi, _c_hi, _i, _c_fp, _c_fp, _c_fp, _c_fp, _i, _f, _c_fp, _i, _i, _i, _i, _i, _c_st]),
}
_BAND_VITERBI_SIGNATURES = {
    "ftr_mutual_information_band_viterbi_supported": (_i, [_i, _i, _i, _i, _i]),
    "ftr_mutual_information_band_viterbi_workspace_bytes": (ctypes.c_size_t, [_i, _i, _i, _i, _i, _i]),
    "ftr_mutual_information_band_viterbi_f32": (_i, [_c_fp, _c_fp, _c_ip, _c_ip, _c_hi, _i, _c_hi, _i, ctypes.c_void_p, ctypes.c_size_t, _c_fp, _c_ip, _c_ip, _c_ip, _i, _i, _i, _i, _c_st]),
}
EXPORTED_SYMBOLS = tuple(_SIGNATURES)
LOWP_SYMBOLS = tuple(_LOWP_SIGNATURES)
PRUNE_SUM_SYMBOLS = tuple(_PRUNE_SUM_SIGNATURES)
JOINER_ACT_SYMBOLS = tuple(_JOINER_ACT_SIGNATURES)
KD_SYMBOLS = tuple(_KD_SIGNATURES)
FUSED_SYMBOLS = tuple(_FUSED_SIGNATURES)
BAND_TDT_SYMBOLS = tuple(_BAND_TDT_SIGNATURES)
BAND_MULTIBLANK_SYMBOLS = tuple(_BAND_MULTIBLANK_SIGNATURES)
BAND_VITERBI_SYMBOLS = tuple(_BAND_VITERBI_SIGNATURES)
band_tdt_recursions = 0
band_multiblank_recursions = 0
FTR_KD_FULL, FTR_KD_COLLAPSED = 0, 1
FTR_MI_WS_CLEAN = 1
FTR_DTYPE_F32, FTR_DTYPE_BF16, FTR_DTYPE_FP16 = 0, 1, 2
FTR_ACT_TANH, FTR_ACT_RELU = 1, 2
FTR_PRUNED_HAT = 1


def lib() -> ctypes.CDLL:
    global _lib
    if _lib is None:
        if not os.path.exists(LIB_PATH):
            raise ImportError(
                f"{LIB_PATH} is missing: build the HIP extension first (python -c 'import __graft_entry__ as g; "
                "g.build()' or make -C tf-fast-rnnt_amd/csrc).  tf_fast_rnnt has no CPU fallback.")
        handle = ctypes.CDLL(LIB_PATH)
        for name, (restype, argtypes) in {**_SIGNATURES, **_LOWP_SIGNATURES, **_PRUNE_SUM_SIGNATURES, **_JOINER_ACT_SIGNATURES, **_KD_SIGNATURES, **_FUSED_SIGNATURES,
                                            **_BAND_TDT_SIGNATURES, **_BAND_MULTIBLANK_SIGNATURES, **_BAND_VITERBI_SIGNATURES}.items():
            fn = getattr(handle, name)
            fn.restype = restype
            fn.argtypes = argtypes
        _lib = handle
    return _lib


class FtrError(RuntimeError):
    """A native entry point returned an FTR_ERR_* code (the reference raises tf.errors.Internal,
    tf_fast_rnnt_op.cc:114-116)."""


def check(rc: int, what: str) -> None:
    if rc != 1:
        msg = lib().ftr_last_error().decode("utf-8", "replace")
        raise FtrError(f"{what} failed with code {rc}: {msg}")


_profile_hook = None


def set_profile_hook(hook) -> None:
    global _profile_hook
    _profile_hook = hook


def call(name: str, *args) -> None:
    fn = getattr(lib(), name)
    if _profile_hook is None:
        rc = fn(*args)
    else:
        with _profile_hook(name):
            rc = fn(*args)
    check(rc, name)
```

### tf-fast-rnnt_amd/tf_fast_rnnt/rnnt_loss.py

```python
from __future__ import annotations

from typing import Optional, Tuple, Union

import ctypes
import os
import weakref

import torch

from . import _lib
from .mutual_information import (_as_boundary, _ptr, _require_gpu, _stream_ptr, band_multiblank_forward_backward,
                                 band_multiblank_supported, band_tdt_forward_backward, band_tdt_supported, band_viterbi_supported, cummin, mb_forward_backward, mi_forward_backward,
                                 mutual_information_recursion, mutual_information_viterbi, mutual_information_viterbi_tdt, mutual_information_viterbi_tdt_band,
                                 tdt_forward_backward)

_NEG_INF = float("-inf")
_TINY = 1.401298464324817e-45


def tune_normalizer_gemms(enable: bool = True, filename: Optional[str] = None, search: bool = True, when: str = "second") -> None:
    if when not in ("first", "second"):
        raise ValueError("when must be 'first' or 'second'")
    os.environ["FTR_GEMM_TUNE"] = when if (enable and search) else "off"


def normalizer_gemm_choice(kind: int, B: int, T: int, S: int, C: int):
    sol, cand = ctypes.c_int(0), ctypes.c_int(0)
    us, usd = ctypes.c_float(0), ctypes.c_float(0)
    if not _lib.lib().ftr_normalizer_gemm_choice(int(kind), int(B), int(T), int(S) + 1, int(C), ctypes.byref(sol), ctypes.byref(us),
                                                  ctypes.byref(usd), ctypes.byref(cand)):
        return None
    return dict(solution=sol.value, us=us.value, us_default=usd.value, candidates=cand.value)


def set_normalizer_gemm_choice(kind: int, B: int, T: int, S: int, C: int, solution: int) -> None:
    _lib.call("ftr_normalizer_gemm_set_choice", int(kind), int(B), int(T), int(S) + 1, int(C), int(solution))


def _gemm(kind: int, x: torch.Tensor, y: torch.Tensor, B: int, T: int, S: int, C: int, st) -> torch.Tensor:
    shape = ((B, S + 1, T), (B, S + 1, C), (B, T, C))[kind]
    out = torch.empty(shape, dtype=torch.float32, device=x.device)
    _lib.call("ftr_normalizer_gemm_f32", kind, _ptr(x), _ptr(y), _ptr(out), B, T, S + 1, C, st)
    return out


def _check_type(rnnt_type: str) -> None:
    if rnnt_type not in ("regular", "modified", "constrained"):
        raise ValueError(f"rnnt_type should be ('regular' | 'modified' | 'constrained'), given {rnnt_type}")


def _i64(t: torch.Tensor) -> torch.Tensor:
    return t if t.dtype == torch.int64 else t.to(torch.int64)


def fix_for_boundary(px: torch.Tensor, boundary: Optional[torch.Tensor] = None) -> torch.Tensor:
    if boundary is None:
        return px
    B, S, T1 = px.shape
    idx = _i64(boundary[:, 3]).reshape(B, 1, 1).expand(B, S, 1)
    return px.scatter(2, idx, _NEG_INF)


def _use_fused_builder(C: int) -> bool:
    return os.environ.get("FTR_BUILDER_GEMM", "fused") != "library" and bool(_lib.lib().ftr_simple_logprobs_fused_supported(int(C)))


_FUSED_BWD_MEASURED = {
    (32, 512, 100, 500): True,
    (32, 1000, 200, 500): True,
    (32, 2000, 300, 1024): True,
    (8, 8000, 1000, 512): True,
    (16, 3000, 600, 768): True,
    (8, 1000, 200, 256): True,
}


def _use_fused_builder_bwd(T: int, C: int, B: int = 1) -> bool:
    mode = os.environ.get("FTR_BUILDER_BWD", "auto")
    if mode == "library" or not _use_fused_builder(C) or not _lib.lib().ftr_simple_logprobs_fused_bwd_supported(int(T), int(C)):
        return False
    return True


def _simple_builder(amc, lmc, symbols, am_probs, lm_probs, am_max, lm_max, boundary, blank, delay_penalty, px, py,
                    B, T, S, C, modified, st):
    if _use_fused_builder(C):
        prod = torch.empty((B, S + 1, T), dtype=torch.float32, device=amc.device)
        _lib.call("ftr_simple_logprobs_fused_fwd_f32", _ptr(amc), _ptr(lmc), _ptr(symbols), _ptr(am_probs), _ptr(lm_probs),
                  _ptr(am_max), _ptr(lm_max), _ptr(boundary), int(blank), float(delay_penalty), _ptr(px), _ptr(py),
                  _ptr(prod), B, T, S, C, int(modified), st)
        return prod
    prod = _gemm(0, lm_probs, am_probs, B, T, S, C, st)
    _lib.call("ftr_simple_logprobs_fwd_f32", _ptr(amc), _ptr(lmc), _ptr(symbols), _ptr(prod), _ptr(am_max),
              _ptr(lm_max), _ptr(boundary), int(blank), float(delay_penalty), _ptr(px), _ptr(py),
              B, T, S, C, int(modified), st)
    return prod


def _simple_forward(lm, am, symbols, termination_symbol, boundary, modified, delay_penalty):
    B, T, C = am.shape
    S = lm.shape[1] - 1
    T1 = T if modified else T + 1
    amc = am.detach().contiguous(); lmc = lm.detach().contiguous()
    dev = amc.device
    am_probs = torch.empty_like(amc); lm_probs = torch.empty_like(lmc)
    am_max = torch.empty((B, T), dtype=torch.float32, device=dev)
    lm_max = torch.empty((B, S + 1), dtype=torch.float32, device=dev)
    px = torch.empty((B, S, T1), dtype=torch.float32, device=dev)
    py = torch.empty((B, S + 1, T), dtype=torch.float32, device=dev)
    with torch.cuda.device(dev):
        st = _stream_ptr(amc)
        _lib.call("ftr_rowmax_exp_pair_f32", _ptr(amc), _ptr(am_probs), _ptr(am_max), B * T,
                  _ptr(lmc), _ptr(lm_probs), _ptr(lm_max), B * (S + 1), C, st)
        prod = _simple_builder(amc, lmc, symbols, am_probs, lm_probs, am_max, lm_max, boundary, termination_symbol,
                               delay_penalty, px, py, B, T, S, C, modified, st)
    return px, py, (am_probs, lm_probs, prod, symbols, boundary), (int(termination_symbol), int(modified))


def _simple_backward(saved, meta, gpx, gpy, scale=None, stride=0, mul=1.0):
    am_probs, lm_probs, prod, symbols, boundary = saved
    blank, modified = meta
    B, T, C = am_probs.shape
    S = lm_probs.shape[1] - 1
    dev = am_probs.device
    gpx = gpx.contiguous(); gpy = gpy.contiguous()
    W = torch.empty_like(prod)
    rsx = torch.empty((B, S + 1), dtype=torch.float32, device=dev)
    rsy = torch.empty((B, S + 1), dtype=torch.float32, device=dev)
    d_am = torch.empty_like(am_probs); d_lm = torch.empty_like(lm_probs)
    with torch.cuda.device(dev):
        st = _stream_ptr(am_probs)
        _lib.call("ftr_simple_logprobs_bwd_w_scaled_f32", _ptr(gpx), _ptr(gpy), _ptr(scale), stride, mul,
                  _ptr(prod), _ptr(boundary), _ptr(W), _ptr(rsx), _ptr(rsy), B, T, S, modified, st)
        dlmp = _gemm(1, W, am_probs, B, T, S, C, st)
        if _use_fused_builder_bwd(T, C, B):
            _lib.call("ftr_simple_logprobs_fused_bwd_am_w_f32", _ptr(gpx), _ptr(gpy), _ptr(scale), stride, mul,
                      _ptr(W), _ptr(lm_probs), _ptr(am_probs), _ptr(symbols), _ptr(boundary), blank, _ptr(d_am),
                      B, T, S, C, modified, st)
        else:
            damp = _gemm(2, W, lm_probs, B, T, S, C, st)
            _lib.call("ftr_simple_logprobs_bwd_am_scaled_f32", _ptr(gpx), _ptr(gpy), _ptr(scale), stride, mul,
                      _ptr(damp), _ptr(am_probs), _ptr(symbols), _ptr(boundary), blank, _ptr(d_am), B, T, S, C,
                      modified, st)
        _lib.call("ftr_simple_logprobs_bwd_lm_f32", _ptr(dlmp), _ptr(lm_probs), _ptr(symbols), _ptr(rsx), _ptr(rsy),
                  blank, _ptr(d_lm), B, S, C, st)
    return d_lm, d_am


class _SimpleLogprobs(torch.autograd.Function):

    @staticmethod
    def forward(ctx, lm, am, symbols, termination_symbol, boundary, modified, delay_penalty):
        px, py, saved, meta = _simple_forward(lm, am, symbols, termination_symbol, boundary, modified, delay_penalty)
        ctx.save_for_backward(*saved)
        ctx.meta = meta
        return px, py

    @staticmethod
    def backward(ctx, gpx, gpy):
        d_lm, d_am = _simple_backward(ctx.saved_tensors, ctx.meta, gpx, gpy)
        return d_lm, d_am, None, None, None, None, None


class _SimpleLoss(torch.autograd.Function):

    @staticmethod
    def forward(ctx, lm, am, symbols, termination_symbol, boundary, modified, delay_penalty, code, want_occupancies):
        px, py, saved, meta = _simple_forward(lm, am, symbols, termination_symbol, boundary, modified, delay_penalty)
        need = bool(want_occupancies) or ctx.needs_input_grad[0] or ctx.needs_input_grad[1]
        if need:
            ans, px_grad, py_grad, loss = mi_forward_backward(px, py, boundary, True, ans_grad_is_one=True, loss_code=code)
        else:
            ans, px_grad, py_grad = mi_forward_backward(px, py, boundary, False, ans_grad_is_one=True)
            loss = _negated_reduce_native(ans, code)
        shape_x, shape_y = px.shape, py.shape
        del px, py
        if need:
            ctx.save_for_backward(*saved, px_grad, py_grad)
        else:
            px_grad = torch.zeros(shape_x, dtype=torch.float32, device=loss.device)
            py_grad = torch.zeros(shape_y, dtype=torch.float32, device=loss.device)
        ctx.meta = meta
        ctx.code = int(code)
        ctx.mark_non_differentiable(px_grad, py_grad)
        ctx.set_materialize_grads(False)
        return loss, px_grad, py_grad

    @staticmethod
    def backward(ctx, g_loss, _g1, _g2):
        if g_loss is None:
            return (None,) * 9
        *saved, px_grad, py_grad = ctx.saved_tensors
        scale, stride, mul = _upstream_scale(g_loss, ctx.code, px_grad.shape[0])
        d_lm, d_am = _simple_backward(saved, ctx.meta, px_grad, py_grad, scale, stride, mul)
        return d_lm, d_am, None, None, None, None, None, None, None


def _check_simple_inputs(lm, am, symbols, termination_symbol):
    _require_gpu(am, "am"); _require_gpu(lm, "lm")
    if am.dtype != torch.float32 or lm.dtype != torch.float32:
        raise TypeError("am and lm must be float32")
    B, T, C = am.shape
    S = lm.shape[1] - 1
    if lm.shape[0] != B or lm.shape[2] != C:
        raise ValueError(f"lm {tuple(lm.shape)} and am {tuple(am.shape)} disagree")
    symbols = torch.as_tensor(symbols, device=am.device)
    if tuple(symbols.shape) != (B, S):
        raise ValueError(f"symbols must have shape {(B, S)}, got {tuple(symbols.shape)}")
    if not 0 <= int(termination_symbol) < C:
        raise ValueError(f"termination_symbol {termination_symbol} not in [0, {C})")
    return symbols.to(torch.int32).contiguous()


def _simple_logprobs_native(lm, am, symbols, termination_symbol, rnnt_type, boundary, delay_penalty=0.0):
    symbols = _check_simple_inputs(lm, am, symbols, termination_symbol)
    boundary = _as_boundary(boundary, am.shape[0], am.device)
    px, py = _SimpleLogprobs.apply(lm, am, symbols, termination_symbol, boundary, rnnt_type != "regular",
                                   _penalty(delay_penalty))
    if rnnt_type == "constrained":
        px = px + py[:, 1:, :]
    return px, py


def get_rnnt_logprobs(
    lm: torch.Tensor,
    am: torch.Tensor,
    symbols: torch.Tensor,
    termination_symbol: int,
    rnnt_type: str = "regular",
    boundary: Optional[torch.Tensor] = None,
) -> Tuple[torch.Tensor, torch.Tensor]:
    _check_type(rnnt_type)
    return _simple_logprobs_native(lm, am, symbols, termination_symbol, rnnt_type, boundary)


def _penalty(delay_penalty) -> float:
    return float(delay_penalty) if delay_penalty > 0.0 else 0.0


def _apply_delay_penalty(px, boundary, rnnt_type, delay_penalty):
    if not delay_penalty > 0.0:
        return px
    B, S, T0 = px.shape
    T = T0 if rnnt_type != "regular" else T0 - 1
    if boundary is None:
        offset = torch.full((B,), (T - 1) / 2, dtype=torch.float64, device=px.device)
    else:
        offset = (boundary[:, 3].to(torch.float64) - 1) / 2
    penalty = offset.reshape(B, 1, 1) - torch.arange(T0, dtype=torch.float64, device=px.device).reshape(1, 1, T0)
    penalty = penalty * delay_penalty
    return px + penalty.to(px.dtype)


_REDUCTIONS = {"none": 0, "mean": 1, "sum": 2}


def _reduction_code(reduction: Optional[str]) -> int:
    if reduction not in _REDUCTIONS:
        raise ValueError(f"reduction should be ('none' | 'mean' | 'sum'), given {reduction}")
    return _REDUCTIONS[reduction]


def _reduce(negated_loss: torch.Tensor, reduction: Optional[str]) -> torch.Tensor:
    code = _reduction_code(reduction)
    if code == 0:
        return -negated_loss
    return -torch.mean(negated_loss) if code == 1 else -torch.sum(negated_loss)


def _negated_reduce_native(ans: torch.Tensor, code: int) -> torch.Tensor:
    B = ans.shape[0]
    out = torch.empty((B,) if code == 0 else (), dtype=torch.float32, device=ans.device)
    with torch.cuda.device(ans.device):
        _lib.call("ftr_negated_reduce_f32", _ptr(ans), B, code, _ptr(out), _stream_ptr(ans))
    return out


def _upstream_scale(g_loss: torch.Tensor, code: int, B: int):
    g = g_loss.to(torch.float32).contiguous()
    return g, (1 if code == 0 else 0), (-1.0 / B if code == 1 else -1.0)


def _drive(px, py, boundary, reduction, calc_gradients):
    scores_and_grads = mutual_information_recursion(px=px, py=py, boundary=boundary, calc_gradients=calc_gradients)
    negated_loss = scores_and_grads[0] if calc_gradients else scores_and_grads
    loss = _reduce(negated_loss, reduction)
    return (loss, scores_and_grads[1]) if calc_gradients else loss


def rnnt_loss_simple(
# ... 985 lines not shown
    boundary: torch.Tensor = None,
    sigma: float = 0.0,
    rnnt_type: str = "regular",
    delay_penalty: float = 0.0,
    reduction: Optional[str] = "mean",
) -> torch.Tensor:
    if rnnt_type != "regular":
        raise ValueError(f"the TDT loss is defined for rnnt_type 'regular' only, given {rnnt_type}")
    code = _reduction_code(reduction)
    symbols_i, ranges_i, boundary_i = _pruned_inputs(logits, symbols, ranges, boundary)
    _tdt_args(durations, termination_symbol, logits.shape[3])
    return _TdtLoss.apply(logits, symbols_i, ranges_i, termination_symbol, tuple(durations), boundary_i, _check_sigma(sigma),
                          _penalty(delay_penalty), code)


def rnnt_loss_tdt(
    logits: torch.Tensor,
    symbols: torch.Tensor,
    termination_symbol: int,
    durations,
    boundary: Optional[torch.Tensor] = None,
    sigma: float = 0.0,
    rnnt_type: str = "regular",
    delay_penalty: float = 0.0,
    reduction: Optional[str] = "mean",
) -> torch.Tensor:
    if rnnt_type != "regular":
        raise ValueError(f"the TDT loss is defined for rnnt_type 'regular' only, given {rnnt_type}")
    ranges = _joint_inputs(logits, symbols)
    return rnnt_loss_tdt_pruned(logits=logits, symbols=symbols, ranges=ranges, termination_symbol=termination_symbol,
                                durations=durations, boundary=boundary, sigma=sigma, delay_penalty=delay_penalty,
                                reduction=reduction)



def rnnt_alignment_tdt_pruned(
    logits: torch.Tensor,
    symbols: torch.Tensor,
    ranges: torch.Tensor,
    termination_symbol: int,
    durations,
    boundary: Optional[torch.Tensor] = None,
    sigma: float = 0.0,
) -> Tuple[torch.Tensor, torch.Tensor, torch.Tensor, torch.Tensor]:
    with torch.no_grad():
        symbols, ranges, boundary = _pruned_inputs(logits, symbols, ranges, boundary)
        arr, durs, blank_durs, C = _tdt_args(durations, termination_symbol, logits.shape[3])
        x = logits.detach().contiguous()
        B, T, r, _ = x.shape
        S = symbols.shape[1]
        if _align_band_path_ok(ranges, boundary, T, S, r, len(durs), len(blank_durs)):
            _, _, pxb, pyb = _tdt_band_builder_fwd(x, symbols, ranges, boundary, int(termination_symbol), arr, durs, blank_durs, C,
                                                   _check_sigma(sigma), 0.0)
            return mutual_information_viterbi_tdt_band(pxb, pyb, ranges, durs, blank_durs, boundary, S=S)
        _, _, px, py = _tdt_builder_fwd(x, symbols, ranges, boundary, int(termination_symbol), arr, durs, blank_durs, C,
                                        _check_sigma(sigma), 0.0)
        return mutual_information_viterbi_tdt(px, py, durs, blank_durs, boundary)


def rnnt_alignment_multiblank_pruned(
    logits: torch.Tensor,
    symbols: torch.Tensor,
    ranges: torch.Tensor,
    termination_symbol: int,
    big_blanks,
    boundary: Optional[torch.Tensor] = None,
    sigma: float = 0.0,
) -> Tuple[torch.Tensor, torch.Tensor, torch.Tensor, torch.Tensor]:
    with torch.no_grad():
        symbols, ranges, boundary = _pruned_inputs(logits, symbols, ranges, boundary)
        x = logits.detach().contiguous()
        ids, durs, dt = _big_blank_args(tuple(map(tuple, big_blanks)), termination_symbol, x.shape[3])
        B, T, r, _ = x.shape
        S = symbols.shape[1]
        if _align_band_path_ok(ranges, boundary, T, S, r, 1, len(dt)):
            _, pxb, pyb = _mb_band_builder_fwd(x, symbols, ranges, boundary, int(termination_symbol), ids, durs, len(dt),
                                               _check_sigma(sigma), 0.0)
            return mutual_information_viterbi_tdt_band(pxb.unsqueeze(1), pyb, ranges, (0,), dt, boundary, S=S)
        _, px, py = _mb_builder_fwd(x, symbols, ranges, boundary, int(termination_symbol), ids, durs, len(dt),
                                    _check_sigma(sigma), 0.0)
        return mutual_information_viterbi_tdt(px.unsqueeze(1), py, (0,), dt, boundary)


def _colsum_weighted(x: torch.Tensor, w: torch.Tensor, rows: int, C: int, st) -> torch.Tensor:
    n = _lib.lib().ftr_colsum_weighted_workspace_floats(rows, C)
    ws = torch.empty((max(n, 1),), dtype=torch.float32, device=x.device)
    out = torch.empty((C,), dtype=torch.float32, device=x.device)
    _lib.call("ftr_colsum_weighted_f32", _ptr(x), _ptr(w), _ptr(out), _ptr(ws), n, rows, C, st)
    return out


def _smoothed_forward(lm, am, symbols, termination_symbol, boundary, modified, lm_only_scale, am_only_scale,
                      process_group, delay_penalty):
    B, T, C = am.shape
    S = lm.shape[1] - 1
    T1 = T if modified else T + 1
    cs = 1.0 - lm_only_scale - am_only_scale
    ls = lm_only_scale if lm_only_scale != 0.0 else 1.0e-20
    a_s = am_only_scale if am_only_scale != 0.0 else 1.0e-20
    amc = am.detach().contiguous(); lmc = lm.detach().contiguous()
    dev = amc.device
    am_probs = torch.empty_like(amc); lm_probs = torch.empty_like(lmc)
    am_max = torch.empty((B, T), dtype=torch.float32, device=dev)
    lm_max = torch.empty((B, S + 1), dtype=torch.float32, device=dev)
    lm_sum = torch.empty((B, S + 1), dtype=torch.float32, device=dev)
    px = torch.empty((B, S, T1), dtype=torch.float32, device=dev)
    py = torch.empty((B, S + 1, T), dtype=torch.float32, device=dev)
    with torch.cuda.device(dev):
        st = _stream_ptr(amc)
        _lib.call("ftr_rowmax_exp_sum_f32", _ptr(lmc), _ptr(lm_probs), _ptr(lm_max), _ptr(lm_sum),
                  B * (S + 1), C, st)
        inv = (1.0 / lm_sum).contiguous()
        ratio_sum = _colsum_weighted(lm_probs, inv, B * (S + 1), C, st)
        count = float(B * (S + 1))
        if process_group is not None:
            packed = torch.cat((ratio_sum, torch.full((1,), count, dtype=torch.float32, device=dev)))
            torch.distributed.all_reduce(packed, group=process_group)
            ratio_sum, count = packed[:C], packed[C]
        u = (ratio_sum / count + _TINY).contiguous()
        am_dot = torch.empty((B * T,), dtype=torch.float32, device=dev)
        _lib.call("ftr_rowmax_exp_dot_f32", _ptr(amc), _ptr(am_probs), _ptr(am_max), _ptr(u), _ptr(am_dot), B * T, C, st)
        fused = _use_fused_builder(C)
        prod = torch.empty((B, S + 1, T), dtype=torch.float32, device=dev) if fused else \
            _gemm(0, lm_probs, am_probs, B, T, S, C, st)
        amonly = (am_dot.log().reshape(B, T) + am_max).contiguous()
        ulog = u.log().contiguous()
        lmonly = (lm_sum.log() + lm_max).contiguous()
        if fused:
            _lib.call("ftr_smoothed_logprobs_fused_fwd_f32", _ptr(amc), _ptr(lmc), _ptr(symbols), _ptr(am_probs),
                      _ptr(lm_probs), _ptr(am_max), _ptr(lm_max), _ptr(lmonly), _ptr(amonly), _ptr(ulog), _ptr(boundary),
                      int(termination_symbol), float(delay_penalty), cs, ls, a_s, _ptr(px), _ptr(py), _ptr(prod),
                      B, T, S, C, int(modified), st)
        else:
            _lib.call("ftr_smoothed_logprobs_fwd_pen_f32", _ptr(amc), _ptr(lmc), _ptr(symbols), _ptr(prod), _ptr(am_max),
                      _ptr(lm_max), _ptr(lmonly), _ptr(amonly), _ptr(ulog), _ptr(boundary), int(termination_symbol),
                      float(delay_penalty), cs, ls, a_s, _ptr(px), _ptr(py), B, T, S, C, int(modified), st)
    saved = (am_probs, lm_probs, prod, symbols, boundary, inv, u, am_dot)
    meta = (int(termination_symbol), int(modified), cs, ls, a_s, count, process_group)
    return px, py, saved, meta


def _smoothed_backward(saved, meta, gpx, gpy, scale=None, stride=0, mul=1.0):
    am_probs, lm_probs, prod, symbols, boundary, inv, u, am_dot = saved
    blank, modified, cs, ls, a_s, count, group = meta
    B, T, C = am_probs.shape
    S = lm_probs.shape[1] - 1
    dev = am_probs.device
    gpx = gpx.contiguous(); gpy = gpy.contiguous()
    W = torch.empty_like(prod)
    rsx = torch.empty((B, S + 1), dtype=torch.float32, device=dev)
    rsy = torch.empty((B, S + 1), dtype=torch.float32, device=dev)
    R = torch.empty((B, T), dtype=torch.float32, device=dev)
    d_am = torch.empty_like(am_probs); d_lm = torch.empty_like(lm_probs)
    with torch.cuda.device(dev):
        st = _stream_ptr(am_probs)
        _lib.call("ftr_smoothed_logprobs_bwd_w_scaled_f32", _ptr(gpx), _ptr(gpy), _ptr(scale), stride, mul, _ptr(prod),
                  _ptr(boundary), cs, _ptr(W), _ptr(rsx), _ptr(rsy), B, T, S, modified, st)
        dlmp = _gemm(1, W, am_probs, B, T, S, C, st)
        if _use_fused_builder_bwd(T, C, B):
            _lib.call("ftr_smoothed_logprobs_fused_bwd_am_w_f32", _ptr(gpx), _ptr(gpy), _ptr(scale), stride, mul, _ptr(W),
                      _ptr(lm_probs), _ptr(am_probs), _ptr(symbols), _ptr(boundary), blank, cs + a_s, _ptr(u),
                      _ptr(am_dot), a_s, _ptr(R), _ptr(d_am), B, T, S, C, modified, st)
        else:
            damp = _gemm(2, W, lm_probs, B, T, S, C, st)
            _lib.call("ftr_smoothed_logprobs_bwd_am_scaled_f32", _ptr(gpx), _ptr(gpy), _ptr(scale), stride, mul, _ptr(damp),
                      _ptr(am_probs), _ptr(symbols), _ptr(boundary), blank, cs + a_s, _ptr(u), _ptr(am_dot), a_s, _ptr(R),
                      _ptr(d_am), B, T, S, C, modified, st)
        du = _colsum_weighted(am_probs, R, B * T, C, st)
        gul = torch.zeros((C,), dtype=torch.float32, device=dev)
        if S > 0:
            gul.index_add_(0, _i64(symbols).reshape(-1), rsx[:, :S].reshape(-1))
        gul[blank] += rsy.sum()
        du = du + a_s * gul / u
        if group is not None:
            torch.distributed.all_reduce(du, group=group)
        gu = (du / count).contiguous()
        dotq = torch.empty((B, S + 1), dtype=torch.float32, device=dev)
        _lib.call("ftr_rowdot_f32", _ptr(lm_probs), _ptr(gu), _ptr(dotq), B * (S + 1), C, st)
        dotq = dotq * inv
        arow = ((-ls) * (rsx + rsy) - dotq) * inv
        arow = arow.contiguous()
        _lib.call("ftr_smoothed_logprobs_bwd_lm_f32", _ptr(dlmp), _ptr(lm_probs), _ptr(symbols), _ptr(rsx),
                  _ptr(rsy), blank, cs + ls, _ptr(arow), _ptr(inv), _ptr(gu), _ptr(d_lm), B, S, C, st)
    return d_lm, d_am


class _SmoothedLogprobs(torch.autograd.Function):

    @staticmethod
    def forward(ctx, lm, am, symbols, termination_symbol, boundary, modified, lm_only_scale, am_only_scale,
                process_group):
        px, py, saved, meta = _smoothed_forward(lm, am, symbols, termination_symbol, boundary, modified, lm_only_scale,
                                                am_only_scale, process_group, 0.0)
        ctx.save_for_backward(*saved)
        ctx.meta = meta
        return px, py

    @staticmethod
    def backward(ctx, gpx, gpy):
        d_lm, d_am = _smoothed_backward(ctx.saved_tensors, ctx.meta, gpx, gpy)
        return d_lm, d_am, None, None, None, None, None, None, None


class _SmoothedLoss(torch.autograd.Function):

    @staticmethod
    def forward(ctx, lm, am, symbols, termination_symbol, boundary, modified, lm_only_scale, am_only_scale,
                process_group, delay_penalty, code, want_occupancies):
        px, py, saved, meta = _smoothed_forward(lm, am, symbols, termination_symbol, boundary, modified, lm_only_scale,
                                                am_only_scale, process_group, delay_penalty)
        need = bool(want_occupancies) or ctx.needs_input_grad[0] or ctx.needs_input_grad[1]
        if need:
            ans, px_grad, py_grad, loss = mi_forward_backward(px, py, boundary, True, ans_grad_is_one=True, loss_code=code)
        else:
            ans, px_grad, py_grad = mi_forward_backward(px, py, boundary, False, ans_grad_is_one=True)
            loss = _negated_reduce_native(ans, code)
        if need:
            ctx.save_for_backward(*saved, px_grad, py_grad)
        else:
            px_grad = torch.zeros_like(px); py_grad = torch.zeros_like(py)
        del px, py
        ctx.meta = meta
        ctx.code = int(code)
        ctx.mark_non_differentiable(px_grad, py_grad)
        ctx.set_materialize_grads(False)
        return loss, px_grad, py_grad

    @staticmethod
    def backward(ctx, g_loss, _g1, _g2):
        if g_loss is None:
            return (None,) * 12
        *saved, px_grad, py_grad = ctx.saved_tensors
        scale, stride, mul = _upstream_scale(g_loss, ctx.code, px_grad.shape[0])
        d_lm, d_am = _smoothed_backward(saved, ctx.meta, px_grad, py_grad, scale, stride, mul)
        return d_lm, d_am, None, None, None, None, None, None, None, None, None, None


def get_rnnt_logprobs_smoothed(
    lm: torch.Tensor,
    am: torch.Tensor,
    symbols: torch.Tensor,
    termination_symbol: int,
    lm_only_scale: float = 0.1,
    am_only_scale: float = 0.1,
    boundary: Optional[torch.Tensor] = None,
    rnnt_type: str = "regular",
    process_group=None,
) -> Tuple[torch.Tensor, torch.Tensor]:
    _check_type(rnnt_type)
    symbols = _check_simple_inputs(lm, am, symbols, termination_symbol)
    boundary = _as_boundary(boundary, am.shape[0], am.device)
    px, py = _SmoothedLogprobs.apply(lm, am, symbols, termination_symbol, boundary, rnnt_type != "regular",
                                     float(lm_only_scale), float(am_only_scale), process_group)
    if rnnt_type == "constrained":
        px = px + py[:, 1:, :]
    return px, py


def rnnt_loss_smoothed(
    lm: torch.Tensor,
    am: torch.Tensor,
    symbols: torch.Tensor,
    termination_symbol: int,
    lm_only_scale: float = 0.1,
    am_only_scale: float = 0.1,
    boundary: Optional[torch.Tensor] = None,
    rnnt_type: str = "regular",
    delay_penalty: float = 0.0,
    reduction: Optional[str] = "mean",
    calc_gradients: bool = False,
    process_group=None,
) -> Union[Tuple[torch.Tensor, Tuple[torch.Tensor, torch.Tensor]], torch.Tensor]:
    _check_type(rnnt_type)
    code = _reduction_code(reduction)
    boundary = _as_boundary(boundary, am.shape[0], am.device)
    if rnnt_type == "constrained":
        px, py = get_rnnt_logprobs_smoothed(lm=lm, am=am, symbols=symbols, termination_symbol=termination_symbol,
                                            lm_only_scale=lm_only_scale, am_only_scale=am_only_scale,
                                            boundary=boundary, rnnt_type=rnnt_type, process_group=process_group)
        px = _apply_delay_penalty(px, boundary, rnnt_type, delay_penalty)
        return _drive(px, py, boundary, reduction, calc_gradients)
    symbols_i = _check_simple_inputs(lm, am, symbols, termination_symbol)
    loss, px_grad, py_grad = _SmoothedLoss.apply(lm, am, symbols_i, termination_symbol, boundary, rnnt_type != "regular",
                                                 float(lm_only_scale), float(am_only_scale), process_group,
                                                 _penalty(delay_penalty), code, bool(calc_gradients))
    return (loss, (px_grad, py_grad)) if calc_gradients else loss
```

Measured before the change: 24700 utterances/s.

## Skip zero-gradient S-blocks in fused backward am kernel using per-row live ranges

The bwd_w kernel now records, for each (b,s) row, the range of t where the gradient weights are nonzero, and writes it into scratch space borrowed from d_lm. The fused backward-am kernel reduces these ranges per T-tile to find the span of live S-blocks and limits its K loop and symbol-list pass to that span, skipping blocks whose W is all zero. This targets the band structure of the simple-loss gradient, which is often concentrated near the alignment path. It adds an extra block reduction and two syncs per tile, reuses d_lm memory before it is written, and changes the launch-bounds occupancy hint for larger NCB.

```diff
diff --git a/include/ftr_live.h b/include/ftr_live.h
--- /dev/null
+++ b/include/ftr_live.h
@@ -0,0 +1,32 @@
+#ifndef FTR_LIVE_H_
+#define FTR_LIVE_H_
+#include "ftr_fused.h"
+
+#ifdef __cplusplus
+extern "C" {
+#endif
+
+int ftr_simple_logprobs_bwd_w_live_f32(const float* gpx, const float* gpy, const float* scale, int scale_stride,
+                                       float scale_mul, const float* prod, const int32_t* boundary, float* W, float* rsx,
+                                       float* rsy, int32_t* live, int B, int T, int S, int modified, void* stream);
+int ftr_smoothed_logprobs_bwd_w_live_f32(const float* gpx, const float* gpy, const float* scale, int scale_stride,
+                                         float scale_mul, const float* prod, const int32_t* boundary, float combined_scale,
+                                         float* W, float* rsx, float* rsy, int32_t* live, int B, int T, int S, int modified,
+                                         void* stream);
+
+int ftr_simple_logprobs_fused_bwd_am_live_f32(const float* gpx, const float* gpy, const float* scale, int scale_stride,
+                                              float scale_mul, const float* W, const int32_t* live, const float* lm_probs,
+                                              const float* am_probs, const int32_t* symbols, const int32_t* boundary,
+                                              int termination_symbol, float* d_am, int B, int T, int S, int C, int modified,
+                                              void* stream);
+int ftr_smoothed_logprobs_fused_bwd_am_live_f32(const float* gpx, const float* gpy, const float* scale, int scale_stride,
+                                                float scale_mul, const float* W, const int32_t* live, const float* lm_probs,
+                                                const float* am_probs, const int32_t* symbols, const int32_t* boundary,
+                                                int termination_symbol, float direct_scale, const float* unigram,
+                                                const float* am_dot, float am_only_scale, float* R, float* d_am, int B, int T,
+                                                int S, int C, int modified, void* stream);
+
+#ifdef __cplusplus
+}
+#endif
+#endif
diff --git a/tf-fast-rnnt_amd/csrc/capi.hip b/tf-fast-rnnt_amd/csrc/capi.hip
--- a/tf-fast-rnnt_amd/csrc/capi.hip
+++ b/tf-fast-rnnt_amd/csrc/capi.hip
@@ -510,13 +510,14 @@
 
 static int bwd_w_entry(const char* what, const float* gpx, const float* gpy, const float* scale, int scale_stride,
                        float scale_mul, const float* prod, const int32_t* boundary, float combined_scale, float* W,
-                       float* rsx, float* rsy, int B, int T, int S, int modified, void* stream) {
+                       float* rsx, float* rsy, int B, int T, int S, int modified, void* stream, int32_t* live = nullptr,
+                       bool want_live = false) {
   clear_error();
   FTR_TRY(check_sizes(what, B >= 0 && T >= 1 && S >= 0));
   FTR_TRY(check_scale_stride(what, scale_stride));
   if (B == 0) return FTR_OK;
-  FTR_TRY(pointers_then_device(what, gpy && prod && W && rsx && rsy && (gpx || S == 0)));
-  return simple_logprobs_bwd_w(gpx, gpy, Scale{scale, scale_stride, scale_mul}, prod, boundary, W, rsx, rsy, combined_scale, B, T, S, modified, stream_of(stream));
+  FTR_TRY(pointers_then_device(what, gpy && prod && W && rsx && rsy && (gpx || S == 0) && (live || !want_live)));
+  return simple_logprobs_bwd_w(gpx, gpy, Scale{scale, scale_stride, scale_mul}, prod, boundary, W, rsx, rsy, combined_scale, B, T, S, modified, stream_of(stream), live);
 }
 
 int ftr_simple_logprobs_bwd_w_f32(const float* gpx, const float* gpy, const float* prod, const int32_t* boundary,
@@ -739,13 +740,13 @@
                                 const float* am_probs, const int32_t* symbols, const int32_t* boundary,
                                 int termination_symbol, float direct_scale, const float* unigram, const float* am_dot,
                                 float am_only_scale, float* R, float* d_am, int B, int T, int S, int C, int modified,
-                                void* stream) {
+                                void* stream, const int32_t* live = nullptr, bool want_live = false) {
   clear_error();
   FTR_TRY(check_builder(what, B >= 0 && T >= 1 && S >= 0 && C >= 1, termination_symbol, C, true));
   FTR_TRY(check_scale_stride(what, scale_stride));
   if (B == 0) return FTR_OK;
-  FTR_TRY(pointers_then_device(what, gpy && W && lm_probs && am_probs && d_am && (!smoothed || (unigram && am_dot && R)) && (gpx || S == 0) && (symbols || S == 0)));
-  return simple_fused_bwd_am_w(gpx, gpy, Scale{scale, scale_stride, scale_mul}, W, lm_probs, am_probs, symbols, boundary, termination_symbol, direct_scale, unigram, am_dot, am_only_scale, R, d_am, B, T, S, C, modified, stream_of(stream));
+  FTR_TRY(pointers_then_device(what, gpy && W && lm_probs && am_probs && d_am && (!smoothed || (unigram && am_dot && R)) && (gpx || S == 0) && (symbols || S == 0) && (live || !want_live)));
+  return simple_fused_bwd_am_w(gpx, gpy, Scale{scale, scale_stride, scale_mul}, W, lm_probs, am_probs, symbols, boundary, termination_symbol, direct_scale, unigram, am_dot, am_only_scale, R, d_am, B, T, S, C, modified, stream_of(stream), live);
 }
 
 int ftr_simple_logprobs_fused_bwd_am_w_f32(const float* gpx, const float* gpy, const float* scale, int scale_stride,
@@ -765,6 +766,36 @@
 }
 
 int ftr_simple_logprobs_fused_bwd_am_w_columns(int B, int T, int C) { return simple_fused_bwd_columns(B, T, C); }
+
+int ftr_simple_logprobs_bwd_w_live_f32(const float* gpx, const float* gpy, const float* scale, int scale_stride,
+                                       float scale_mul, const float* prod, const int32_t* boundary, float* W, float* rsx,
+                                       float* rsy, int32_t* live, int B, int T, int S, int modified, void* stream) {
+  return bwd_w_entry("simple_logprobs_bwd_w_live", gpx, gpy, scale, scale_stride, scale_mul, prod, boundary, 1.0f, W, rsx, rsy, B, T, S, modified, stream, live, true);
+}
+
+int ftr_smoothed_logprobs_bwd_w_live_f32(const float* gpx, const float* gpy, const float* scale, int scale_stride,
+                                         float scale_mul, const float* prod, const int32_t* boundary, float combined_scale,
+                                         float* W, float* rsx, float* rsy, int32_t* live, int B, int T, int S, int modified,
+                                         void* stream) {
+  return bwd_w_entry("smoothed_logprobs_bwd_w_live", gpx, gpy, scale, scale_stride, scale_mul, prod, boundary, combined_scale, W, rsx, rsy, B, T, S, modified, stream, live, true);
+}
+
+int ftr_simple_logprobs_fused_bwd_am_live_f32(const float* gpx, const float* gpy, const float* scale, int scale_stride,
+                                              float scale_mul, const float* W, const int32_t* live, const float* lm_probs,
+                                              const float* am_probs, const int32_t* symbols, const int32_t* boundary,
+                                              int termination_symbol, float* d_am, int B, int T, int S, int C, int modified,
+                                              void* stream) {
+  return fused_bwd_am_w_entry("simple_logprobs_fused_bwd_am_live", false, gpx, gpy, scale, scale_stride, scale_mul, W, lm_probs, am_probs, symbols, boundary, termination_symbol, 1.0f, nullptr, nullptr, 0.0f, nullptr, d_am, B, T, S, C, modified, stream, live, true);
+}
+
+int ftr_smoothed_logprobs_fused_bwd_am_live_f32(const float* gpx, const float* gpy, const float* scale, int scale_stride,
+                                                float scale_mul, const float* W, const int32_t* live, const float* lm_probs,
+                                                const float* am_probs, const int32_t* symbols, const int32_t* boundary,
+                                                int termination_symbol, float direct_scale, const float* unigram,
+                                                const float* am_dot, float am_only_scale, float* R, float* d_am, int B, int T,
+                                                int S, int C, int modified, void* stream) {
+  return fused_bwd_am_w_entry("smoothed_logprobs_fused_bwd_am_live", true, gpx, gpy, scale, scale_stride, scale_mul, W, lm_probs, am_probs, symbols, boundary, termination_symbol, direct_scale, unigram, am_dot, am_only_scale, R, d_am, B, T, S, C, modified, stream, live, true);
+}
 
 int ftr_mutual_information_band_supported(int T, int S, int r) { return mi_band_supported(T, S, r); }
 
diff --git a/tf-fast-rnnt_amd/csrc/ftr_common.h b/tf-fast-rnnt_amd/csrc/ftr_common.h
--- a/tf-fast-rnnt_amd/csrc/ftr_common.h
+++ b/tf-fast-rnnt_amd/csrc/ftr_common.h
@@ -124,6 +124,16 @@
   v = fmaxf(v, dpp_take<0x142, 0xa, 0xf>(ninf, v));
   v = fmaxf(v, dpp_take<0x143, 0xc, 0xf>(ninf, v));
   return __builtin_bit_cast(float, __builtin_amdgcn_readlane(__builtin_bit_cast(int, v), 63));
+}
+__device__ __forceinline__ int wave_max_int_dpp(int v) {
+  constexpr int lo = -2147483647 - 1;
+  v = max(v, __builtin_amdgcn_update_dpp(lo, v, 0x111, 0xf, 0xf, false));
+  v = max(v, __builtin_amdgcn_update_dpp(lo, v, 0x112, 0xf, 0xf, false));
+  v = max(v, __builtin_amdgcn_update_dpp(lo, v, 0x114, 0xf, 0xe, false));
+  v = max(v, __builtin_amdgcn_update_dpp(lo, v, 0x118, 0xf, 0xc, false));
+  v = max(v, __builtin_amdgcn_update_dpp(lo, v, 0x142, 0xa, 0xf, false));
+  v = max(v, __builtin_amdgcn_update_dpp(lo, v, 0x143, 0xc, 0xf, false));
+  return __builtin_amdgcn_readlane(v, 63);
 }
 
 struct Shift { float cx2, cy2; };
@@ -223,7 +233,8 @@
 size_t simple_colsum_workspace_floats(size_t rows, int C);
 int simple_colsum_weighted(const float* x, const float* w, float* out, float* ws, size_t ws_floats, size_t rows, int C, hipStream_t st);
 int simple_logprobs_fwd(const float* am, const float* lm, const int32_t* symbols, const float* prod, const float* am_max, const float* lm_max, const int32_t* boundary, int blank, double delay_penalty, const float* lmonly_norm, const float* amonly_norm, const float* ulog, float cs, float ls, float as, float* px, float* py, int B, int T, int S, int C, int modified, hipStream_t st);
-int simple_logprobs_bwd_w(const float* gpx, const float* gpy, Scale scale, const float* prod, const int32_t* boundary, float* W, float* rsx, float* rsy, float cs, int B, int T, int S, int modified, hipStream_t st);
+int simple_logprobs_bwd_w(const float* gpx, const float* gpy, Scale scale, const float* prod, const int32_t* boundary, float* W, float* rsx, float* rsy, float cs, int B, int T, int S, int modified, hipStream_t st, int32_t* live = nullptr);
+int bwd_live_dense();
 int simple_logprobs_bwd_am(const float* gpx, const float* gpy, Scale scale, const float* damp, const float* am_probs, const int32_t* symbols, const int32_t* boundary, int blank, float kdir, const float* uvec, const float* amdot, float as, float* Rout, float* d_am, int B, int T, int S, int C, int modified, hipStream_t st);
 int simple_logprobs_bwd_lm(const float* dlmp, const float* lm_probs, const int32_t* symbols, const float* rsx, const float* rsy, int blank, float kdir, const float* arow, const float* invsum, const float* gu, float* d_lm, int B, int S, int C, hipStream_t st);
 int simple_fused_supported(int C);
@@ -234,7 +245,7 @@
 int simple_fused_fwd(const float* am, const float* lm, const int32_t* symbols, const float* am_probs, const float* lm_probs, const float* am_max, const float* lm_max, const int32_t* boundary, int blank, double delay_penalty, const float* lmonly_norm, const float* amonly_norm, const float* ulog, float cs, float ls, float as, float* px, float* py, float* prod_out, int B, int T, int S, int C, int modified, hipStream_t st);
 int simple_fused_bwd_am(const float* gpx, const float* gpy, Scale scale, const float* prod, const float* lm_probs, const float* am_probs, const int32_t* symbols, const int32_t* boundary, int blank, float cs, float kdir, const float* uvec, const float* amdot, float as, float* Rout, float* d_am, int B, int T, int S, int C, int modified, hipStream_t st);
 int simple_fused_bwd_columns(int B, int T, int C);
-int simple_fused_bwd_am_w(const float* gpx, const float* gpy, Scale scale, const float* W, const float* lm_probs, const float* am_probs, const int32_t* symbols, const int32_t* boundary, int blank, float kdir, const float* uvec, const float* amdot, float as, float* Rout, float* d_am, int B, int T, int S, int C, int modified, hipStream_t st);
+int simple_fused_bwd_am_w(const float* gpx, const float* gpy, Scale scale, const float* W, const float* lm_probs, const float* am_probs, const int32_t* symbols, const int32_t* boundary, int blank, float kdir, const float* uvec, const float* amdot, float as, float* Rout, float* d_am, int B, int T, int S, int C, int modified, hipStream_t st, const int32_t* live = nullptr);
 int negated_reduce(const float* ans, int B, int reduction, float* out, hipStream_t st, float sign = -1.0f);
 int pruned_kd_fwd(const void* logits, int dtype, const void* teacher, int teacher_dtype, const int32_t* symbols, const int32_t* ranges, const int32_t* boundary, int blank, float temperature, int collapsed, float* node, float* saved, float* utt, int B, int T, int S, int C, int r, hipStream_t st);
 int pruned_kd_bwd(const void* logits, int dtype, const void* teacher, int teacher_dtype, const int32_t* symbols, const int32_t* ranges, const int32_t* boundary, int blank, float temperature, int collapsed, const float* saved, Scale scale, void* glogits, int B, int T, int S, int C, int r, hipStream_t st);
diff --git a/tf-fast-rnnt_amd/csrc/simple_fused.hip b/tf-fast-rnnt_amd/csrc/simple_fused.hip
--- a/tf-fast-rnnt_amd/csrc/simple_fused.hip
+++ b/tf-fast-rnnt_amd/csrc/simple_fused.hip
@@ -275,11 +275,12 @@
 }
 
 template <bool MOD, bool USEW, int NCB>
-__global__ __launch_bounds__(256, NCB <= 8 ? 4 : 2) void simple_fused_bwd_am_kernel(
+__global__ __launch_bounds__(256, NCB <= 8 ? 4 : 3) void simple_fused_bwd_am_kernel(
     const float* __restrict__ gpx, const float* __restrict__ gpy, const Scale scale, const float* __restrict__ prod,
     const float* __restrict__ lm_probs, const float* __restrict__ am_probs, const int32_t* __restrict__ symbols,
     const int32_t* __restrict__ boundary, int blank, float cs, float kdir, const float* __restrict__ uvec,
-    const float* __restrict__ amdot, float as, float* __restrict__ Rout, float* __restrict__ d_am, int T, int S, int C) {
+    const float* __restrict__ amdot, float as, float* __restrict__ Rout, float* __restrict__ d_am, int T, int S, int C,
+    const int32_t* __restrict__ live) {
   extern __shared__ __attribute__((aligned(16))) float smem[];
   constexpr int CT = 16 * NCB, LDC = CT, NG = NCB / 4;
   static_assert(NCB % 4 == 0 && NCB >= 8 && NCB <= 16, "column blocks come in interleaved groups of four");
@@ -306,6 +307,25 @@
   const float* prb = prod + (size_t)b * (S + 1) * T;
   const float* lmb = lm_probs + (size_t)b * (S + 1) * C;
   const int nk = (S + 1 + kBS - 1) / kBS;
+  int kc_lo = 0, kc_hi = nk;
+  if (live) {
+    const int32_t* lv = live + (size_t)b * (S + 1) * 2;
+    int smin = S + 1, smax = -1;
+    for (int s = tid; s <= S; s += 256) {
+      const int2 iv = *reinterpret_cast<const int2*>(lv + 2 * s);
+      if (iv.x < t0 + kBT && iv.y > t0) { smin = min(smin, s); smax = s; }
+    }
+    smin = -wave_max_int_dpp(-smin); smax = wave_max_int_dpp(smax);
+    int* red = reinterpret_cast<int*>(csb);
+    if (lane == 0) { red[wave] = smin; red[4 + wave] = smax; }
+    __syncthreads();
+    smin = min(min(red[0], red[1]), min(red[2], red[3]));
+    smax = max(max(red[4], red[5]), max(red[6], red[7]));
+    smin = __builtin_amdgcn_readfirstlane(smin); smax = __builtin_amdgcn_readfirstlane(smax);
+    kc_lo = smax < 0 ? 0 : smin / kBS;
+    kc_hi = smax < 0 ? 0 : smax / kBS + 1;
+    __syncthreads();
+  }
 
   constexpr int NL = (kBS * CT / 4) / 256;
   int lrow[NL], lcol[NL];
@@ -392,15 +412,17 @@
         __builtin_amdgcn_sched_barrier(0);
       }
     };
-    Stage g;
-    load(0, g, true);
-    park(0, g);
-    __syncthreads();
-    for (int kc = 0; kc < nk; ++kc) {
-      if (kc + 1 < nk) load(kc + 1, g, true);
-      compute(kc);
-      if (kc + 1 < nk) park(kc + 1, g);
+    if (kc_lo < kc_hi) {
+      Stage g;
+      load(kc_lo, g, true);
+      park(kc_lo, g);
       __syncthreads();
+      for (int kc = kc_lo; kc < kc_hi; ++kc) {
+        if (kc + 1 < kc_hi) load(kc + 1, g, true);
+        compute(kc);
+        if (kc + 1 < kc_hi) park(kc + 1, g);
+        __syncthreads();
+      }
     }
   }
   *reinterpret_cast<f4*>(csb + (0 * kBS + wrow) * kBT + 4 * wq) = sx;
@@ -444,11 +466,12 @@
     int* wcnt = reinterpret_cast<int*>(csb);
     int count = 0;
     const bool listed = S <= 65535;
+    const int r_lo = min(kc_lo * kBS, S), r_hi = min(kc_hi * kBS, S);
     __syncthreads();
     if (listed) {
-      for (int base = 0; base < S; base += 256) {
+      for (int base = r_lo; base < r_hi; base += 256) {
         const int srow = base + tid;
-        const int sy = srow < S ? min(max(symbols[(size_t)b * S + srow], 0), C - 1) : -1;
+        const int sy = srow < r_hi ? min(max(symbols[(size_t)b * S + srow], 0), C - 1) : -1;
         const bool mine = sy >= c0 && sy < c0 + CT;
         const unsigned long long m = __ballot(mine);
         if (lane == 0) wcnt[wave] = __popcll(m);
@@ -463,8 +486,8 @@
       }
     }
     const bool all_rows = !listed || count > kCap;
-    if (all_rows) count = S;
-    auto row_of = [&](int i) { return all_rows ? i : (int)rlist[i]; };
+    if (all_rows) count = r_hi - r_lo;
+    auto row_of = [&](int i) { return all_rows ? r_lo + i : (int)rlist[i]; };
     constexpr int NX = kB2 * (kBT / 4) / 256;
     for (int r0 = 0; r0 < count; r0 += kB2) {
       f4 xv[NX];
@@ -575,7 +598,7 @@
 static int fused_bwd_am_launch(const char* what, int ncb, const float* gpx, const float* gpy, Scale scale, const float* prod_or_w,
                                const float* lm_probs, const float* am_probs, const int32_t* symbols, const int32_t* boundary,
                                int blank, float cs, float kdir, const float* uvec, const float* amdot, float as, float* Rout,
-                               float* d_am, int B, int T, int S, int C, int modified, hipStream_t st) {
+                               float* d_am, int B, int T, int S, int C, int modified, hipStream_t st, const int32_t* live = nullptr) {
   if (!simple_fused_bwd_supported(T, C)) {
     set_error("%s: T = %d, C = %d is outside the fused kernel's domain (T %% 4 == 0, C %% 4 == 0)", what, T, C);
     return FTR_ERR_UNSUPPORTED;
@@ -585,7 +608,7 @@
   dispatch(modified != 0, [&](auto mod) {
     dispatch_among<8, kBCB>(ncb, [&](auto nb) {
       constexpr int NCB = USEW ? decltype(nb)::value : kBCB;
-      hipLaunchKernelGGL((simple_fused_bwd_am_kernel<decltype(mod)::value, USEW, NCB>), grid, dim3(256), fused_bwd_lds_bytes<NCB>(), st, gpx, gpy, scale, prod_or_w, lm_probs, am_probs, symbols, boundary, blank, cs, kdir, uvec, amdot, as, Rout, d_am, T, S, C);
+      hipLaunchKernelGGL((simple_fused_bwd_am_kernel<decltype(mod)::value, USEW, NCB>), grid, dim3(256), fused_bwd_lds_bytes<NCB>(), st, gpx, gpy, scale, prod_or_w, lm_probs, am_probs, symbols, boundary, blank, cs, kdir, uvec, amdot, as, Rout, d_am, T, S, C, live);
     });
   });
   return check_launch(what);
@@ -601,9 +624,9 @@
 int simple_fused_bwd_am_w(const float* gpx, const float* gpy, Scale scale, const float* W, const float* lm_probs,
                           const float* am_probs, const int32_t* symbols, const int32_t* boundary, int blank, float kdir,
                           const float* uvec, const float* amdot, float as, float* Rout, float* d_am, int B, int T, int S,
-                          int C, int modified, hipStream_t st) {
+                          int C, int modified, hipStream_t st, const int32_t* live) {
   const int ncb = simple_fused_bwd_columns(B, T, C) / 16;
-  return fused_bwd_am_launch<true>("simple_logprobs_fused_bwd_am_w", ncb, gpx, gpy, scale, W, lm_probs, am_probs, symbols, boundary, blank, 1.0f, kdir, uvec, amdot, as, Rout, d_am, B, T, S, C, modified, st);
-}
-
-}
+  return fused_bwd_am_launch<true>("simple_logprobs_fused_bwd_am_w", ncb, gpx, gpy, scale, W, lm_probs, am_probs, symbols, boundary, blank, 1.0f, kdir, uvec, amdot, as, Rout, d_am, B, T, S, C, modified, st, live);
+}
+
+}
diff --git a/tf-fast-rnnt_amd/csrc/simple_logprobs.hip b/tf-fast-rnnt_amd/csrc/simple_logprobs.hip
--- a/tf-fast-rnnt_amd/csrc/simple_logprobs.hip
+++ b/tf-fast-rnnt_amd/csrc/simple_logprobs.hip
@@ -1,5 +1,6 @@
 #include "ftr_common.h"
 #include "launch.h"
+#include <string.h>
 
 namespace ftr {
 namespace {
@@ -218,12 +219,16 @@
   }
 }
 
+__device__ __forceinline__ bool any_nonzero_bits(float x, float y, float w) {
+  return ((__builtin_bit_cast(unsigned, x) | __builtin_bit_cast(unsigned, y) | __builtin_bit_cast(unsigned, w)) & 0x7fffffffu) != 0u;
+}
 template <bool MOD>
 __global__ __launch_bounds__(256) void simple_bwd_w_kernel(const float* __restrict__ gpx, const float* __restrict__ gpy,
                                                            const Scale scale, const float* __restrict__ prod,
                                                            const int32_t* __restrict__ boundary, float* __restrict__ W,
                                                            float* __restrict__ rsx, float* __restrict__ rsy, float cs,
-                                                           int T, int S, int B) {
+                                                           int T, int S, int B, int32_t* __restrict__ live,
+                                                           int live_dense) {
   const int lane = threadIdx.x & 63;
   const size_t rowid = (size_t)blockIdx.x * 4 + (threadIdx.x >> 6);
   if (rowid >= (size_t)B * (S + 1)) return;
@@ -236,6 +241,7 @@
   const float sc = scale.at(b);
   const bool hasx = s < S;
   float sx = 0.0f, sy = 0.0f;
+  int tlo = T, thi = 0;
   const int n4 = T >> 2;
   for (int q = lane; q < n4; q += 64) {
     const int t = 4 * q;
@@ -251,6 +257,8 @@
       const float y = gy[e] * sc;
       sx += x; sy += y;
       w[e] = -cs * (x + y) / (pr[e] + kTiny);
+      const bool lv = any_nonzero_bits(x, y, w[e]);
+      tlo = min(tlo, lv ? t + e : T); thi = lv ? t + e + 1 : thi;
     }
     *reinterpret_cast<f4u*>(W + rowy + t) = w;
   }
@@ -259,10 +267,17 @@
     if (hasx && (MOD || t != te)) x = gpx[rowx + t] * sc;
     const float y = gpy[rowy + t] * sc;
     sx += x; sy += y;
-    W[rowy + t] = -cs * (x + y) / (prod[rowy + t] + kTiny);
+    const float w = -cs * (x + y) / (prod[rowy + t] + kTiny);
+    W[rowy + t] = w;
+    if (any_nonzero_bits(x, y, w)) { tlo = min(tlo, t); thi = t + 1; }
   }
   sx = wave_sum(sx); sy = wave_sum(sy);
   if (lane == 0) { rsx[rowid] = sx; rsy[rowid] = sy; }
+  if (live) {
+    tlo = -wave_max_int_dpp(-tlo); thi = wave_max_int_dpp(thi);
+    if (live_dense) { tlo = 0; thi = T; }
+    if (lane == 0) { live[2 * rowid] = tlo; live[2 * rowid + 1] = thi; }
+  }
 }
 
 constexpr int kBwdAmPF = 1;
@@ -561,12 +576,19 @@
   });
 }
 
+int bwd_live_dense() {
+  const char* e = getenv("FTR_BWD_LIVE");
+  return (e && strcmp(e, "dense") == 0) ? 1 : 0;
+}
+
 int simple_logprobs_bwd_w(const float* gpx, const float* gpy, Scale scale, const float* prod, const int32_t* boundary,
-                          float* W, float* rsx, float* rsy, float cs, int B, int T, int S, int modified, hipStream_t st) {
+                          float* W, float* rsx, float* rsy, float cs, int B, int T, int S, int modified, hipStream_t st,
+                          int32_t* live) {
   const size_t rows = (size_t)B * (S + 1);
+  const int live_dense = bwd_live_dense();
   const dim3 grid((unsigned)((rows + 3) / 4));
   dispatch(modified != 0, [&](auto mod) {
-    hipLaunchKernelGGL(simple_bwd_w_kernel<decltype(mod)::value>, grid, dim3(256), 0, st, gpx, gpy, scale, prod, boundary, W, rsx, rsy, cs, T, S, B);
+    hipLaunchKernelGGL(simple_bwd_w_kernel<decltype(mod)::value>, grid, dim3(256), 0, st, gpx, gpy, scale, prod, boundary, W, rsx, rsy, cs, T, S, B, live, live_dense);
   });
   return check_launch("simple_logprobs_bwd_w");
 }
diff --git a/tf-fast-rnnt_amd/tf_fast_rnnt/_lib.py b/tf-fast-rnnt_amd/tf_fast_rnnt/_lib.py
--- a/tf-fast-rnnt_amd/tf_fast_rnnt/_lib.py
+++ b/tf-fast-rnnt_amd/tf_fast_rnnt/_lib.py
@@ -117,6 +117,12 @@
     "ftr_smoothed_logprobs_fused_bwd_am_w_f32": (_i, [_c_fp, _c_fp, _c_fp, _i, _f, _c_fp, _c_fp, _c_fp, _c_ip, _c_ip, _i, _f, _c_fp, _c_fp, _f, _c_fp, _c_fp, _i, _i, _i, _i, _i, _c_st]),
     "ftr_simple_logprobs_fused_bwd_am_w_columns": (_i, [_i, _i, _i]),
 }
+_LIVE_SIGNATURES = {
+    "ftr_simple_logprobs_bwd_w_live_f32": (_i, [_c_fp, _c_fp, _c_fp, _i, _f, _c_fp, _c_ip, _c_fp, _c_fp, _c_fp, _c_ip, _i, _i, _i, _i, _c_st]),
+    "ftr_smoothed_logprobs_bwd_w_live_f32": (_i, [_c_fp, _c_fp, _c_fp, _i, _f, _c_fp, _c_ip, _f, _c_fp, _c_fp, _c_fp, _c_ip, _i, _i, _i, _i, _c_st]),
+    "ftr_simple_logprobs_fused_bwd_am_live_f32": (_i, [_c_fp, _c_fp, _c_fp, _i, _f, _c_fp, _c_ip, _c_fp, _c_fp, _c_ip, _c_ip, _i, _c_fp, _i, _i, _i, _i, _i, _c_st]),
+    "ftr_smoothed_logprobs_fused_bwd_am_live_f32": (_i, [_c_fp, _c_fp, _c_fp, _i, _f, _c_fp, _c_ip, _c_fp, _c_fp, _c_ip, _c_ip, _i, _f, _c_fp, _c_fp, _f, _c_fp, _c_fp, _i, _i, _i, _i, _i, _c_st]),
+}
 _BAND_TDT_SIGNATURES = {
     "ftr_mutual_information_band_tdt_workspace_floats": (ctypes.c_size_t, [_i, _i, _i, _i, _i, _i]),
     "ftr_mutual_information_band_tdt_supported": (_i, [_i, _i, _i, _i, _i]),
@@ -142,6 +148,7 @@
 JOINER_ACT_SYMBOLS = tuple(_JOINER_ACT_SIGNATURES)
 KD_SYMBOLS = tuple(_KD_SIGNATURES)
 FUSED_SYMBOLS = tuple(_FUSED_SIGNATURES)
+LIVE_SYMBOLS = tuple(_LIVE_SIGNATURES)
 BAND_TDT_SYMBOLS = tuple(_BAND_TDT_SIGNATURES)
 BAND_MULTIBLANK_SYMBOLS = tuple(_BAND_MULTIBLANK_SIGNATURES)
 BAND_VITERBI_SYMBOLS = tuple(_BAND_VITERBI_SIGNATURES)
@@ -162,7 +169,7 @@
                 f"{LIB_PATH} is missing: build the HIP extension first (python -c 'import __graft_entry__ as g; "
                 "g.build()' or make -C tf-fast-rnnt_amd/csrc).  tf_fast_rnnt has no CPU fallback.")
         handle = ctypes.CDLL(LIB_PATH)
-        for name, (restype, argtypes) in {**_SIGNATURES, **_LOWP_SIGNATURES, **_PRUNE_SUM_SIGNATURES, **_JOINER_ACT_SIGNATURES, **_KD_SIGNATURES, **_FUSED_SIGNATURES,
+        for name, (restype, argtypes) in {**_SIGNATURES, **_LOWP_SIGNATURES, **_PRUNE_SUM_SIGNATURES, **_JOINER_ACT_SIGNATURES, **_KD_SIGNATURES, **_FUSED_SIGNATURES, **_LIVE_SIGNATURES,
                                             **_BAND_TDT_SIGNATURES, **_BAND_MULTIBLANK_SIGNATURES, **_BAND_VITERBI_SIGNATURES}.items():
             fn = getattr(handle, name)
             fn.restype = restype
diff --git a/tf-fast-rnnt_amd/tf_fast_rnnt/rnnt_loss.py b/tf-fast-rnnt_amd/tf_fast_rnnt/rnnt_loss.py
--- a/tf-fast-rnnt_amd/tf_fast_rnnt/rnnt_loss.py
+++ b/tf-fast-rnnt_amd/tf_fast_rnnt/rnnt_loss.py
@@ -80,6 +80,10 @@
     if mode == "library" or not _use_fused_builder(C) or not _lib.lib().ftr_simple_logprobs_fused_bwd_supported(int(T), int(C)):
         return False
     return True
+
+
+def _live_scratch(d_lm: torch.Tensor, B: int, S: int) -> torch.Tensor:
+    return d_lm.view(-1)[:2 * B * (S + 1)].view(torch.int32).view(B, S + 1, 2)
 
 
 def _simple_builder(amc, lmc, symbols, am_probs, lm_probs, am_max, lm_max, boundary, blank, delay_penalty, px, py,
@@ -128,14 +132,20 @@
     rsx = torch.empty((B, S + 1), dtype=torch.float32, device=dev)
     rsy = torch.empty((B, S + 1), dtype=torch.float32, device=dev)
     d_am = torch.empty_like(am_probs); d_lm = torch.empty_like(lm_probs)
+    fused = _use_fused_builder_bwd(T, C, B)
     with torch.cuda.device(dev):
         st = _stream_ptr(am_probs)
-        _lib.call("ftr_simple_logprobs_bwd_w_scaled_f32", _ptr(gpx), _ptr(gpy), _ptr(scale), stride, mul,
-                  _ptr(prod), _ptr(boundary), _ptr(W), _ptr(rsx), _ptr(rsy), B, T, S, modified, st)
+        if fused:
+            live = _live_scratch(d_lm, B, S)
+            _lib.call("ftr_simple_logprobs_bwd_w_live_f32", _ptr(gpx), _ptr(gpy), _ptr(scale), stride, mul,
+                      _ptr(prod), _ptr(boundary), _ptr(W), _ptr(rsx), _ptr(rsy), _ptr(live), B, T, S, modified, st)
+        else:
+            _lib.call("ftr_simple_logprobs_bwd_w_scaled_f32", _ptr(gpx), _ptr(gpy), _ptr(scale), stride, mul,
+                      _ptr(prod), _ptr(boundary), _ptr(W), _ptr(rsx), _ptr(rsy), B, T, S, modified, st)
         dlmp = _gemm(1, W, am_probs, B, T, S, C, st)
-        if _use_fused_builder_bwd(T, C, B):
-            _lib.call("ftr_simple_logprobs_fused_bwd_am_w_f32", _ptr(gpx), _ptr(gpy), _ptr(scale), stride, mul,
-                      _ptr(W), _ptr(lm_probs), _ptr(am_probs), _ptr(symbols), _ptr(boundary), blank, _ptr(d_am),
+        if fused:
+            _lib.call("ftr_simple_logprobs_fused_bwd_am_live_f32", _ptr(gpx), _ptr(gpy), _ptr(scale), stride, mul,
+                      _ptr(W), _ptr(live), _ptr(lm_probs), _ptr(am_probs), _ptr(symbols), _ptr(boundary), blank, _ptr(d_am),
                       B, T, S, C, modified, st)
         else:
             damp = _gemm(2, W, lm_probs, B, T, S, C, st)
@@ -1427,14 +1437,20 @@
     rsy = torch.empty((B, S + 1), dtype=torch.float32, device=dev)
     R = torch.empty((B, T), dtype=torch.float32, device=dev)
     d_am = torch.empty_like(am_probs); d_lm = torch.empty_like(lm_probs)
+    fused = _use_fused_builder_bwd(T, C, B)
     with torch.cuda.device(dev):
         st = _stream_ptr(am_probs)
-        _lib.call("ftr_smoothed_logprobs_bwd_w_scaled_f32", _ptr(gpx), _ptr(gpy), _ptr(scale), stride, mul, _ptr(prod),
-                  _ptr(boundary), cs, _ptr(W), _ptr(rsx), _ptr(rsy), B, T, S, modified, st)
+        if fused:
+            live = _live_scratch(d_lm, B, S)
+            _lib.call("ftr_smoothed_logprobs_bwd_w_live_f32", _ptr(gpx), _ptr(gpy), _ptr(scale), stride, mul, _ptr(prod),
+                      _ptr(boundary), cs, _ptr(W), _ptr(rsx), _ptr(rsy), _ptr(live), B, T, S, modified, st)
+        else:
+            _lib.call("ftr_smoothed_logprobs_bwd_w_scaled_f32", _ptr(gpx), _ptr(gpy), _ptr(scale), stride, mul, _ptr(prod),
+                      _ptr(boundary), cs, _ptr(W), _ptr(rsx), _ptr(rsy), B, T, S, modified, st)
         dlmp = _gemm(1, W, am_probs, B, T, S, C, st)
-        if _use_fused_builder_bwd(T, C, B):
-            _lib.call("ftr_smoothed_logprobs_fused_bwd_am_w_f32", _ptr(gpx), _ptr(gpy), _ptr(scale), stride, mul, _ptr(W),
-                      _ptr(lm_probs), _ptr(am_probs), _ptr(symbols), _ptr(boundary), blank, cs + a_s, _ptr(u),
+        if fused:
+            _lib.call("ftr_smoothed_logprobs_fused_bwd_am_live_f32", _ptr(gpx), _ptr(gpy), _ptr(scale), stride, mul, _ptr(W),
+                      _ptr(live), _ptr(lm_probs), _ptr(am_probs), _ptr(symbols), _ptr(boundary), blank, cs + a_s, _ptr(u),
                       _ptr(am_dot), a_s, _ptr(R), _ptr(d_am), B, T, S, C, modified, st)
         else:
             damp = _gemm(2, W, lm_probs, B, T, S, C, st)
```

Result: faster. 25270 utterances/s, median of 6 (+2.3%).
